# ezeli/InSentiCap_model

Hardware: AMD Instinct MI355X
Metric: captions/sec (greedy, 36-region feats, len-20) (higher is better)
Workload: dtype f32

## Files before the change

include/insenticap_hip.h:

```cpp
#ifndef INSENTICAP_HIP_H
#define INSENTICAP_HIP_H

#include <stdint.h>

#ifdef __cplusplus
extern "C" {
#endif

#define ISC_OK 0
#define ISC_E_NULL (-1)
#define ISC_E_SHAPE (-2)
#define ISC_E_ALIGN (-3)
#define ISC_E_WORKSPACE (-4)
#define ISC_E_STATE (-5)

#define ISC_MAX_SEG 4

int isc_abi_version(void);
const char *isc_target_arch(void);
int isc_set_tile_override(int tile);
int isc_set_h3_mode(int mode);
long long isc_h3_launches(void);
int isc_set_gemv_rows(int rows);
long long isc_gemv_launches(void);
long long isc_h3x_launches(void);
long long isc_h3s_launches(void);
long long isc_f32_launches(int kind);
long long isc_h3_kernel_launches(int kind);
int isc_h3_weights_begin(void *buf, long long bytes, void *stream);
int isc_h3_weights_end(void *stream);
int isc_h3_weights_suspend(void *stream);
int isc_h3_weights_resume(void *buf, void *stream);
int isc_h3_weights_refresh(void *stream);

typedef struct {
    const float *A;
    const float *W;
    int32_t lda, ldw, K;
    int32_t a_f16;
    const void *A_hi, *A_lo;
} isc_seg;

typedef struct {
    isc_seg seg[ISC_MAX_SEG];
    int32_t nseg, M, N, relu;
    const float *bias0, *bias1, *bias2;
    const uint8_t *keep_mask;
    float mask_scale;
    int32_t ldc;
    float *C;
    float *C_pre;
    int32_t accumulate;
    int32_t _pad;
    float *splitk_ws;
    int64_t splitk_ws_floats;
} isc_linear_problem;

int isc_linear_fwd(const isc_linear_problem *probs_host, int n_prob, void *stream);
int isc_linear_f16_native(const isc_linear_problem *probs_host, int n_prob, void *stream);
long long isc_h3_f16a_launches(void);
int isc_f16_to_f32(const void *src, int64_t ld_src, float *dst, int64_t ld_dst, int64_t rows, int64_t cols,
                   void *stream);
long long isc_f16_convert_launches(void);

#define ISC_LAYOUT_NN 1
#define ISC_LAYOUT_TN 2
int isc_gemm_bwd(const isc_linear_problem *probs_host, int n_prob, int layout, void *stream);

typedef struct {
    isc_seg seg[ISC_MAX_SEG];
    int32_t nseg, M, H, _pad;
    const float *b_ih, *b_hh;
    const float *c_prev;
    float *h_out, *c_out;
    float *gates_out;
    const uint8_t *h_keep_mask;
    float mask_scale;
    float *hdrop_out;
    void *h_hi, *h_lo;
    const float *pre;
    const float *tab;
    const int64_t *tab_ids;
    int64_t tab_ids_stride;
    float *splitk_ws;
    int64_t splitk_ws_floats;
    int32_t pre_div, _pad2;
} isc_lstm_problem;

int isc_lstm_fwd(const isc_lstm_problem *prob_host, void *stream);

int isc_vocab_fwd(const float *h, int ldh, const float *W, int ldw, const float *bias,
                  int M, int V, int K, float *logits, int64_t ld_logits,
                  float *part_max, float *part_sum, int32_t *part_idx,
                  const void *h_hi, const void *h_lo,
                  float *splitk_ws, int64_t splitk_ws_floats, void *stream);

int isc_logsoftmax_apply(float *logits, int64_t ld_logits, int M, int V,
                         const float *part_max, const float *part_sum, float *lse_out,
                         void *stream);
int isc_logsoftmax_apply_steps(float *logits, int64_t ld_b, int64_t ld_t, int B, int T, int V,
                               const float *part_max, const float *part_sum, const float *src, int step_rows,
                               void *stream);

typedef struct {
    const float *P, *V, *q, *q2, *w;
    const float *w_bias;
    int32_t R, A, D;
    int32_t rows;
    float *out;
    float *alpha_out;
    int64_t alpha_ld;
    void *out_hi, *out_lo;
    const int64_t *row_ids;
    int64_t row_ids_ld;
    int32_t row_div, _pad;
} isc_scan_problem;

int isc_attn_scan_fwd(const isc_scan_problem *probs_host, int n_prob, int B, void *stream);

typedef struct {
    isc_scan_problem scan[2];
    const float *G[2];
    const float *zh;
    const float *b_gc, *b_gs;
    const float *w_gate;
    const float *b_gate;
    float *f;
    void *f_hi, *f_lo;
    float *beta;
    int64_t beta_ld;
} isc_scan_gate_args;
int isc_attn_scan_gate_fwd(const isc_scan_gate_args *args_host, int B, void *stream);

int isc_gate_mix_fwd(const float *z, const float *w, const float *w_bias, const float *v,
                     const float *s, int B, int A, int D, float *out, float *beta_out,
                     int64_t beta_ld, void *out_hi, void *out_lo, void *stream);

int isc_embed_relu_fwd(const float *emb, int V, int W, const int64_t *ids, int64_t ids_stride,
                       const float *add, int B, float *out, void *stream);

int isc_embed_relu_mean_fwd(const float *emb, int V, int W, const int64_t *ids, int C, int B,
                            float *out, void *stream);

int isc_embed_senti_words_fwd(const float *emb, int V, int W, const int64_t *ids, int n_words,
                              int64_t pad_id, int B, const uint8_t *keep_mask, float mask_scale,
                              float *out, void *stream);

typedef struct {
    int32_t B, V, T, t;
    int32_t n_tile, W;
    const float *part_max, *part_sum;
    const int32_t *part_idx;
    const float *logits;
    int64_t ld_logits;
    const int64_t *forced;
    const float *sample_u;
    int64_t eos_id;
    int64_t *seq;
    float *seq_logprobs;
    float *seq_masks;
    int32_t *unfinished;
    int32_t *alive;
    int64_t *raw_tokens;
    const float *emb;
    const float *xt_add;
    float *xt_next;
} isc_rollout_step;

int isc_rollout_finalize(const isc_rollout_step *s_host, void *stream);
long long isc_rollout_finalize_launches(void);

typedef struct {
// ... 17 lines not shown
int isc_sched_sample(const float *logp, int64_t ld, int M, int V, const float *part_max,
                     const float *part_sum, const int32_t *part_idx, const float *u_select,
                     const float *u_draw, float ss_prob, const int64_t *base_ids, int64_t base_stride,
                     int64_t *out_ids, void *stream);
int isc_sched_sample_raw(const float *logits, int64_t ld, int M, int V, const float *part_max,
                     const float *part_sum, const int32_t *part_idx, const float *u_select,
                     const float *u_draw, float ss_prob, const int64_t *base_ids, int64_t base_stride,
                     int64_t *out_ids, void *stream);

int isc_beam_topk(const float *logits, int64_t ld_logits, const float *part_max,
                  const float *part_sum, int n_tile, int rows, int V, int beam,
                  const int64_t *last_word, int64_t pad_id, int64_t sos_id, int64_t unk_id,
                  int mask_special, int decoding_constraint, float *top_val, int64_t *top_idx,
                  void *stream);

typedef struct {
    int32_t n_img, beam, T, t;
    int64_t eos_id;
    const float *top_val;
    const int64_t *top_idx;
    const double *score_in;
    double *score_out;
    const int64_t *last_in;
    int64_t *last_out;
    const int64_t *words_in;
    int64_t *words_out;
    const int32_t *len_in;
    int32_t *len_out;
    int32_t *done;
    int64_t *gather;
    int32_t *live;
} isc_beam_merge_args;

int isc_beam_merge(const isc_beam_merge_args *args_host, void *stream);
int isc_beam_gather(const float *state_next, const float *state_cur, const int64_t *gather, float *out,
                    int planes, int rows, int H, void *stream);

#define ISC_COPY_MULTI_MAX 8
int isc_copy_multi(void *const *dst, const void *const *src, const int64_t *bytes, int n, void *stream);

int isc_xe_loss_fwd(const float *logp, const int64_t *target, const int32_t *lengths, int B,
                    int T, int V, float *out2, void *stream);


typedef struct {
    int32_t rows, H, E, A, W, V, R, Mw;
    const float *Wih1, *Whh1;
    const float *Wih2, *Whh2;
    const float *b_ih2, *b_hh2;
    const float *W_h2att, *b_h2att, *w_alpha_c, *b_alpha_c;
    const float *W_h2word, *b_h2word, *w_alpha_s, *b_alpha_s;
    const float *W_gh, *b_gh, *W_gc, *b_gc, *W_gs, *b_gs, *w_gate, *b_gate;
    const float *W_cls, *b_cls;
    const float *pre1;
    const float *tab;
    const float *att_p, *att_e;
    const float *words_p, *words_e;
    const float *label_w;
    const float *xt;
    const int64_t *tok;
    int64_t tok_stride;
    const float *h1_prev, *c1_prev, *h2_prev, *c2_prev;
    float *h1, *c1, *h2, *c2;
    float *g1, *g2;
    float *qa, *v, *qw, *s, *z, *f;
    float *alpha_c, *alpha_s, *beta;
    int64_t alpha_c_ld, alpha_s_ld, beta_ld;
    const uint8_t *out_mask;
    float out_scale;
    int32_t apply_logsoftmax;
    float *hdrop;
    float *logits;
    int64_t ld_logits;
    float *pmax, *psum;
    int32_t *pidx;
    float *splitk_ws;
    int64_t splitk_ws_floats;
    const void *h1_prev_hi, *h1_prev_lo, *h2_prev_hi, *h2_prev_lo;
    void *h1_hi, *h1_lo, *h2_hi, *h2_lo;
    void *v_hi, *v_lo, *s_hi, *s_lo, *f_hi, *f_lo;
    const int64_t *words_ids;
    int64_t words_ids_ld;
    const float *gate_Gc, *gate_Gs;
    int32_t pair_rows_c, _pad2;
    int32_t row_div, pre_rows;
} isc_step_plan;

int isc_step_fwd(const isc_step_plan *plan_host, void *stream);

int isc_set_stream_gate(const int32_t *flag, void *stream);

typedef struct {
    const int64_t *src_row;
    int32_t stats_tile, beam;
    float *cand_val;
    int32_t *cand_idx;
    const int64_t *last_word;
    int64_t pad_id, sos_id, unk_id;
    int32_t mask_special, decoding_constraint;
    int32_t row_div, _pad;
    const int32_t *live_in;
    const isc_rollout_step *fin_prev;
    int32_t *fin_unfinished_out;
} isc_rows_ext;
int isc_rows_stats_tile(int V);
int isc_rows_step_supported(const isc_step_plan *plan_host);
int isc_rows_step_fwd(const isc_step_plan *plan_host, const isc_rows_ext *ext_host, void *stream);
int isc_rows_vocab_fwd(const float *h, int ldh, const float *W, int ldw, const float *bias, int M, int V, int K,
                       float *part_max, float *part_sum, int32_t *part_idx, float *logits, int64_t ld_logits,
                       const isc_rows_ext *ext_host, void *stream);
int isc_set_rows_nt(int mode);
long long isc_rows_launches(void);
int isc_set_rows_scan_max(int rows);
int isc_set_rows_scan_regions(int regions);
int isc_set_h3v(int on);
int isc_set_h3_ksplit(int on);
int isc_set_h3_vocab_tile(int rows);

typedef struct {
    int32_t n_img, beam, T, t;
    int32_t n_tile, V;
    int64_t eos_id;
    const float *part_max, *part_sum;
    const float *cand_val;
    const int32_t *cand_idx;
    const double *score_in;
    double *score_out;
    const int64_t *last_in;
    int64_t *last_out;
    const int64_t *words_in;
    int64_t *words_out;
    const int32_t *len_in;
    int32_t *len_out;
    int32_t *done;
    int64_t *src_row;
    int32_t *live;
    float *top_val;
    int64_t *top_idx;
    const int32_t *live_in;
    const float *state_in;
    float *state_out;
    int32_t state_planes, H;
} isc_beam_select_args;
int isc_beam_select(const isc_beam_select_args *args_host, void *stream);

typedef struct {
    int32_t rows, H, E, A, W, R, Mw, first, last;
    int32_t pair_rows_c;
    const float *Wih1, *Whh1, *Wih2, *Whh2;
    const float *W_h2att, *w_alpha_c, *W_h2word, *w_alpha_s, *W_gh, *W_gc, *W_gs, *w_gate;
    const float *att_p, *att_e, *words_p, *words_e, *label_w;
    const float *g1, *c1_prev, *c1, *g2, *c2_prev, *c2;
    const float *qa, *qw, *v, *s, *z;
    const float *alpha_c, *alpha_s, *beta;
    int64_t alpha_c_ld, alpha_s_ld, beta_ld;
    const float *dhd;
    float *dG1, *dG2;
    float *dG1_sum;
    float *d_feat, *dh1, *dv, *ds;
    float *dh2_rec, *dh1_rec;
    const float *dc1_in, *dc2_in;
    float *dc1_out, *dc2_out;
    float *dqa, *dqw, *dz;
    float *dP_att, *dV_att, *dP_w, *dV_w;
    float *dwc_rows, *dws_rows, *dwg_rows, *dbg_rows;
    float *splitk_ws;
    int64_t splitk_ws_floats;
    float *de_c, *de_s;
    int32_t row_div, _pad;
} isc_step_bwd_plan;

// ... 172 lines not shown
```

insenticap_model_amd/_lib.py:

```python
import ctypes as C
import os

_HERE = os.path.dirname(os.path.abspath(__file__))
LIB_PATH = os.environ.get('ISC_HIP_LIB') or os.path.join(_HERE, 'lib', 'libinsenticap_hip.so')

ISC_MAX_SEG = 4

c_f32p = C.c_void_p


class Seg(C.Structure):
    _fields_ = [('A', C.c_void_p), ('W', C.c_void_p), ('lda', C.c_int32), ('ldw', C.c_int32),
                ('K', C.c_int32), ('a_f16', C.c_int32), ('A_hi', C.c_void_p), ('A_lo', C.c_void_p)]


class LinearProblem(C.Structure):
    _fields_ = [('seg', Seg * ISC_MAX_SEG), ('nseg', C.c_int32), ('M', C.c_int32), ('N', C.c_int32),
                ('relu', C.c_int32), ('bias0', C.c_void_p), ('bias1', C.c_void_p), ('bias2', C.c_void_p),
                ('keep_mask', C.c_void_p), ('mask_scale', C.c_float), ('ldc', C.c_int32),
                ('C', C.c_void_p), ('C_pre', C.c_void_p), ('accumulate', C.c_int32), ('_pad', C.c_int32),
                ('splitk_ws', C.c_void_p), ('splitk_ws_floats', C.c_int64)]


class LstmProblem(C.Structure):
    _fields_ = [('seg', Seg * ISC_MAX_SEG), ('nseg', C.c_int32), ('M', C.c_int32), ('H', C.c_int32),
                ('_pad', C.c_int32), ('b_ih', C.c_void_p), ('b_hh', C.c_void_p),
                ('c_prev', C.c_void_p), ('h_out', C.c_void_p), ('c_out', C.c_void_p),
                ('gates_out', C.c_void_p), ('h_keep_mask', C.c_void_p), ('mask_scale', C.c_float),
                ('hdrop_out', C.c_void_p), ('h_hi', C.c_void_p), ('h_lo', C.c_void_p),
                ('pre', C.c_void_p), ('tab', C.c_void_p),
                ('tab_ids', C.c_void_p), ('tab_ids_stride', C.c_int64),
                ('splitk_ws', C.c_void_p), ('splitk_ws_floats', C.c_int64),
                ('pre_div', C.c_int32), ('_pad2', C.c_int32)]


class ScanProblem(C.Structure):
    _fields_ = [('P', C.c_void_p), ('V', C.c_void_p), ('q', C.c_void_p), ('q2', C.c_void_p),
                ('w', C.c_void_p), ('w_bias', C.c_void_p), ('R', C.c_int32), ('A', C.c_int32),
                ('D', C.c_int32), ('rows', C.c_int32), ('out', C.c_void_p), ('alpha_out', C.c_void_p),
                ('alpha_ld', C.c_int64), ('out_hi', C.c_void_p), ('out_lo', C.c_void_p),
                ('row_ids', C.c_void_p), ('row_ids_ld', C.c_int64), ('row_div', C.c_int32), ('_pad', C.c_int32)]


class ScanBwdProblem(C.Structure):
    _fields_ = [('P', C.c_void_p), ('V', C.c_void_p), ('q', C.c_void_p), ('q2', C.c_void_p),
                ('w', C.c_void_p), ('alpha', C.c_void_p), ('dout', C.c_void_p), ('alpha_ld', C.c_int64),
                ('R', C.c_int32), ('A', C.c_int32), ('D', C.c_int32), ('accumulate', C.c_int32),
                ('dP', C.c_void_p), ('dV', C.c_void_p), ('dq', C.c_void_p), ('dw_rows', C.c_void_p),
                ('de_out', C.c_void_p), ('rows', C.c_int32), ('row_div', C.c_int32)]


class ScanGateArgs(C.Structure):
    _fields_ = [('scan', ScanProblem * 2), ('G', C.c_void_p * 2), ('zh', C.c_void_p), ('b_gc', C.c_void_p),
                ('b_gs', C.c_void_p), ('w_gate', C.c_void_p), ('b_gate', C.c_void_p), ('f', C.c_void_p),
                ('f_hi', C.c_void_p), ('f_lo', C.c_void_p), ('beta', C.c_void_p), ('beta_ld', C.c_int64)]


def _f(names, ctype):
    return [(n, ctype) for n in names.split()]


class StepPlan(C.Structure):
    _fields_ = (_f('rows H E A W V R Mw', C.c_int32) +
                _f('Wih1 Whh1 Wih2 Whh2 b_ih2 b_hh2 W_h2att b_h2att w_alpha_c b_alpha_c W_h2word b_h2word '
                   'w_alpha_s b_alpha_s W_gh b_gh W_gc b_gc W_gs b_gs w_gate b_gate W_cls b_cls '
                   'pre1 tab att_p att_e words_p words_e label_w xt tok', C.c_void_p) +
                [('tok_stride', C.c_int64)] +
                _f('h1_prev c1_prev h2_prev c2_prev h1 c1 h2 c2 g1 g2 qa v qw s z f alpha_c alpha_s beta',
                   C.c_void_p) +
                _f('alpha_c_ld alpha_s_ld beta_ld', C.c_int64) +
                [('out_mask', C.c_void_p), ('out_scale', C.c_float), ('apply_logsoftmax', C.c_int32),
                 ('hdrop', C.c_void_p), ('logits', C.c_void_p), ('ld_logits', C.c_int64),
                 ('pmax', C.c_void_p), ('psum', C.c_void_p), ('pidx', C.c_void_p),
                 ('splitk_ws', C.c_void_p), ('splitk_ws_floats', C.c_int64)] +
                _f('h1_prev_hi h1_prev_lo h2_prev_hi h2_prev_lo h1_hi h1_lo h2_hi h2_lo '
                   'v_hi v_lo s_hi s_lo f_hi f_lo words_ids', C.c_void_p) + [('words_ids_ld', C.c_int64)] +
                _f('gate_Gc gate_Gs', C.c_void_p) + _f('pair_rows_c _pad2 row_div pre_rows', C.c_int32))


class StepBwdPlan(C.Structure):
    _fields_ = (_f('rows H E A W R Mw first last pair_rows_c', C.c_int32) +
                _f('Wih1 Whh1 Wih2 Whh2 W_h2att w_alpha_c W_h2word w_alpha_s W_gh W_gc W_gs w_gate '
                   'att_p att_e words_p words_e label_w g1 c1_prev c1 g2 c2_prev c2 qa qw v s z '
                   'alpha_c alpha_s beta', C.c_void_p) +
                _f('alpha_c_ld alpha_s_ld beta_ld', C.c_int64) +
                _f('dhd dG1 dG2 dG1_sum d_feat dh1 dv ds dh2_rec dh1_rec dc1_in dc2_in dc1_out dc2_out '
                   'dqa dqw dz dP_att dV_att dP_w dV_w dwc_rows dws_rows dwg_rows dbg_rows splitk_ws',
                   C.c_void_p) + [('splitk_ws_floats', C.c_int64), ('de_c', C.c_void_p), ('de_s', C.c_void_p),
                              ('row_div', C.c_int32), ('_pad', C.c_int32)])


class BeamMergeArgs(C.Structure):
    _fields_ = ([('n_img', C.c_int32), ('beam', C.c_int32), ('T', C.c_int32), ('t', C.c_int32), ('eos_id', C.c_int64)] +
                _f('top_val top_idx score_in score_out last_in last_out words_in words_out len_in len_out done gather live',
                   C.c_void_p))


class RowsExt(C.Structure):
    _fields_ = [('src_row', C.c_void_p), ('stats_tile', C.c_int32), ('beam', C.c_int32), ('cand_val', C.c_void_p),
                ('cand_idx', C.c_void_p), ('last_word', C.c_void_p), ('pad_id', C.c_int64), ('sos_id', C.c_int64),
                ('unk_id', C.c_int64), ('mask_special', C.c_int32), ('decoding_constraint', C.c_int32),
                ('row_div', C.c_int32), ('_pad', C.c_int32), ('live_in', C.c_void_p), ('fin_prev', C.c_void_p),
                ('fin_unfinished_out', C.c_void_p)]


class BeamSelectArgs(C.Structure):
    _fields_ = ([('n_img', C.c_int32), ('beam', C.c_int32), ('T', C.c_int32), ('t', C.c_int32), ('n_tile', C.c_int32),
                 ('V', C.c_int32), ('eos_id', C.c_int64)] +
                _f('part_max part_sum cand_val cand_idx score_in score_out last_in last_out words_in words_out len_in '
                   'len_out done src_row live top_val top_idx live_in state_in state_out', C.c_void_p) +
                [('state_planes', C.c_int32), ('H', C.c_int32)])


ISC_COLSUM_MAX_JOBS, ISC_COLSUM_MAX_OUT = 24, 3
ISC_SCALE_SRC_MAX = 4


class ColsumJob(C.Structure):
    _fields_ = [('x', C.c_void_p), ('ld', C.c_int64), ('M', C.c_int32), ('N', C.c_int32),
                ('out', C.c_void_p * ISC_COLSUM_MAX_OUT), ('n_out', C.c_int32), ('accumulate', C.c_int32)]


class RolloutStep(C.Structure):
    _fields_ = [('B', C.c_int32), ('V', C.c_int32), ('T', C.c_int32), ('t', C.c_int32),
                ('n_tile', C.c_int32), ('W', C.c_int32),
                ('part_max', C.c_void_p), ('part_sum', C.c_void_p), ('part_idx', C.c_void_p),
                ('logits', C.c_void_p), ('ld_logits', C.c_int64),
                ('forced', C.c_void_p), ('sample_u', C.c_void_p), ('eos_id', C.c_int64),
                ('seq', C.c_void_p), ('seq_logprobs', C.c_void_p), ('seq_masks', C.c_void_p),
                ('unfinished', C.c_void_p), ('alive', C.c_void_p), ('raw_tokens', C.c_void_p),
                ('emb', C.c_void_p), ('xt_add', C.c_void_p), ('xt_next', C.c_void_p)]


class SampleFilter(C.Structure):
    _fields_ = [('temperature', C.c_float), ('top_k', C.c_int32), ('top_p', C.c_float),
                ('sampling_logprobs', C.c_void_p)]


class DecodeConstraints(C.Structure):
    _fields_ = [('ban_ids', C.c_int64 * 8), ('n_ban', C.c_int32), ('no_repeat', C.c_int32), ('first_id', C.c_int64),
                ('min_len', C.c_int32)]


class SentClsProblem(C.Structure):
    _fields_ = (_f('B L W H V k T_out _pad', C.c_int32) + [('tokens', C.c_void_p), ('tokens_ld', C.c_int64)] +
                _f('lens emb w_ih w_hh b_ih b_hh ex0_w ex0_b ex2_w ex2_b cls0_w cls0_b cls3_w cls3_b labels workspace',
                   C.c_void_p) + [('workspace_bytes', C.c_int64)] + _f('logits weights pred reward feats', C.c_void_p))


SENTI_DET_MAX_CONVS = SENTI_DET_MAX_FCS = 4
SENTI_DET_MAX_HW = 1024
SENTI_DET_KINDS = ('direct', 'split', 'reduce', 'tail', 'pack', 'f16')


class SentiDetProblem(C.Structure):
    _fields_ = ([('feats', C.c_void_p)] + _f('feats_f16 B h w C n_convs n_fcs k neu_idx ksplit', C.c_int32) +
                [('threshold', C.c_float), ('_pad', C.c_int32), ('packed', C.c_void_p),
                 ('conv_b', C.c_void_p * SENTI_DET_MAX_CONVS)] + _f('senti_w senti_b', C.c_void_p) +
                [('fc_w', C.c_void_p * SENTI_DET_MAX_FCS), ('fc_b', C.c_void_p * SENTI_DET_MAX_FCS),
                 ('workspace', C.c_void_p), ('workspace_bytes', C.c_int64)] +
                _f('logits maps labels scores conv_out', C.c_void_p))


SIGNATURES = {
    'isc_abi_version': (C.c_int, []),
    'isc_target_arch': (C.c_char_p, []),
    'isc_set_tile_override': (C.c_int, [C.c_int]),
    'isc_set_h3_mode': (C.c_int, [C.c_int]),
    'isc_h3_launches': (C.c_longlong, []),
    'isc_set_gemv_rows': (C.c_int, [C.c_int]),
    'isc_colsum_multi': (C.c_int, [C.POINTER(ColsumJob), C.c_int, C.c_void_p, C.c_int64, C.c_void_p]),
    'isc_gemv_launches': (C.c_longlong, []),
    'isc_h3x_launches': (C.c_longlong, []),
    'isc_h3s_launches': (C.c_longlong, []),
    'isc_f32_launches': (C.c_longlong, [C.c_int]),
    'isc_h3_kernel_launches': (C.c_longlong, [C.c_int]),
    'isc_h3_weights_begin': (C.c_int, [C.c_void_p, C.c_longlong, C.c_void_p]),
    'isc_h3_weights_end': (C.c_int, [C.c_void_p]),
    'isc_h3_weights_suspend': (C.c_int, [C.c_void_p]),
    'isc_h3_weights_resume': (C.c_int, [C.c_void_p, C.c_void_p]),
    'isc_h3_weights_refresh': (C.c_int, [C.c_void_p]),
    'isc_linear_fwd': (C.c_int, [C.POINTER(LinearProblem), C.c_int, C.c_void_p]),
    'isc_linear_f16_native': (C.c_int, [C.POINTER(LinearProblem), C.c_int, C.c_void_p]),
    'isc_h3_f16a_launches': (C.c_longlong, []),
    'isc_f16_to_f32': (C.c_int, [C.c_void_p, C.c_int64, C.c_void_p, C.c_int64, C.c_int64, C.c_int64, C.c_void_p]),
    'isc_f16_convert_launches': (C.c_longlong, []),
    'isc_gemm_bwd': (C.c_int, [C.POINTER(LinearProblem), C.c_int, C.c_int, C.c_void_p]),
    'isc_lstm_fwd': (C.c_int, [C.POINTER(LstmProblem), C.c_void_p]),
    'isc_step_fwd': (C.c_int, [C.POINTER(StepPlan), C.c_void_p]),
    'isc_set_stream_gate': (C.c_int, [C.c_void_p, C.c_void_p]),
    'isc_step_bwd': (C.c_int, [C.POINTER(StepBwdPlan), C.c_void_p]),
    'isc_rows_stats_tile': (C.c_int, [C.c_int]),
    'isc_rows_step_supported': (C.c_int, [C.POINTER(StepPlan)]),
    'isc_rows_step_fwd': (C.c_int, [C.POINTER(StepPlan), C.POINTER(RowsExt), C.c_void_p]),
    'isc_rows_vocab_fwd': (C.c_int, [C.c_void_p, C.c_int, C.c_void_p, C.c_int, C.c_void_p, C.c_int, C.c_int, C.c_int,
                                     C.c_void_p, C.c_void_p, C.c_void_p, C.c_void_p, C.c_int64, C.POINTER(RowsExt),
                                     C.c_void_p]),
    'isc_set_rows_nt': (C.c_int, [C.c_int]),
    'isc_set_rows_scan_max': (C.c_int, [C.c_int]),
    'isc_set_rows_scan_regions': (C.c_int, [C.c_int]),
    'isc_set_h3v': (C.c_int, [C.c_int]),
    'isc_set_h3_ksplit': (C.c_int, [C.c_int]),
    'isc_set_h3_vocab_tile': (C.c_int, [C.c_int]),
    'isc_copy_multi': (C.c_int, [C.POINTER(C.c_void_p), C.POINTER(C.c_void_p), C.POINTER(C.c_int64), C.c_int, C.c_void_p]),
    'isc_rows_launches': (C.c_longlong, []),
    'isc_beam_select': (C.c_int, [C.POINTER(BeamSelectArgs), C.c_void_p]),
    'isc_vocab_fwd': (C.c_int, [C.c_void_p, C.c_int, C.c_void_p, C.c_int, C.c_void_p, C.c_int, C.c_int,
                                C.c_int, C.c_void_p, C.c_int64, C.c_void_p, C.c_void_p, C.c_void_p,
                                C.c_void_p, C.c_void_p, C.c_void_p, C.c_int64, C.c_void_p]),
    'isc_sched_sample': (C.c_int, [C.c_void_p, C.c_int64, C.c_int, C.c_int, C.c_void_p, C.c_void_p, C.c_void_p,
                                   C.c_void_p, C.c_void_p, C.c_float, C.c_void_p, C.c_int64, C.c_void_p,
                                   C.c_void_p]),
    'isc_sched_sample_raw': (C.c_int, [C.c_void_p, C.c_int64, C.c_int, C.c_int, C.c_void_p, C.c_void_p, C.c_void_p,
                                   C.c_void_p, C.c_void_p, C.c_float, C.c_void_p, C.c_int64, C.c_void_p,
                                   C.c_void_p]),
    'isc_logsoftmax_apply': (C.c_int, [C.c_void_p, C.c_int64, C.c_int, C.c_int, C.c_void_p, C.c_void_p,
                                       C.c_void_p, C.c_void_p]),
    'isc_logsoftmax_apply_steps': (C.c_int, [C.c_void_p, C.c_int64, C.c_int64, C.c_int, C.c_int, C.c_int, C.c_void_p,
                                             C.c_void_p, C.c_void_p, C.c_int, C.c_void_p]),
    'isc_attn_scan_fwd': (C.c_int, [C.POINTER(ScanProblem), C.c_int, C.c_int, C.c_void_p]),
    'isc_attn_scan_gate_fwd': (C.c_int, [C.POINTER(ScanGateArgs), C.c_int, C.c_void_p]),
    'isc_gate_mix_fwd': (C.c_int, [C.c_void_p, C.c_void_p, C.c_void_p, C.c_void_p, C.c_void_p, C.c_int,
                                   C.c_int, C.c_int, C.c_void_p, C.c_void_p, C.c_int64, C.c_void_p, C.c_void_p,
                                   C.c_void_p]),
    'isc_embed_relu_fwd': (C.c_int, [C.c_void_p, C.c_int, C.c_int, C.c_void_p, C.c_int64, C.c_void_p,
                                     C.c_int, C.c_void_p, C.c_void_p]),
    'isc_embed_relu_mean_fwd': (C.c_int, [C.c_void_p, C.c_int, C.c_int, C.c_void_p, C.c_int, C.c_int,
                                          C.c_void_p, C.c_void_p]),
    'isc_embed_senti_words_fwd': (C.c_int, [C.c_void_p, C.c_int, C.c_int, C.c_void_p, C.c_int, C.c_int64,
                                            C.c_int, C.c_void_p, C.c_float, C.c_void_p, C.c_void_p]),
    'isc_rollout_finalize': (C.c_int, [C.POINTER(RolloutStep), C.c_void_p]),
    'isc_rollout_finalize_launches': (C.c_longlong, []),
    'isc_rollout_finalize_filtered': (C.c_int, [C.POINTER(RolloutStep), C.POINTER(SampleFilter), C.c_void_p]),
    'isc_rollout_finalize_constrained': (C.c_int, [C.POINTER(RolloutStep), C.POINTER(SampleFilter),
                                                   C.POINTER(DecodeConstraints), C.c_void_p]),
    'isc_beam_merge': (C.c_int, [C.POINTER(BeamMergeArgs), C.c_void_p]),
    'isc_beam_gather': (C.c_int, [C.c_void_p, C.c_void_p, C.c_void_p, C.c_void_p, C.c_int, C.c_int, C.c_int, C.c_void_p]),
    'isc_beam_topk': (C.c_int, [C.c_void_p, C.c_int64, C.c_void_p, C.c_void_p, C.c_int, C.c_int, C.c_int,
                                C.c_int, C.c_void_p, C.c_int64, C.c_int64, C.c_int64, C.c_int, C.c_int,
                                C.c_void_p, C.c_void_p, C.c_void_p]),
    'isc_xe_loss_fwd': (C.c_int, [C.c_void_p, C.c_void_p, C.c_void_p, C.c_int, C.c_int, C.c_int,
                                  C.c_void_p, C.c_void_p]),
    'isc_logsoftmax_bwd': (C.c_int, [C.c_void_p, C.c_void_p, C.c_int64, C.c_int, C.c_int, C.c_void_p,
                                     C.c_int64, C.c_int, C.c_void_p]),
    'isc_lstm_bwd': (C.c_int, [C.c_void_p, C.c_void_p, C.c_void_p, C.c_void_p, C.c_void_p, C.c_void_p,
                               C.c_int, C.c_int, C.c_void_p, C.c_void_p, C.c_void_p, C.c_void_p]),
    'isc_attn_scan_bwd': (C.c_int, [C.POINTER(ScanBwdProblem), C.c_int, C.c_int, C.c_void_p]),
    'isc_attn_dv_from_alpha': (C.c_int, [C.c_void_p, C.c_int64, C.c_int64, C.c_void_p, C.c_int, C.c_int, C.c_int,
                                         C.c_int, C.c_void_p, C.c_int, C.c_void_p]),
    'isc_attn_dp_from_de': (C.c_int, [C.c_void_p, C.c_void_p, C.c_void_p, C.c_void_p, C.c_void_p, C.c_int, C.c_int,
                                      C.c_int, C.c_int, C.c_void_p, C.c_void_p]),
    'isc_attn_dv_from_alpha_group': (C.c_int, [C.c_void_p, C.c_int64, C.c_int64, C.c_void_p, C.c_int, C.c_int, C.c_int,
                                               C.c_int, C.c_int, C.c_void_p, C.c_int, C.c_void_p]),
    'isc_attn_dp_from_de_group': (C.c_int, [C.c_void_p, C.c_void_p, C.c_void_p, C.c_void_p, C.c_void_p, C.c_int, C.c_int,
                                            C.c_int, C.c_int, C.c_int, C.c_void_p, C.c_void_p]),
    'isc_gate_mix_bwd': (C.c_int, [C.c_void_p, C.c_void_p, C.c_void_p, C.c_void_p, C.c_void_p, C.c_int64,
                                   C.c_void_p, C.c_int, C.c_int, C.c_int, C.c_void_p, C.c_void_p,
                                   C.c_void_p, C.c_void_p, C.c_void_p, C.c_int, C.c_void_p]),
    'isc_embed_relu_bwd': (C.c_int, [C.c_void_p, C.c_int, C.c_int, C.c_void_p, C.c_int64, C.c_int, C.c_int,
                                     C.c_int, C.c_int64, C.c_void_p, C.c_float, C.c_void_p, C.c_float,
                                     C.c_void_p, C.c_int64, C.c_void_p]),
    'isc_embed_relu_bwd_ws': (C.c_int, [C.c_void_p, C.c_int, C.c_int, C.c_void_p, C.c_int64, C.c_int, C.c_int,
                                        C.c_int, C.c_int64, C.c_void_p, C.c_float, C.c_void_p, C.c_float,
                                        C.c_void_p, C.c_int64, C.c_void_p, C.c_int64, C.c_void_p]),
    'isc_colsum': (C.c_int, [C.c_void_p, C.c_int64, C.c_int, C.c_int, C.c_void_p, C.c_int, C.c_void_p, C.c_int64,
                             C.c_void_p]),
    'isc_relu_mask_bwd': (C.c_int, [C.c_void_p, C.c_void_p, C.c_void_p, C.c_float, C.c_int64, C.c_void_p,
                                    C.c_void_p]),
    'isc_xe_loss_bwd': (C.c_int, [C.c_void_p, C.c_void_p, C.c_int, C.c_int, C.c_int, C.c_void_p,
                                  C.c_void_p, C.c_void_p, C.c_void_p]),
    'isc_xe_loss_bwd_sparse': (C.c_int, [C.c_void_p, C.c_int, C.c_int, C.c_void_p, C.c_void_p, C.c_void_p, C.c_void_p]),
    'isc_reward_loss_fwd': (C.c_int, [C.c_void_p, C.c_void_p, C.c_void_p, C.c_int, C.c_int, C.c_void_p, C.c_void_p]),
# ... 71 lines not shown
```

insenticap_model_amd/captioner.py:

```python
import ctypes as C
import itertools
import weakref

import torch
import torch.nn as nn

from . import _lib, ops
from ._lib import RolloutStep


class ContentAttention(nn.Module):
    def __init__(self, settings):
        super().__init__()
        self.h2att = nn.Linear(settings['rnn_hid_dim'], settings['att_hid_dim'])
        self.att_alpha = nn.Linear(settings['att_hid_dim'], 1)


class SentiAttention(nn.Module):
    def __init__(self, settings):
        super().__init__()
        self.h2word = nn.Linear(settings['rnn_hid_dim'], settings['att_hid_dim'])
        self.label2word = nn.Linear(settings['word_emb_dim'], settings['att_hid_dim'])
        self.word_alpha = nn.Linear(settings['att_hid_dim'], 1)

# ... 315 lines not shown
        if cached is not None:
            return cached
        if not build:
            return None
        st = self.settings
        H, E, Wd, V = st['rnn_hid_dim'], st['feat_emb_dim'], st['word_emb_dim'], self.vocab_size
        act = self._new(V, Wd)
        ops.embed_relu_fwd(emb, torch.arange(V, dtype=torch.int64, device=self._dev), act)
        tab = self._new(V, 4 * H)
        ops.linear_fwd([ops.linear_problem([(act, Wih[:, H + E:])], tab)])
        return self._table_cache('_tab_cache', key, tab)

    ROWS_STEP_MAX = 8

    def _rows_step_ok(self, rows, P):
        st = self.settings
        E, A, Wd, H = st['feat_emb_dim'], st['att_hid_dim'], st['word_emb_dim'], st['rnn_hid_dim']
        return (getattr(self, 'rows_step', True) and 0 < rows <= self.ROWS_STEP_MAX and not ops.TIMER.armed
                and self._rows_vocab_ok()
                and ops.TIMER.arm_step is None and getattr(P, 'gate_Gc', None) is not None
                and getattr(P, 'gate_Gs', None) is not None and A == E == Wd and A <= 512 and A % 4 == 0 and H % 4 == 0
                and H <= 1024)

    def _rows_vocab_ok(self):
        V = self.vocab_size
        tw = ops.rows_stats_tile(V)
        return tw > 0 and (V + tw - 1) // tw <= 256

    def _alloc_step_ws(self, rows, P, stats_tile=128):
        st = self.settings
        E, A = st['feat_emb_dim'], st['att_hid_dim']
        has_cont, has_senti = P.att_e3 is not None, P.words_e3 is not None
        ws = {}
        if has_cont:
            ws['qa'], ws['v'] = self._new(rows, A), self._new(rows, E)
        if has_senti:
            ws['qw'], ws['s'] = self._new(rows, A), self._new(rows, E)
        if has_cont and has_senti:
            ws['z'], ws['f'] = self._new(rows, A), self._new(rows, E)
        n_tile = (self.vocab_size + stats_tile - 1) // stats_tile
        ws['pmax'] = self._new(rows, n_tile)
        ws['psum'] = self._new(rows, n_tile)
        ws['pidx'] = self._new(rows, n_tile, dtype=torch.int32)
        return ws

    def _make_plan(self, p, P, rows):
        st = self.settings
        pl = _lib.StepPlan()
        pl.rows, pl.H, pl.E, pl.A = rows, st['rnn_hid_dim'], st['feat_emb_dim'], st['att_hid_dim']
        pl.W, pl.V, pl.R, pl.Mw = st['word_emb_dim'], self.vocab_size, P.R, P.Mw
        for field, key in (('Wih1', 'att_lstm.weight_ih'), ('Whh1', 'att_lstm.weight_hh'),
                           ('Wih2', 'lang_lstm.weight_ih'), ('Whh2', 'lang_lstm.weight_hh'),
                           ('b_ih2', 'lang_lstm.bias_ih'), ('b_hh2', 'lang_lstm.bias_hh'),
                           ('W_h2att', 'attention.cont_att.h2att.weight'), ('b_h2att', 'attention.cont_att.h2att.bias'),
                           ('w_alpha_c', 'attention.cont_att.att_alpha.weight'),
                           ('b_alpha_c', 'attention.cont_att.att_alpha.bias'),
                           ('W_h2word', 'attention.senti_att.h2word.weight'),
                           ('b_h2word', 'attention.senti_att.h2word.bias'),
                           ('w_alpha_s', 'attention.senti_att.word_alpha.weight'),
                           ('b_alpha_s', 'attention.senti_att.word_alpha.bias'),
                           ('W_gh', 'attention.h2att.weight'), ('b_gh', 'attention.h2att.bias'),
                           ('W_gc', 'attention.cont2att.weight'), ('b_gc', 'attention.cont2att.bias'),
                           ('W_gs', 'attention.senti2att.weight'), ('b_gs', 'attention.senti2att.bias'),
                           ('w_gate', 'attention.att_alpha.weight'), ('b_gate', 'attention.att_alpha.bias'),
                           ('W_cls', 'classifier.weight'), ('b_cls', 'classifier.bias')):
            t = p[key]
            assert t.is_contiguous()
            setattr(pl, field, t.data_ptr())
        for field, t in (('pre1', P.pre1), ('tab', P.tab), ('att_p', P.att_p3), ('att_e', P.att_e3),
                         ('words_p', P.words_p3), ('words_e', P.words_e3), ('label_w', P.label_w)):
            if t is not None:
                assert t.is_contiguous()
                setattr(pl, field, t.data_ptr())
        if P.words_ids is not None:
            pl.words_ids, pl.words_ids_ld = P.words_ids.data_ptr(), P.words_ids.stride(0)
        ws = ops.splitk_ws(self._dev)
        pl.splitk_ws, pl.splitk_ws_floats = ws.data_ptr(), ws.numel()
        pl.row_div = P.row_div if P.row_div > 1 else 0
        pl.pre_rows = int(P.pre_rows)
        return pl

    def _step(self, p, P, ws, xt, h_cur, c_cur, h_nxt, c_nxt, alpha_c=None, alpha_s=None, beta=None,
              logits=None, out_mask=None, out_scale=1.0, save=None, tok=None, normalize=False,
              hp_cur=None, hp_nxt=None, rows_ext=None):
        if ops.TIMER.armed:
            return self._step_py(p, P, ws, xt, h_cur, c_cur, h_nxt, c_nxt, alpha_c, alpha_s, beta, logits,
                                 out_mask, out_scale, save, tok, normalize, hp_cur, hp_nxt)
        save = save or {}
        pl = ws.get('_plan')
        if pl is None:
            pl = ws['_plan'] = self._make_plan(p, P, h_cur[0].shape[0])
        ptr = ops.ptr
        pl.xt = ptr(xt)
        if tok is not None and P.tab is not None:
            pl.tok, pl.tok_stride = tok.data_ptr(), tok.stride(0)
        pl.h1_prev, pl.h2_prev, pl.c1_prev, pl.c2_prev = (h_cur[0].data_ptr(), h_cur[1].data_ptr(),
                                                          c_cur[0].data_ptr(), c_cur[1].data_ptr())
        pl.h1, pl.h2, pl.c1, pl.c2 = (h_nxt[0].data_ptr(), h_nxt[1].data_ptr(), c_nxt[0].data_ptr(),
                                      c_nxt[1].data_ptr())
        if hp_cur is not None:
            pl.h1_prev_hi, pl.h1_prev_lo = ops.planes_ptrs(hp_cur[0])
            pl.h2_prev_hi, pl.h2_prev_lo = ops.planes_ptrs(hp_cur[1])
            pl.h1_hi, pl.h1_lo = ops.planes_ptrs(hp_nxt[0])
            pl.h2_hi, pl.h2_lo = ops.planes_ptrs(hp_nxt[1])
            for k in ('v', 's', 'f'):
                pp = ws.get(k + 'p')
                hi, lo = (None, None) if pp is None else ops.planes_ptrs(pp)
                setattr(pl, k + '_hi', hi)
                setattr(pl, k + '_lo', lo)
        else:
            for k in ('h1_prev_hi', 'h1_prev_lo', 'h2_prev_hi', 'h2_prev_lo', 'h1_hi', 'h1_lo', 'h2_hi', 'h2_lo',
                      'v_hi', 'v_lo', 's_hi', 's_lo', 'f_hi', 'f_lo'):
                setattr(pl, k, None)
        pl.g1, pl.g2 = ptr(save.get('g1')), ptr(save.get('g2'))
        for k in ('qa', 'v', 'qw', 's', 'z', 'f'):
            setattr(pl, k, ptr(ws.get(k)))
        pl.alpha_c, pl.alpha_c_ld = (alpha_c.data_ptr(), alpha_c.stride(0)) if alpha_c is not None else (None, 0)
        pl.alpha_s, pl.alpha_s_ld = (alpha_s.data_ptr(), alpha_s.stride(0)) if alpha_s is not None else (None, 0)
        pl.beta, pl.beta_ld = (beta.data_ptr(), beta.stride(0)) if beta is not None else (None, 0)
        hdrop = None
        if out_mask is not None:
            hdrop = save['hdrop'] if 'hdrop' in save else self._new(h_cur[0].shape[0], pl.H)
        pl.out_mask, pl.out_scale, pl.hdrop = ptr(out_mask), out_scale, ptr(hdrop)
        pl.logits, pl.ld_logits = (logits.data_ptr(), logits.stride(0)) if logits is not None else (None, 0)
        pl.apply_logsoftmax = int(normalize)
        pl.pmax, pl.psum, pl.pidx = ptr(ws.get('pmax')), ptr(ws.get('psum')), ptr(ws.get('pidx'))
        pl.gate_Gc, pl.gate_Gs = ptr(getattr(P, 'gate_Gc', None)), ptr(getattr(P, 'gate_Gs', None))
        if rows_ext is not None:
            ops.rows_step_fwd(pl, rows_ext)
        else:
            ops.step_fwd(pl)

    def _step_py(self, p, P, ws, xt, h_cur, c_cur, h_nxt, c_nxt, alpha_c=None, alpha_s=None, beta=None,
                 logits=None, out_mask=None, out_scale=1.0, save=None, tok=None, normalize=False,
                 hp_cur=None, hp_nxt=None):
        save = save or {}
        st = self.settings
        E, H = st['feat_emb_dim'], st['rnn_hid_dim']
        Wih, Whh = p['att_lstm.weight_ih'], p['att_lstm.weight_hh']
        rows = h_cur[0].shape[0]
        pc = (lambda l: None) if hp_cur is None else (lambda l: hp_cur[l])
        pn = (lambda l: None) if hp_nxt is None else (lambda l: hp_nxt[l])
        wp = (lambda k: None) if hp_cur is None else (lambda k: ws.get(k + 'p'))
        segs = [(h_cur[1], Wih[:, 0:H], pc(1)), (h_cur[0], Whh, pc(0))]
        if P.tab is None:
            segs.insert(1, (xt, Wih[:, H + E:]))
        ops.lstm_fwd(segs, None, None, c_cur[0], h_nxt[0], c_nxt[0], gates_out=save.get('g1'),
                     pre=P.pre1, tab=P.tab, tab_ids=tok if P.tab is not None else None, h_planes=pn(0),
                     pre_div=1 if P.pre_rows else P.row_div)
        h1 = h_nxt[0]
        has_cont, has_senti = P.att_e3 is not None, P.words_e3 is not None
        probs, scans = [], []
        if has_cont:
            probs.append(ops.linear_problem([(h1, p['attention.cont_att.h2att.weight'], pn(0))], ws['qa'],
                                            p['attention.cont_att.h2att.bias']))
            scans.append(ops.scan_problem(P.att_p3, P.att_e3, ws['qa'],
                                          p['attention.cont_att.att_alpha.weight'],
                                          p['attention.cont_att.att_alpha.bias'], ws['v'], alpha_c,
                                          out_planes=wp('v'), row_div=P.row_div))
        if has_senti:
            probs.append(ops.linear_problem([(h1, p['attention.senti_att.h2word.weight'], pn(0))], ws['qw'],
                                            p['attention.senti_att.h2word.bias']))
            scans.append(ops.scan_problem(P.words_p3, P.words_e3, ws['qw'],
                                          p['attention.senti_att.word_alpha.weight'],
                                          p['attention.senti_att.word_alpha.bias'], ws['s'], alpha_s,
                                          q2=P.label_w, out_planes=wp('s'), row_ids=P.words_ids,
                                          row_div=P.row_div))
        gate = has_cont and has_senti
        if gate:
            probs.append(ops.linear_problem([(h1, p['attention.h2att.weight'], pn(0))], ws['z'],
                                            p['attention.h2att.bias']))
        ops.linear_fwd(probs)
        fused_gate = gate and getattr(P, 'gate_Gc', None) is not None and getattr(P, 'gate_Gs', None) is not None
        if fused_gate:
            ops.attn_scan_gate_fwd(scans, (P.gate_Gc, P.gate_Gs), ws['z'], p['attention.cont2att.bias'],
                                   p['attention.senti2att.bias'], p['attention.att_alpha.weight'],
                                   p['attention.att_alpha.bias'], ws['f'], beta, f_planes=wp('f'))
            feat, featp = ws['f'], wp('f')
        else:
            ops.attn_scan_fwd(scans, rows)
        if fused_gate:
            pass
        elif gate:
            ops.linear_fwd([ops.linear_problem(
                [(ws['v'], p['attention.cont2att.weight'], wp('v')),
                 (ws['s'], p['attention.senti2att.weight'], wp('s'))],
                ws['z'], p['attention.cont2att.bias'], p['attention.senti2att.bias'], accumulate=True)])
            ops.gate_mix_fwd(ws['z'], p['attention.att_alpha.weight'], p['attention.att_alpha.bias'],
                             ws['v'], ws['s'], ws['f'], beta, out_planes=wp('f'))
            feat, featp = ws['f'], wp('f')
        else:
            feat, featp = (ws['v'], wp('v')) if has_cont else (ws['s'], wp('s'))
        Wih2, Whh2 = p['lang_lstm.weight_ih'], p['lang_lstm.weight_hh']
        hdrop = None
        if out_mask is not None:
            hdrop = save['hdrop'] if 'hdrop' in save else self._new(rows, H)
        ops.lstm_fwd([(feat, Wih2[:, 0:E], featp), (h1, Wih2[:, E:E + H], pn(0)), (h_cur[1], Whh2, pc(1))],
                     p['lang_lstm.bias_ih'], p['lang_lstm.bias_hh'], c_cur[1], h_nxt[1], c_nxt[1],
                     gates_out=save.get('g2'), h_keep_mask=out_mask, mask_scale=out_scale, hdrop_out=hdrop,
                     h_planes=pn(1))
        if ws.get('pmax') is None:
            return
        ops.vocab_fwd(hdrop if hdrop is not None else h_nxt[1], p['classifier.weight'],
                      p['classifier.bias'], ws['pmax'], ws['psum'], ws['pidx'], logits,
                      h_planes=None if hdrop is not None else pn(1))
        if normalize:
            ops.logsoftmax_apply(logits, ws['pmax'], ws['psum'])

    def _set_weights(self, aC, aS, bG, steps):
        self._weights_pending = (aC, aS, bG, steps)
# ... 190 lines not shown
                             'torch.no_grad() (the backward through 1 / temperature is not built)')
        if not sample_max and not self._needs_grad() and _replay is None and (
                filtered or return_sampling_logprobs or _uniforms is not None or generator is not None):
            filt = self._sample_filter(temperature, top_k, top_p, generator, _uniforms, return_sampling_logprobs)
            out = self._rollout(fc_feats, att_feats, cpt_words, senti_words, senti_labels, max_seq_len, 0, None,
                                _masks, filt, group=n_cap, cons=cons)
            return out[:3] + ((filt['slp'],) if return_sampling_logprobs else ())
        if return_sampling_logprobs or _uniforms is not None or generator is not None:
            raise ValueError('generator / return_sampling_logprobs / _uniforms are not available with gradients enabled')
        if not sample_max and self._needs_grad():
            from .autograd import rollout_with_grad
            return rollout_with_grad(self, fc_feats, att_feats, cpt_words, senti_words, senti_labels,
                                     max_seq_len, _replay, _masks, cons, group=n_cap)
        if (sample_max and cons is None and self.__dict__.get('_rollout_graphs') is not None and not self._needs_grad()
                and not self.training and _replay is None and _masks is None and ops.TIMER.arm_step is None
                and fc_feats.shape[0] <= self.ROLLOUT_GRAPH_MAX_ROWS and ops.graphs_allowed_here()
                and fc_feats.is_cuda and not torch.cuda.is_current_stream_capturing()
                and self._features_in_domain(fc_feats, att_feats)):
            return self._graphed_rollout(fc_feats, att_feats, cpt_words, senti_words, senti_labels, max_seq_len)
        return self._rollout(fc_feats, att_feats, cpt_words, senti_words, senti_labels, max_seq_len,
                             sample_max, _replay, _masks, group=n_cap, cons=cons)[:3]

    def _decode_constraints(self, suppress_special, decoding_constraint, min_len, max_seq_len):
        special, no_repeat, min_len = ops.check_decode_constraints(suppress_special, decoding_constraint, min_len,
                                                                   max_seq_len)
        ban = []
        if special and self.pad_id != self.eos_id:
            for i in (self.pad_id, self.sos_id, self.unk_id):
                if i not in ban:
                    ban.append(i)
        if not ban and not no_repeat and not min_len:
            return None
        if self.vocab_size <= len(ban) + 2:
            raise ValueError('a vocabulary of %d words leaves nothing to choose under the constraints' % self.vocab_size)
        return ops.decode_constraints(ban, no_repeat, self.sos_id, min_len)

    def _check_captions_per_image(self, n, sample_max, masks, fc_feats=None, senti_labels=None):
        if isinstance(n, bool) or not hasattr(n, '__index__'):
            raise ValueError('captions_per_image must be an integer >= 1, got %r' % (n,))
        n = int(n)
        if n < 1:
            raise ValueError('captions_per_image must be an integer >= 1, got %r' % (n,))
        if n == 1:
            return 1
        if sample_max:
            raise ValueError('captions_per_image > 1 applies to sampled roll-outs (sample_max=0): %d greedy captions of '
                             'one image would be identical' % n)
        grad = self._needs_grad()
        if bool(self.training) != grad:
            raise ValueError('captions_per_image > 1 runs in two forms: inference-only (eval mode under torch.no_grad()) '
                             'or the differentiable training roll-out (training mode with gradients enabled); got '
                             'training=%s with gradients %s' % (bool(self.training), 'enabled' if grad else 'disabled'))
        if masks is not None and not grad:
            raise ValueError('captions_per_image > 1 without gradients does not take _masks (dropout masks belong to '
                             'training)')
        if grad and fc_feats is not None and senti_labels is not None:
            images, labels = int(fc_feats.shape[0]), int(senti_labels.numel())
            if labels != images:
                raise ValueError('captions_per_image=%d with gradients: senti_labels must hold one label per image (%d) - '
                                 'the roll-out takes its labels from the image - got %d' % (n, images, labels))
        return n

    def _sample_filter(self, temperature=1.0, top_k=0, top_p=1.0, generator=None, uniforms=None, want_slp=False):
        temperature, top_k, top_p = ops.check_sample_filter(temperature, top_k, top_p)
        return dict(temperature=temperature, top_k=top_k, top_p=top_p, generator=generator, uniforms=uniforms,
                    want_slp=bool(want_slp),
                    filtered=temperature != 1.0 or 0 < top_k < self.vocab_size or top_p < 1.0)

    def enable_rollout_graphs(self, on=True, max_graphs=4):
        self._rollout_graphs = {} if on else None
        self._rollout_graphs_max = max_graphs
        self._graphs_explicit = bool(on)

    def _rollout_stream(self):
        st = self.__dict__.get('_ro_stream')
        if st is None or st.device != self._dev:
            st = self.__dict__['_ro_stream'] = ops.private_stream(self._dev)
            idx = self._dev.index if self._dev.index is not None else torch.cuda.current_device()
            weakref.finalize(self, ops.release_stream_state, idx, st.cuda_stream)
        return st

    def _graphed_rollout(self, fc_feats, att_feats, cpt_words, senti_words, senti_labels, T):
        ins = [self._feat(fc_feats), self._feat(att_feats), cpt_words, senti_words, senti_labels]
        key = (tuple((tuple(x.shape), x.dtype) for x in ins), T, self._weights_key(), torch.cuda.current_device())
        cache = self._rollout_graphs
        st = self._rollout_stream()
        idx = self._dev.index if self._dev.index is not None else torch.cuda.current_device()
        skey = ((idx, st.cuda_stream),)
        cur = torch.cuda.current_stream(self._dev)

        def on_stream(fn):
            st.wait_stream(cur)
            with torch.cuda.stream(st):
                out = fn()
            cur.wait_stream(st)
            return out
        entry = cache.get(key)
        if isinstance(entry, tuple) and entry[4] != ops.h3_weights_scope.cold_begins(skey):
            entry = cache[key] = 'seen'
        if entry is None:
            while len(cache) >= self._rollout_graphs_max:
                self._graph_evicted(cache.pop(next(iter(cache))), 'roll-out')
                if self._rollout_graphs is None:
                    return self._rollout(*ins, T, 1, None, None)[:3]
            cache[key] = 'seen'
            outs = on_stream(lambda: self._rollout(*ins, T, 1, None, None)[:3])
            for o in outs:
                o.record_stream(cur)
            return outs
        cache[key] = cache.pop(key)
        if entry == 'seen':
            static = [x.clone() for x in ins]
            graph = torch.cuda.CUDAGraph()

            def capture():
                with ops.graph_capture(graph, stream=st):
                    o = self._rollout(*static, T, 1, None, None)[:3]
                    return o, self.__dict__.get('_weights_pending')
            outs, pending = on_stream(capture)
            entry = cache[key] = (graph, static, outs, pending, ops.h3_weights_scope.cold_begins(skey))
        graph, static, outs, pending = entry[:4]
        ops.stage_inputs(static, ins)
        graph.replay()
        self._weights_pending = pending
        fresh = [torch.empty_like(o) for o in outs]
        ops.copy_multi(fresh, outs)
        return tuple(fresh)

    GRAPH_THRASH_LIMIT = 8

    def _graph_evicted(self, entry, what):
        if isinstance(entry, str):
            return
        n = self.__dict__['_graph_evictions'] = self.__dict__.get('_graph_evictions', 0) + 1
        if n == self.GRAPH_THRASH_LIMIT and not self.__dict__.get('_graphs_explicit', False):
            import warnings
            warnings.warn('insenticap_model_amd: %d captured %s / beam graphs evicted - input geometries keep changing; '
                          'default graph serving is off for this captioner (enable_rollout_graphs / enable_beam_graphs '
                          'with a larger max_graphs to keep it)' % (n, what))
            self._rollout_graphs = None
            self._beam_graphs = None

    def enable_beam_graphs(self, on=True, max_graphs=4):
        self._beam_graphs = {} if on else None
        self._beam_graphs_max = max_graphs
        self._graphs_explicit = bool(on)

    def _weights_key(self):
        return (('captioner', self._wnonce[0]),) + tuple((q.data_ptr(), q._version) for q in self.parameters()) + \
            (ops.WEIGHT_EPOCH,)

    def _renew_weights_nonce(self):
        self._wnonce[0] = next(_INSTANCE_NONCE)

    def _apply(self, fn, *args, **kwargs):
        out = super()._apply(fn, *args, **kwargs)
        self._renew_weights_nonce()
        return out

    def load_state_dict(self, *args, **kwargs):
        out = super().load_state_dict(*args, **kwargs)
        self._renew_weights_nonce()
        return out

    def _graph_buffers(self):
        gb = self.__dict__.get('_graph_bufs')
        if gb is None or gb[0].device != self._dev:
# ... 8 lines not shown
        if not self._features_in_domain(fc_feats, att_feats):
            with ops.exact_fp32_engine(), ops.h3_weights_scope(self._dev, key=self._weights_key()):
                return self._rollout_impl(fc_feats, att_feats, cpt_words, senti_words, senti_labels, T, sample_max,
                                          replay, masks, filt, group, cons)
        with ops.h3_weights_scope(self._dev, key=self._weights_key()):
            return self._rollout_impl(fc_feats, att_feats, cpt_words, senti_words, senti_labels, T, sample_max,
                                      replay, masks, filt, group, cons)

    SPLIT_F16_MAX = 65504.0

    def _features_in_domain(self, *feats):
        feats = [x for x in feats if x is not None and torch.is_tensor(x) and x.is_floating_point()]
        if (not getattr(self, 'numerics_checks', True) or self.__dict__.get('_domain_check_off') or not feats
                or not all(x.is_cuda for x in feats)
                or ops.h3_mode() == 0 or torch.cuda.is_current_stream_capturing()):
            return True
        memo = self.__dict__.setdefault('_domain_memo', {})
        verdict, fresh = True, []
        for x in feats:
            e = memo.get(id(x))
            if e is not None and e[0]() is x and e[1] == x._version:
                verdict = verdict and e[2]
            else:
                fresh.append(x)
        if fresh:
            worst = torch.stack([torch.linalg.vector_norm(x.detach().reshape(-1), float('inf')).float()
                                 for x in fresh]).amax()
            v = float(worst)
            ok = bool(v < self.SPLIT_F16_MAX)
            for k in [k for k, e in memo.items() if e[0]() is None]:
                del memo[k]
            while len(memo) >= 16:
                memo.pop(next(iter(memo)))
            for x in fresh:
                memo[id(x)] = (weakref.ref(x), x._version, ok)
            verdict = verdict and ok
            if not ok:
                self._warn_out_of_domain('max |x| = %g' % v)
        return verdict

    def _known_out_of_domain(self, *feats, remember=False):
        bad = self.__dict__.setdefault('_domain_bad', {})
        keys = [(x.data_ptr(), x.numel(), x._version) for x in feats
                if x is not None and torch.is_tensor(x) and x.is_floating_point()]
        if remember:
            while len(bad) >= 16:
                bad.pop(next(iter(bad)))
            for k in keys:
                bad[k] = True
            return True
        return any(k in bad for k in keys)

    def _warn_out_of_domain(self, what):
        if not self.__dict__.get('_domain_warned'):
            import warnings
            self.__dict__['_domain_warned'] = True
            warnings.warn('insenticap_model_amd: features beyond the split-f16 operand domain |x| < 65504 (%s): the call '
                          'runs on the exact-fp32 GEMM engine (~2x slower; results as the reference\'s). Scale the '
                          'features to keep the fast engine.' % what)

    def _rollout_impl(self, fc_feats, att_feats, cpt_words, senti_words, senti_labels, T, sample_max, replay,
                      masks, filt=None, group=1, cons=None):
        p = self._p()
        arm = ops.TIMER.arm_step
        ops.TIMER.armed, ops.TIMER.phase = (arm == -1), 'prologue'
        n_rows = fc_feats.shape[0] * group
        want = False
        if not torch.is_grad_enabled() or not any(q.requires_grad for q in self.parameters()):
            want = 'build' if n_rows * T >= self.vocab_size // 4 else 'cached'
        P = self._prologue(p, 'rl', fc_feats, att_feats, cpt_words, senti_words, senti_labels, masks,
                           want_table=want, words_table=bool(want) and getattr(self, 'words_table', True),
                           gate_rows=n_rows if want and group == 1 else 0)
        ops.TIMER.armed, ops.TIMER.phase = False, 'step'
        P.row_div = group
        B, V = P.B * group, self.vocab_size
        H, Wd = self.att_lstm.hidden_size, self.settings['word_emb_dim']
        rows_ext = None
        if ((sample_max or replay is not None) and masks is None and not self.training and group == 1
                and cons is None and self._rows_step_ok(B, P)):
            rows_ext = _lib.RowsExt()
            rows_ext.stats_tile = ops.rows_stats_tile(V)
        planes = rows_ext is None and getattr(self, 'state_planes', True)
        f32, i64 = torch.float32, torch.int64
        h0, c0, hp0 = self._zeros_many(((2, B, H), f32), ((2, B, H), f32),
                                       ((2, 2, B, H) if planes else (0,), torch.float16))
        seq, raw, seq_logprobs, seq_masks, alive, aC, aS, bG, unf = self._zeros_many(
            ((B, T), i64), ((B, T), i64), ((B, T), f32), ((B, T), f32), ((T + 1,), torch.int32), ((B, T, P.R), f32),
            ((B, T, P.Mw), f32), ((B, T), f32), ((T + 1, B), torch.int32))
        h, c = [h0, self._new(2, B, H)], [c0, self._new(2, B, H)]
        hp = [hp0, torch.empty(2, 2, B, H, dtype=torch.float16, device=self._dev)] if planes else [None, None]
        ws = self._alloc_step_ws(B, P, rows_ext.stats_tile if rows_ext is not None else 128)
        if hp[0] is not None:
            for k in ('v', 's', 'f'):
                if k in ws:
                    ws[k + 'p'] = torch.empty((2,) + tuple(ws[k].shape), dtype=torch.float16, device=self._dev)
        unf[0:1].fill_(1)
        unfinished = unf[0]
        alive[0:1].fill_(B)
        use_tab = P.tab is not None
        xt = [None, None] if use_tab else [self._new(B, Wd) for _ in range(2)]
        emb = p['word_embed.0.weight']
        sos = torch.full((B,), self.sos_id, dtype=torch.int64, device=self._dev)
        if not use_tab:
            ops.embed_relu_fwd(emb, sos, xt[0])
        need_logits = (not sample_max) or cons is not None
        logits = self._new(B, V) if need_logits else None
        forced = sample_u = None
        if not sample_max:
            if replay is not None:
                forced = self._ids(replay)
            elif filt is not None and filt['uniforms'] is not None:
                sample_u = filt['uniforms']
                if (not torch.is_tensor(sample_u) or sample_u.dtype != torch.float32 or tuple(sample_u.shape) != (B, T)):
                    raise ValueError('_uniforms must be a float32 tensor of shape [B, T] = [%d, %d]' % (B, T))
                sample_u = sample_u.to(self._dev).contiguous()
            elif filt is not None and filt['generator'] is not None:
                sample_u = torch.rand(B, T, device=self._dev, generator=filt['generator'])
            else:
                sample_u = torch.rand(B, T, device=self._dev)
        filtered = filt is not None and filt['filtered']
        slp = None
        if filt is not None and filt['want_slp'] and (filtered or cons is not None):
            slp = self._zeros(B, T)
        mask_for = self._mask_source(masks)
        rs = RolloutStep()
        rs.B, rs.V, rs.T, rs.n_tile, rs.W = B, V, T, ws['pmax'].shape[1], Wd
        rs.part_max, rs.part_sum, rs.part_idx = ws['pmax'].data_ptr(), ws['psum'].data_ptr(), ws['pidx'].data_ptr()
        rs.logits, rs.ld_logits = ops.ptr(logits), V
        rs.forced, rs.sample_u = ops.ptr(forced), ops.ptr(sample_u)
        rs.eos_id = self.eos_id
        rs.seq, rs.seq_logprobs, rs.seq_masks = seq.data_ptr(), seq_logprobs.data_ptr(), seq_masks.data_ptr()
        rs.unfinished, rs.alive, rs.raw_tokens = unfinished.data_ptr(), alive.data_ptr(), raw.data_ptr()
        rs.emb, rs.xt_add = emb.data_ptr(), None
        fuse = (rows_ext is not None and sample_max and replay is None and use_tab and arm is None and B <= 4
                and getattr(self, 'rows_fused_finalize', True))
        rs_prev = RolloutStep.from_buffer_copy(rs) if fuse else None
        with ops.h3_weights_scope(self._dev):
            for t in range(T):
                cur, nxt = t & 1, (t + 1) & 1
                om, osc = mask_for('out%d' % t, B, H)
                ops.TIMER.armed = (arm == t)
                if fuse:
                    if t > 0:
                        rs_prev.t, rs_prev.unfinished = t - 1, unf[t - 1].data_ptr()
                        rows_ext.fin_prev, rows_ext.fin_unfinished_out = C.addressof(rs_prev), unf[t].data_ptr()
                    else:
                        rows_ext.fin_prev = rows_ext.fin_unfinished_out = None
                self._step(p, P, ws, xt[cur], h[cur], c[cur], h[nxt], c[nxt], aC[:, t], aS[:, t], bG[:, t:t + 1],
                           logits, om, osc, tok=(sos if t == 0 else seq[:, t - 1]) if use_tab else None,
                           hp_cur=hp[cur], hp_nxt=hp[nxt], rows_ext=rows_ext)
                if fuse and t + 1 < T:
                    continue
                rs.t = t
                rs.unfinished = unf[t].data_ptr() if fuse else unfinished.data_ptr()
                rs.xt_next = None if use_tab else xt[nxt].data_ptr()
                ops.rollout_finalize_step(rs, cons, filt, slp)
        ops.TIMER.armed = False
        if filt is not None and filt['want_slp']:
            filt['slp'] = slp if slp is not None else seq_logprobs.clone()
        self._set_weights(aC, aS, bG, alive)
        return seq, seq_logprobs, seq_masks, raw, alive

    def sample(self, fc_feat, att_feat, senti_words=None, senti_label=None,
               beam_size=3, decoding_constraint=1, max_seq_len=16):
        caps, scores, _ = self.sample_batch(
            fc_feat.reshape(1, -1), att_feat.reshape(1, -1, att_feat.shape[-1]),
            None if senti_words is None else senti_words.reshape(1, -1),
            None if senti_label is None else senti_label.reshape(1),
            beam_size, decoding_constraint, max_seq_len)
        return caps[0], scores[0]

    @torch.no_grad()
    def sample_batch(self, fc_feats, att_feats, senti_words=None, senti_labels=None,
                     beam_size=3, decoding_constraint=1, max_seq_len=16):
        from .beam import beam_search_batch, replay_if_captured
        if self.training:
            self.eval()
        checks = getattr(self, 'numerics_checks', True)

        def on_exact_engine():
            self._p()
            with ops.exact_fp32_engine(), ops.h3_weights_scope(self._dev, key=self._weights_key()):
                res = beam_search_batch(self, fc_feats, att_feats, senti_words, senti_labels, beam_size,
                                        decoding_constraint, max_seq_len, graphs=False)
            ops.device_status(reset=True)
            return res
        if checks and ops.h3_mode() != 0 and self._known_out_of_domain(fc_feats, att_feats):
            return on_exact_engine()
        out = replay_if_captured(self, fc_feats, att_feats, senti_words, senti_labels, beam_size, decoding_constraint,
                                 max_seq_len)
        if out is None:
            self._p()
            with ops.h3_weights_scope(self._dev, key=self._weights_key()):
                out = beam_search_batch(self, fc_feats, att_feats, senti_words, senti_labels, beam_size,
                                        decoding_constraint, max_seq_len)
        if checks:
            if ops.h3_mode() != 0 and ops.device_status(reset=True):
                self._known_out_of_domain(fc_feats, att_feats, remember=True)
                self._warn_out_of_domain('non-finite values in a beam search')
                return on_exact_engine()
            ops.check_numerics('Captioner.sample')
        return out

    @torch.no_grad()
    def sample_captions(self, fc_feats, att_feats, cpt_words, senti_words, senti_labels, n=1, max_seq_len=16,
                        temperature=1.0, top_k=0, top_p=1.0, generator=None, _uniforms=None, share_image=False,
                        suppress_special=False, decoding_constraint=0, min_len=0):
        n = int(n)
        if n < 1:
            raise ValueError('n must be >= 1, got %r' % (n,))
        ops.check_sample_filter(temperature, top_k, top_p)
        cons = dict(zip(('suppress_special', 'decoding_constraint', 'min_len'),
                        ops.check_decode_constraints(suppress_special, decoding_constraint, min_len, max_seq_len)))
        if self.training:
            self.eval()

        def rep(x):
            return None if x is None else x.repeat_interleave(n, dim=0)
        if share_image and n > 1:
            seq, _, masks = self.forward_rl(fc_feats, att_feats, cpt_words, senti_words, senti_labels, max_seq_len, 0,
                                            temperature=temperature, top_k=top_k, top_p=top_p, generator=generator,
                                            _uniforms=_uniforms, captions_per_image=n, **cons)
        else:
            seq, _, masks = self.forward_rl(rep(fc_feats), rep(att_feats), rep(cpt_words), rep(senti_words),
                                            rep(senti_labels), max_seq_len, 0, temperature=temperature, top_k=top_k,
                                            top_p=top_p, generator=generator, _uniforms=_uniforms, **cons)
        seq_h, len_h = seq.cpu().tolist(), masks.sum(1).long().cpu().tolist()
        i2w, eos = self.idx2word, self.eos_id
        captions, ids = [], []
        for i in range(len(seq_h) // n):
            rows = [seq_h[i * n + j][:len_h[i * n + j]] for j in range(n)]
            captions.append([' '.join(i2w[w] for w in words if w != eos) for words in rows])
            ids.append(rows)
# ... 23 lines not shown
```

insenticap_model_amd/csrc/attention.hip:

```cpp
#include "common.h"

struct DevScan {
    const float *P, *V, *q, *q2, *w, *w_bias;
    int R, A, D;
    float *out, *alpha_out;
    long long alpha_ld;
    _Float16 *out_hi, *out_lo;
    const int64_t *ids;
    long long ids_ld;
    int rid_off;
    int rows;
};
struct DevScanLaunch {
    DevScan p[2];
    int nt;
    const int *gate;
};
#define ISC_SCAN_NT_BYTES (128LL << 20)
typedef float f4v __attribute__((ext_vector_type(4)));
__device__ __forceinline__ float4 ld4(const float4 *p, bool nt) {
    if (nt) {
        const f4v v = __builtin_nontemporal_load(reinterpret_cast<const f4v *>(p));
        return make_float4(v.x, v.y, v.z, v.w);
    }
// ... 593 lines not shown
    {
        int rc = ISC_OK;
        if (rows_scan_gate_try(a, B, (hipStream_t)stream, &rc)) return rc;
    }
    DevScanGate L = {};
    L.gate = isc_stream_gate_(stream);
    size_t lds = 0;
    const int A = a->scan[0].A, D = a->scan[0].D;
    if (A <= 0 || A != D || (A & 3) || A > 1024) return ISC_E_SHAPE;
    for (int i = 0; i < 2; ++i) {
        const isc_scan_problem &q = a->scan[i];
        if (!q.P || !q.V || !q.q || !q.w) return ISC_E_NULL;
        if (q.R <= 0 || q.A != A || q.D != D) return ISC_E_SHAPE;
        if (!isc_aligned16(q.P) || !isc_aligned16(q.V) || !isc_aligned16(q.q) || !isc_aligned16(q.w) ||
            !isc_aligned16(a->G[i]) || (q.q2 && !isc_aligned16(q.q2)) || (q.out && !isc_aligned16(q.out)))
            return ISC_E_ALIGN;
        if ((q.out_hi == nullptr) != (q.out_lo == nullptr)) return ISC_E_NULL;
        DevScan &d = L.p[i];
        d.P = q.P; d.V = q.V; d.q = q.q; d.q2 = q.q2; d.w = q.w; d.w_bias = q.w_bias;
        d.R = q.R; d.A = q.A; d.D = q.D; d.out = q.out; d.alpha_out = q.alpha_out; d.alpha_ld = q.alpha_ld;
        d.out_hi = static_cast<_Float16 *>(q.out_hi); d.out_lo = static_cast<_Float16 *>(q.out_lo);
        const int nd4 = q.D / 4;
        size_t need = (((size_t)q.R + 3) & ~(size_t)3) + 2 * (size_t)(256 / nd4) * q.D;
        d.ids = q.row_ids; d.ids_ld = q.row_ids_ld; d.rid_off = (int)need;
        if (q.row_ids) need += ((size_t)q.R + 3) & ~(size_t)3;
        if (need > lds) lds = need;
        L.G[i] = a->G[i];
    }
    if (!isc_aligned16(a->zh) || !isc_aligned16(a->b_gc) || !isc_aligned16(a->b_gs) || !isc_aligned16(a->w_gate) ||
        !isc_aligned16(a->f))
        return ISC_E_ALIGN;
    if (lds < (size_t)(2 * A + 16)) lds = 2 * A + 16;
    lds = (lds + 3) & ~(size_t)3;
    L.lds_half = (int)lds;
    lds *= 2 * sizeof(float);
    if (lds > 60000) return ISC_E_SHAPE;
    L.zh = a->zh; L.b_c = a->b_gc; L.b_s = a->b_gs; L.w_g = a->w_gate; L.b_g = a->b_gate;
    L.f = a->f; L.beta = a->beta; L.beta_ld = a->beta_ld;
    L.f_hi = static_cast<_Float16 *>(a->f_hi); L.f_lo = static_cast<_Float16 *>(a->f_lo);
    dim3 grid(B), block(512);
    hipStream_t st = (hipStream_t)stream;
    if (A <= 256) hipLaunchKernelGGL((attn_scan_gate_kernel<1>), grid, block, lds, st, L);
    else if (A <= 512) hipLaunchKernelGGL((attn_scan_gate_kernel<2>), grid, block, lds, st, L);
    else hipLaunchKernelGGL((attn_scan_gate_kernel<4>), grid, block, lds, st, L);
    ISC_LAUNCH_CHECK();
    return ISC_OK;
}

__device__ __forceinline__ bool isc_aligned16_dev(const void *p) { return (reinterpret_cast<uintptr_t>(p) & 15u) == 0; }

__global__ __launch_bounds__(256) void gate_mix_kernel(const float *z, const float *w, const float *w_bias,
                                                       const float *v, const float *s, int B, int A,
                                                       int D, float *out, float *beta_out,
                                                       long long beta_ld, _Float16 *out_hi, _Float16 *out_lo) {
    const int lane = threadIdx.x & 63;
    const int b = blockIdx.x * 4 + (threadIdx.x >> 6);
    if (b >= B) return;
    float acc = 0.f;
    if ((A & 3) == 0 && isc_aligned16_dev(z) && isc_aligned16_dev(w)) {
        const float4 *z4 = reinterpret_cast<const float4 *>(z + (long long)b * A);
        const float4 *w4 = reinterpret_cast<const float4 *>(w);
        for (int a = lane; a < (A >> 2); a += 64) {
            const float4 zz = z4[a], ww = w4[a];
            acc += ww.x * isc_tanh(zz.x);
            acc += ww.y * isc_tanh(zz.y);
            acc += ww.z * isc_tanh(zz.z);
            acc += ww.w * isc_tanh(zz.w);
        }
    } else {
        for (int a = lane; a < A; a += 64) acc += w[a] * isc_tanh(z[(long long)b * A + a]);
    }
    acc = wave_sum(acc);
    const float beta = isc_sigmoid(acc + (w_bias ? w_bias[0] : 0.f));
    if (lane == 0 && beta_out) beta_out[(long long)b * beta_ld] = beta;
    if ((D & 3) == 0) {
        const float4 *v4 = reinterpret_cast<const float4 *>(v + (long long)b * D);
        const float4 *s4 = reinterpret_cast<const float4 *>(s + (long long)b * D);
        float4 *o4 = reinterpret_cast<float4 *>(out + (long long)b * D);
        for (int d = lane; d < (D >> 2); d += 64) {
            const float4 a = v4[d], c = s4[d];
            float4 f;
            f.x = beta * a.x + (1.0f - beta) * c.x; f.y = beta * a.y + (1.0f - beta) * c.y;
            f.z = beta * a.z + (1.0f - beta) * c.z; f.w = beta * a.w + (1.0f - beta) * c.w;
            o4[d] = f;
            if (out_hi) store_planes4(out_hi, out_lo, b, 4 * d, D, f);
        }
        return;
    }
    for (int d = lane; d < D; d += 64) {
        const long long o = (long long)b * D + d;
        const float f = beta * v[o] + (1.0f - beta) * s[o];
        out[o] = f;
        if (out_hi) {
            const long long po = plane_index(b, d, D);
            isc_split_f16(f, out_hi[po], out_lo[po]);
        }
    }
}

extern "C" int isc_gate_mix_fwd(const float *z, const float *w, const float *w_bias, const float *v,
                                const float *s, int B, int A, int D, float *out, float *beta_out,
                                int64_t beta_ld, void *out_hi, void *out_lo, void *stream) {
    if (!z || !w || !v || !s || !out) return ISC_E_NULL;
    if ((out_hi == nullptr) != (out_lo == nullptr)) return ISC_E_NULL;
    if ((D & 3) == 0 && (!isc_aligned16(v) || !isc_aligned16(s) || !isc_aligned16(out))) return ISC_E_ALIGN;
    if (B <= 0 || A <= 0 || D <= 0) return ISC_E_SHAPE;
    hipLaunchKernelGGL(gate_mix_kernel, dim3((B + 3) / 4), dim3(256), 0, (hipStream_t)stream, z, w,
                       w_bias, v, s, B, A, D, out, beta_out, (long long)beta_ld, static_cast<_Float16 *>(out_hi),
                       static_cast<_Float16 *>(out_lo));
    ISC_LAUNCH_CHECK();
    return ISC_OK;
}
```

insenticap_model_amd/csrc/gemm_f32.hip:

```cpp
#include <atomic>
#include <mutex>
#include <type_traits>
#include <utility>

#include "common.h"

typedef float f32x16 __attribute__((ext_vector_type(16)));

using I0 = std::integral_constant<int, 0>;
using I1 = std::integral_constant<int, 1>;
using I2 = std::integral_constant<int, 2>;
using I3 = std::integral_constant<int, 3>;
template <class F, int... Is>
__device__ __forceinline__ void static_for_seq(F &&f, std::integer_sequence<int, Is...>) {
    (f(std::integral_constant<int, Is>{}), ...);
}
template <int N, class F>
__device__ __forceinline__ void static_for(F &&f) {
    static_for_seq(f, std::make_integer_sequence<int, N>{});
}

#define BK 32
#define LDT 36

// ... 239 lines not shown
            if (P.C_pre)
                *reinterpret_cast<float4 *>(P.C_pre + (long long)gm * P.ldc + gn) =
                    make_float4(pre[0], pre[1], pre[2], pre[3]);
            return;
        }
    }
    for (int e = 0; e < NE && gn + e < N; ++e) {
        dst[e] = o[e];
        if (P.C_pre) P.C_pre[(long long)gm * P.ldc + gn + e] = pre[e];
    }
}

template <int BM, int BN>
__device__ __forceinline__ void epi_linear_tile(const DevProb &P, const float *Cs, int row0, int col0, int tid,
                                                int ks, int ksplit) {
    constexpr int LDC = BN + 4;
    const int M = P.M, N = P.N;
    if (ksplit > 1) {
        float *slab = P.slab + (long long)ks * P.slab_stride;
        for (int idx = tid; idx < BM * (BN / 4); idx += 256) {
            const int row = idx / (BN / 4), c4 = (idx % (BN / 4)) * 4;
            const int gm = row0 + row, gn = col0 + c4;
            if (gm < M && gn < N)
                *reinterpret_cast<float4 *>(slab + (long long)gm * N + gn) =
                    *reinterpret_cast<const float4 *>(Cs + row * LDC + c4);
        }
        return;
    }
    for (int idx = tid; idx < BM * (BN / 4); idx += 256) {
        const int row = idx / (BN / 4), c4 = (idx % (BN / 4)) * 4;
        const int gm = row0 + row, gn = col0 + c4;
        if (gm >= M || gn >= N) continue;
        const float4 v = *reinterpret_cast<const float4 *>(Cs + row * LDC + c4);
        float o[4] = {v.x, v.y, v.z, v.w};
        epi_linear_finish<4>(P, gm, gn, o);
    }
}

template <int NE>
__device__ __forceinline__ void lstm_cells(const DevProb &P, const int (&gm)[NE], int unit, const bool (&ok)[NE],
                                           float (&g)[NE][4]) {
    const int H = P.H;
    const bool has_b = P.bias0 != nullptr, has_pre = P.pre != nullptr, has_tab = P.tab != nullptr;
    float q[NE][4], t[NE][4], b[4], cp[NE];
    long long tok[NE];
    if (has_tab) {
#pragma unroll
        for (int e = 0; e < NE; ++e) tok[e] = ok[e] ? P.tab_ids[(long long)gm[e] * P.tab_ids_stride] : 0;
    }
#pragma unroll
    for (int e = 0; e < NE; ++e) cp[e] = ok[e] ? P.c_prev[(long long)gm[e] * H + unit] : 0.f;
    if (has_pre && P.pre_div > 1) {
#pragma unroll
        for (int e = 0; e < NE; ++e) {
            const long long pm = ok[e] ? (unsigned)gm[e] / (unsigned)P.pre_div : 0;
#pragma unroll
            for (int k = 0; k < 4; ++k) q[e][k] = ok[e] ? P.pre[pm * 4 * H + k * H + unit] : 0.f;
        }
    } else if (has_pre) {
#pragma unroll
        for (int e = 0; e < NE; ++e)
#pragma unroll
            for (int k = 0; k < 4; ++k) q[e][k] = ok[e] ? P.pre[(long long)gm[e] * 4 * H + k * H + unit] : 0.f;
    }
    if (has_tab) {
#pragma unroll
        for (int e = 0; e < NE; ++e)
#pragma unroll
            for (int k = 0; k < 4; ++k) t[e][k] = ok[e] ? P.tab[tok[e] * 4 * H + k * H + unit] : 0.f;
    }
    if (has_b) {
#pragma unroll
        for (int k = 0; k < 4; ++k) b[k] = P.bias0[k * H + unit] + P.bias1[k * H + unit];
    }
#pragma unroll
    for (int e = 0; e < NE; ++e) {
#pragma unroll
        for (int k = 0; k < 4; ++k) g[e][k] = isc_lstm_gate_sum(g[e][k], has_b, b[k], has_pre, q[e][k], has_tab, t[e][k]);
        float c2, h2;
        isc_lstm_cell(g[e], cp[e], c2, h2);
        if (ok[e]) {
            const long long o = (long long)gm[e] * H + unit;
            P.c_out[o] = c2;
            P.h_out[o] = h2;
            if (P.h_hi) {
                const long long po = plane_index(gm[e], unit, H);
                isc_split_f16(h2, P.h_hi[po], P.h_lo[po]);
            }
            if (P.hmask) P.hdrop[o] = h2 * (float)P.hmask[o] * P.mask_scale;
            if (P.gates_out) {
                float *go_ = P.gates_out + (long long)gm[e] * 4 * H + unit;
#pragma unroll
                for (int k = 0; k < 4; ++k) go_[k * H] = g[e][k];
            }
        }
    }
}

template <int BM, int BN>
__device__ __forceinline__ void epi_lstm_tile(const DevProb &P, const float *Cs, int row0, int tn, int tid) {
    constexpr int LDC = BN + 4, NE = 4;
    static_assert(BM * 32 % (256 * NE) == 0, "tile rows per thread must be a multiple of the batch");
    const int u = tid & 31;
    for (int base = tid; base < BM * 32; base += 256 * NE) {
        int gm[NE];
        bool ok[NE];
        float g[NE][4];
#pragma unroll
        for (int e = 0; e < NE; ++e) {
            const int row = (base + 256 * e) >> 5;
            gm[e] = row0 + row;
            ok[e] = gm[e] < P.M;
            const float *cr = Cs + row * LDC + u;
            g[e][0] = cr[0]; g[e][1] = cr[32]; g[e][2] = cr[64]; g[e][3] = cr[96];
        }
        lstm_cells<NE>(P, gm, tn * 32 + u, ok, g);
    }
}

__device__ __forceinline__ void epi_lstm_frag(const DevProb &P, f32x16 (&acc)[4], int frow0, int lane, int row0, int tn) {
#pragma unroll
    for (int half = 0; half < 2; ++half) {
        int gm[8];
        bool ok[8];
        float g[8][4];
#pragma unroll
        for (int e = 0; e < 8; ++e) {
            const int r = half * 8 + e;
            gm[e] = row0 + frow0 + Frag32::row(r, lane);
            ok[e] = gm[e] < P.M;
#pragma unroll
            for (int k = 0; k < 4; ++k) g[e][k] = acc[k][r];
        }
        lstm_cells<8>(P, gm, tn * 32 + (lane & 31), ok, g);
    }
}

ISC_STATUS_DECL(gemm)

template <class F, int NC, bool EDGE, bool FEAT, bool RELU, bool CHECK, class Acc>
__device__ __forceinline__ void epi_linear_frag_impl(const DevProb &P, const Acc &acc, int frow0, int fcol0, int lane,
                                                     int row0, int col0) {
    const int M = P.M, N = P.N, gn0 = col0 + fcol0 + F::col(lane);
    float b0[NC], b1[NC], b2[NC];
    bool cok[NC];
    const bool h0 = P.bias0 != nullptr, h1 = P.bias1 != nullptr, h2 = P.bias2 != nullptr;
    const bool f_acc = FEAT && P.accumulate, f_pre = FEAT && P.C_pre != nullptr, f_mask = FEAT && P.mask != nullptr;
    [[maybe_unused]] bool bad = false;
#pragma unroll
    for (int j = 0; j < NC; ++j) {
        const int gn = gn0 + j * F::CW;
        cok[j] = !EDGE || gn < N;
        b0[j] = (h0 && cok[j]) ? P.bias0[gn] : 0.f;
        b1[j] = (h1 && cok[j]) ? P.bias1[gn] : 0.f;
        b2[j] = (h2 && cok[j]) ? P.bias2[gn] : 0.f;
    }
#pragma unroll
    for (int e = 0; e < F::NR; ++e) {
        const int gm = row0 + frow0 + F::row(e, lane);
        if (EDGE && gm >= M) continue;
        float *crow = P.C + (long long)gm * P.ldc + gn0;
        float prev[NC];
        if (f_acc) {
#pragma unroll
            for (int j = 0; j < NC; ++j) prev[j] = (!EDGE || cok[j]) ? crow[j * F::CW] : 0.f;
        }
#pragma unroll
// ... 503 lines not shown
    ISC_GATE_RETURN(L);
    f32_dma_tile_body<F32TileMD, EPI_LINEAR>(L);
}

__device__ __forceinline__ int h3_lstm_wrow_in_gate(int t) { return 2 * (t & 15) + ((t >> 4) & 1); }

__device__ __forceinline__ void epi_lstm_frag16(const DevProb &P, f32x4 (&acc)[2][8], int frow0, int lane, int row0,
                                                int tn) {
    const int H = P.H, u0 = tn * 32 + 2 * (lane & 15);
    const bool has_b = P.bias0 != nullptr, has_pre = P.pre != nullptr, has_tab = P.tab != nullptr;
    float2 b[4];
    if (has_b) {
#pragma unroll
        for (int k = 0; k < 4; ++k) {
            const float2 x = *reinterpret_cast<const float2 *>(P.bias0 + k * H + u0);
            const float2 y = *reinterpret_cast<const float2 *>(P.bias1 + k * H + u0);
            b[k] = make_float2(x.x + y.x, x.y + y.y);
        }
    }
#pragma unroll
    for (int i = 0; i < 2; ++i) {
        int gm[4];
        bool ok[4];
        long long tok[4];
        float2 cp[4], q[4][4], t[4][4];
#pragma unroll
        for (int r = 0; r < 4; ++r) {
            gm[r] = row0 + frow0 + i * 16 + 4 * (lane >> 4) + r;
            ok[r] = gm[r] < P.M;
        }
        if (has_tab) {
#pragma unroll
            for (int r = 0; r < 4; ++r) tok[r] = ok[r] ? P.tab_ids[(long long)gm[r] * P.tab_ids_stride] : 0;
        }
#pragma unroll
        for (int r = 0; r < 4; ++r)
            cp[r] = ok[r] ? *reinterpret_cast<const float2 *>(P.c_prev + (long long)gm[r] * H + u0) : make_float2(0.f, 0.f);
        if (has_pre && P.pre_div > 1) {
#pragma unroll
            for (int r = 0; r < 4; ++r) {
                const long long pm = ok[r] ? (unsigned)gm[r] / (unsigned)P.pre_div : 0;
#pragma unroll
                for (int k = 0; k < 4; ++k)
                    q[r][k] = ok[r] ? *reinterpret_cast<const float2 *>(P.pre + pm * 4 * H + k * H + u0)
                                    : make_float2(0.f, 0.f);
            }
        } else if (has_pre) {
#pragma unroll
            for (int r = 0; r < 4; ++r)
#pragma unroll
                for (int k = 0; k < 4; ++k)
                    q[r][k] = ok[r] ? *reinterpret_cast<const float2 *>(P.pre + (long long)gm[r] * 4 * H + k * H + u0)
                                    : make_float2(0.f, 0.f);
        }
        if (has_tab) {
#pragma unroll
            for (int r = 0; r < 4; ++r)
#pragma unroll
                for (int k = 0; k < 4; ++k)
                    t[r][k] = ok[r] ? *reinterpret_cast<const float2 *>(P.tab + tok[r] * 4 * H + k * H + u0)
                                    : make_float2(0.f, 0.f);
        }
#pragma unroll
        for (int r = 0; r < 4; ++r) {
            float h2[2], c2[2], ga[2][4];
#pragma unroll
            for (int hf = 0; hf < 2; ++hf) {
                float g[4];
#pragma unroll
                for (int k = 0; k < 4; ++k) {
                    g[k] = acc[i][2 * k + hf][r];
                    if (has_b) g[k] += hf ? b[k].y : b[k].x;
                    if (has_pre) g[k] += hf ? q[r][k].y : q[r][k].x;
                    if (has_tab) g[k] += hf ? t[r][k].y : t[r][k].x;
                }
                const float gi = isc_sigmoid(g[0]), gf = isc_sigmoid(g[1]), gg = isc_tanh(g[2]), go = isc_sigmoid(g[3]);
                c2[hf] = gf * (hf ? cp[r].y : cp[r].x) + gi * gg;
                h2[hf] = go * isc_tanh(c2[hf]);
                ga[hf][0] = gi; ga[hf][1] = gf; ga[hf][2] = gg; ga[hf][3] = go;
            }
            if (ok[r]) {
                const long long o = (long long)gm[r] * H + u0;
                *reinterpret_cast<float2 *>(P.c_out + o) = make_float2(c2[0], c2[1]);
                *reinterpret_cast<float2 *>(P.h_out + o) = make_float2(h2[0], h2[1]);
                if (P.h_hi) {
                    typedef _Float16 h2v __attribute__((ext_vector_type(2)));
                    _Float16 a0, a1, l0, l1;
                    isc_split_f16(h2[0], a0, l0);
                    isc_split_f16(h2[1], a1, l1);
                    const long long po = plane_index(gm[r], u0, H);
                    h2v hi = {a0, a1};
                    h2v lo = {l0, l1};
                    *reinterpret_cast<h2v *>(P.h_hi + po) = hi;
                    *reinterpret_cast<h2v *>(P.h_lo + po) = lo;
                }
                if (P.hmask) {
                    const uint8_t m0 = P.hmask[o], m1 = P.hmask[o + 1];
                    *reinterpret_cast<float2 *>(P.hdrop + o) =
                        make_float2(h2[0] * (float)m0 * P.mask_scale, h2[1] * (float)m1 * P.mask_scale);
                }
                if (P.gates_out) {
                    float *go_ = P.gates_out + (long long)gm[r] * 4 * H + u0;
#pragma unroll
                    for (int k = 0; k < 4; ++k)
                        *reinterpret_cast<float2 *>(go_ + k * H) = make_float2(ga[0][k], ga[1][k]);
                }
            }
        }
    }
}

template <int NB, bool CHECK>
__device__ __forceinline__ void epi_slab_frag16(const DevProb &P, f32x4 (&acc)[2][NB], int frow0, int lane, int row0, int col0,
                                                int ks) {
    float *base = P.slab + (long long)ks * P.slab_stride;
    bool bad = false;
#pragma unroll
    for (int e = 0; e < Frag16::NR; ++e) {
        const int gm = row0 + frow0 + Frag16::row(e, lane);
        if (gm >= P.M) continue;
#pragma unroll
        for (int j = 0; j < NB; ++j) {
            const int gn = col0 + j * Frag16::CW + Frag16::col(lane);
            if (gn >= P.N) continue;
            const float o = Frag16::get(acc, e, j);
            if constexpr (CHECK) bad |= !(fabsf(o) <= 3.0e38f);
            base[(long long)gm * P.N + gn] = o;
        }
    }
    if constexpr (CHECK) {
        if (__any(bad) && lane == 0) isc_flag_gemm(ISC_STATUS_WORD_LINEAR);
    }
}

typedef _Float16 h8 __attribute__((ext_vector_type(8)));

__device__ __forceinline__ void h3_frag_from_f32(const char *row, int oct, int sw, h8 &hi, h8 &lo) {
    const float4 v0 = *reinterpret_cast<const float4 *>(row + (((2 * oct) ^ sw) * 16));
    const float4 v1 = *reinterpret_cast<const float4 *>(row + (((2 * oct + 1) ^ sw) * 16));
    const float x[8] = {v0.x, v0.y, v0.z, v0.w, v1.x, v1.y, v1.z, v1.w};
#pragma unroll
    for (int e = 0; e < 8; ++e) {
        _Float16 h, l;
        isc_split_f16(x[e], h, l);
        hi[e] = h;
        lo[e] = l;
    }
}

#ifndef H3_STAMP
#define H3_STAMP 0
#endif
#if H3_STAMP
#define H3_STAMP_AT(v) const unsigned long long v = __builtin_amdgcn_s_memtime()
__device__ unsigned long long g_h3_stamp[16];
extern "C" int isc_debug_h3_stamps(unsigned long long *out16_host, int reset) {
    if (out16_host && hipMemcpyFromSymbol(out16_host, HIP_SYMBOL(g_h3_stamp), sizeof(g_h3_stamp)) != hipSuccess) return 1;
    if (reset) {
        const unsigned long long z[16] = {};
        if (hipMemcpyToSymbol(HIP_SYMBOL(g_h3_stamp), z, sizeof(z)) != hipSuccess) return 1;
    }
    return ISC_OK;
}
#else
#define H3_STAMP_AT(v)
#endif

// ... 684 lines not shown
    for (int i = 0; i < AHEAD; ++i)
        if (i < nblk) issue(i, i);
    int st = 0;
    for (int b = 0; b < nblk; ++b) {
        const int younger = nblk - 1 - b < AHEAD - 1 ? nblk - 1 - b : AHEAD - 1;
        if (younger >= 3) asm volatile("s_waitcnt vmcnt(15)" ::: "memory");
        else if (younger == 2) asm volatile("s_waitcnt vmcnt(10)" ::: "memory");
        else if (younger == 1) asm volatile("s_waitcnt vmcnt(5)" ::: "memory");
        else asm volatile("s_waitcnt vmcnt(0)" ::: "memory");
        __syncthreads();
        if (b + AHEAD < nblk) issue(b + AHEAD, st == 0 ? H3V_STAGES - 1 : st - 1);
        const char *ia = lds + st * H3V_STAGE_BYTES + fr * 128;
        const char *iw = ia + 4096 + wave * 4096;
        h8 a1[2], a2[2], b1[2], b2[2];
        h3s_read_frags(ia, iw, af32, fh, fsw, a1, a2, b1, b2);
#pragma unroll
        for (int kk = 0; kk < 2; ++kk) {
            acc0 = __builtin_amdgcn_mfma_f32_32x32x16_f16(a1[kk], b1[kk], acc0, 0, 0, 0);
            acc1 = __builtin_amdgcn_mfma_f32_32x32x16_f16(a1[kk], b2[kk], acc1, 0, 0, 0);
            acc1 = __builtin_amdgcn_mfma_f32_32x32x16_f16(a2[kk], b1[kk], acc1, 0, 0, 0);
        }
        st = st == H3V_STAGES - 1 ? 0 : st + 1;
    }
#pragma unroll
    for (int r = 0; r < 16; ++r) acc0[r] = fmaf(acc1[r], ISC_SPLIT_LO_WEIGHT, acc0[r]);
    __syncthreads();
    f32x16 accv[1] = {acc0};
    epi_vocab_frag<Frag32, 1, 4, BM>(P, accv, 0, wave * 32, wave, lane, row0, col0, tn, smem);
    __syncthreads();
    h3s_vocab_combine<BM>(P, smem, tid, row0, tn);
}

__global__ __launch_bounds__(256) void splitk_linear_kernel(const DevLaunch L) {
    ISC_GATE_RETURN(L);
    rows_kernarg_warm<ROWS_KERNARG_LINES(DevLaunch)>();
    const DevProb &P = L.p[blockIdx.y];
    const long long n4 = (long long)P.M * (P.N >> 2);
    const long long i = (long long)blockIdx.x * 256 + threadIdx.x;
    if (i >= n4) return;
    const int N = P.N, gm = (int)(i / (N >> 2)), gn = (int)(i % (N >> 2)) * 4;
    const float *sl = P.slab + (long long)gm * N + gn;
    float4 part[16];
    const int S = P.ksplit;
#pragma unroll
    for (int s = 0; s < 16; ++s)
        part[s] = s < S ? *reinterpret_cast<const float4 *>(sl + (long long)s * P.slab_stride)
                        : make_float4(0.f, 0.f, 0.f, 0.f);
    float4 v = part[0];
#pragma unroll
    for (int s = 1; s < 16; ++s) { v.x += part[s].x; v.y += part[s].y; v.z += part[s].z; v.w += part[s].w; }
    float o[4] = {v.x, v.y, v.z, v.w};
    epi_linear_finish<4>(P, gm, gn, o);
}

__global__ __launch_bounds__(256) __attribute__((amdgpu_waves_per_eu(6))) void splitk_lstm_kernel(const DevLaunch L) {
    ISC_GATE_RETURN(L);
    const DevProb &P = L.p[0];
    const int H = P.H;
    const long long i = (long long)blockIdx.x * 256 + threadIdx.x;
    if (i >= (long long)P.M * H) return;
    const int gm = (int)(i / H), unit = (int)(i % H);
    float part[4][16];
    const int S = P.ksplit;
#pragma unroll
    for (int k = 0; k < 4; ++k) {
        const float *sl = P.slab + (long long)gm * 4 * H + k * H + unit;
#pragma unroll
        for (int s = 0; s < 16; ++s) part[k][s] = s < S ? sl[(long long)s * P.slab_stride] : 0.f;
    }
    const int gma[1] = {gm};
    const bool ok[1] = {true};
    float g[1][4];
#pragma unroll
    for (int k = 0; k < 4; ++k) {
        float a = part[k][0];
#pragma unroll
        for (int s = 1; s < 16; ++s) a += part[k][s];
        g[0][k] = a;
    }
    asm volatile("" : "+v"(g[0][0]), "+v"(g[0][1]), "+v"(g[0][2]), "+v"(g[0][3]));
    lstm_cells<1>(P, gma, unit, ok, g);
}

__device__ __forceinline__ void wave_vocab_tile128(const DevProb &P, int gm, int tn, const float (&v)[2], int lane) {
    float x[2];
    int col[2];
#pragma unroll
    for (int h = 0; h < 2; ++h) {
        col[h] = tn * 128 + lane + 64 * h;
        const bool ok = col[h] < P.N;
        x[h] = ok ? v[h] + P.bias0[col[h]] : -INFINITY;
        if (ok && P.C) P.C[(long long)gm * P.ld_logits + col[h]] = x[h];
    }
    float mx = x[0];
    int ix = col[0];
    if (x[1] > mx) { mx = x[1]; ix = col[1]; }
    wave_argmax(mx, ix);
    float sm = (x[0] > -INFINITY ? __expf(x[0] - mx) : 0.f) + (x[1] > -INFINITY ? __expf(x[1] - mx) : 0.f);
    sm = wave_sum(sm);
    if (lane == 0) {
        const long long o = (long long)gm * P.ntile_total + tn;
        P.pmax[o] = mx;
        P.psum[o] = sm;
        P.pidx[o] = ix;
    }
}

__global__ __launch_bounds__(256) void splitk_vocab_kernel(const DevLaunch L) {
    ISC_GATE_RETURN(L);
    const DevProb &P = L.p[0];
    const int lane = threadIdx.x & 63;
    const long long w = (long long)blockIdx.x * 4 + (threadIdx.x >> 6);
    const int n_tile = P.ntile_total;
    if (w >= (long long)P.M * n_tile) return;
    const int gm = (int)(w / n_tile), tn = (int)(w % n_tile);
    const int N = P.N, S = P.ksplit;
    float v[2];
#pragma unroll
    for (int h = 0; h < 2; ++h) {
        const int col = tn * 128 + lane + 64 * h;
        const bool ok = col < N;
        const float *sl = P.slab + (long long)gm * N + (ok ? col : 0);
        float part[16];
#pragma unroll
        for (int s = 0; s < 16; ++s) part[s] = (ok && s < S) ? sl[(long long)s * P.slab_stride] : 0.f;
        float a = part[0];
#pragma unroll
        for (int s = 1; s < 16; ++s) a += part[s];
        v[h] = a;
    }
    wave_vocab_tile128(P, gm, tn, v, lane);
}

#define GEMV_MAX_ROWS 8
#define GEMV_MAX_K 4096
template <int HALF, int MASK, int NV>
__device__ __forceinline__ void wave_reduce_scatter_step(float (&v)[NV], int lane) {
    const bool up = (lane & MASK) != 0;
#pragma unroll
    for (int i = 0; i < HALF; ++i) {
        const float send = up ? v[i] : v[i + HALF];
        const float keep = up ? v[i + HALF] : v[i];
        v[i] = keep + __shfl_xor(send, MASK, 64);
    }
    if constexpr (HALF > 1) wave_reduce_scatter_step<HALF / 2, MASK / 2, NV>(v, lane);
}
template <int NV>
__device__ __forceinline__ void wave_reduce_scatter(float (&v)[NV], int lane) {
    static_assert(NV == 32 || NV == 64, "4 or 8 weight rows x 8 activation rows");
    wave_reduce_scatter_step<NV / 2, 32, NV>(v, lane);
    if (NV == 32) v[0] += __shfl_xor(v[0], 1, 64);
}

template <int NR, int CB>
__device__ __forceinline__ void gemv_batch(const float *Wb, const long long (&wrow)[NR], long long ldw, int Ks, int c0,
                                           const float *Ak, int Ktot, int lane, float (&acc)[NR * GEMV_MAX_ROWS]) {
    constexpr int MR = GEMV_MAX_ROWS;
    float4 w[NR][CB];
    int kc[CB];
    bool in[CB];
#pragma unroll
    for (int c = 0; c < CB; ++c) {
        const int kk = c0 + c * 256 + lane * 4;
        in[c] = kk < Ks;
        kc[c] = in[c] ? kk : Ks - 4;
    }
// ... 77 lines not shown
                for (int m = 0; m < MR; ++m)
                    v[m] = *reinterpret_cast<const float4 *>(Ab + (long long)(m < M ? m : M - 1) * lda + k4 * 4);
#pragma unroll
                for (int m = 0; m < MR; ++m) {
                    if (m >= M) v[m] = make_float4(0.f, 0.f, 0.f, 0.f);
                    *reinterpret_cast<float4 *>(As + (long long)m * Ktot + koff + k4 * 4) = v[m];
                }
            }
            koff += Ks;
        }
    }
    __syncthreads();

    if constexpr (EPI == EPI_VOCAB) {
        const int col0 = tile * 128;
        for (int rnd = 0; rnd < 2; ++rnd) {
            long long wrow[8];
#pragma unroll
            for (int r = 0; r < 8; ++r) {
                const int c = col0 + wave * 16 + rnd * 8 + r;
                wrow[r] = c < N ? c : N - 1;
            }
            float acc[8 * MR];
            gemv_accumulate<2, 2>(P, wrow, As, Ktot, lane, 0, nchunk, acc);
            wave_reduce_scatter<64>(acc, lane);
            red[(lane & 7) * 128 + wave * 16 + rnd * 8 + (lane >> 3)] = acc[0];
        }
        __syncthreads();
        for (int m = wave; m < M; m += NW) {
            const float v[2] = {red[m * 128 + lane], red[m * 128 + lane + 64]};
            wave_vocab_tile128(P, m, tile, v, lane);
        }
    } else {
        const int KS = P.ksplit;
        const int qpw = NW / KS;
        const int qw = wave / KS, ks = wave - qw * KS;
        const int quad = tile * qpw + qw;
        long long wrow[4];
        bool live;
        if constexpr (EPI == EPI_LSTM) {
            live = quad < P.H;
#pragma unroll
            for (int r = 0; r < 4; ++r) wrow[r] = (long long)r * P.H + (live ? quad : 0);
        } else {
            live = quad * 4 < N;
#pragma unroll
            for (int r = 0; r < 4; ++r) { const int c = quad * 4 + r; wrow[r] = c < N ? c : N - 1; }
        }
        float acc[4 * MR];
        gemv_accumulate<1, 8>(P, wrow, As, Ktot, lane, nchunk * ks / KS, nchunk * (ks + 1) / KS, acc);
        wave_reduce_scatter<32>(acc, lane);
        if ((lane & 1) == 0) red[wave * 32 + (lane >> 1)] = acc[0];
        __syncthreads();
        if (ks == 0 && live) {
            const float *rq = red + wave * 32;
            if constexpr (EPI == EPI_LSTM) {
                if (lane < M) {
                    const int gm[1] = {lane};
                    const bool ok[1] = {true};
                    float g[1][4];
#pragma unroll
                    for (int k = 0; k < 4; ++k) {
                        float v = rq[k * MR + lane];
                        for (int j = 1; j < KS; ++j) v += rq[j * 32 + k * MR + lane];
                        g[0][k] = v;
                    }
                    lstm_cells<1>(P, gm, quad, ok, g);
                }
            } else {
                const int m = lane >> 2, e = lane & 3, n = quad * 4 + e;
                if (lane < 4 * MR && m < M && n < N) {
                    float o[1] = {rq[e * MR + m]};
                    for (int j = 1; j < KS; ++j) o[0] += rq[j * 32 + e * MR + m];
                    epi_linear_finish<1>(P, m, n, o);
                }
            }
        }
    }
}

static int check_segs(const isc_seg *seg, int nseg) {
    if (nseg < 1 || nseg > ISC_MAX_SEG) return ISC_E_SHAPE;
    for (int s = 0; s < nseg; ++s) {
        if (!seg[s].A || !seg[s].W) return ISC_E_NULL;
        if (seg[s].K <= 0 || (seg[s].K % BK) != 0) return ISC_E_SHAPE;
        if ((seg[s].lda & 3) || (seg[s].ldw & 3)) return ISC_E_ALIGN;
        if (!isc_aligned16(seg[s].A) || !isc_aligned16(seg[s].W)) return ISC_E_ALIGN;
    }
    return ISC_OK;
}

static void copy_segs(DevProb &d, const isc_seg *seg, int nseg) {
    d.nseg = nseg;
    for (int s = 0; s < nseg; ++s) {
        d.seg[s].A = seg[s].A; d.seg[s].W = seg[s].W;
        d.seg[s].lda = seg[s].lda; d.seg[s].ldw = seg[s].ldw; d.seg[s].K = seg[s].K; d.seg[s].a_f16 = seg[s].a_f16;
        d.seg[s].A_hi = static_cast<const _Float16 *>(seg[s].A_hi);
        d.seg[s].A_lo = static_cast<const _Float16 *>(seg[s].A_lo);
    }
}

static bool segs_any_f16(const isc_seg *seg, int nseg) {
    for (int s = 0; s < nseg && s < ISC_MAX_SEG; ++s)
        if (seg[s].a_f16) return true;
    return false;
}

template <class K>
static int lds_attr_once(std::atomic<bool> &done, size_t bytes, K k0, K k1 = nullptr) {
    if (bytes <= 65536 || done.load()) return ISC_OK;
    for (K k : {k0, k1}) {
        if (!k) continue;
        hipError_t e = hipFuncSetAttribute(reinterpret_cast<const void *>(k), hipFuncAttributeMaxDynamicSharedMemorySize,
                                           (int)bytes);
        if (e != hipSuccess) return (int)e;
    }
    done.store(true);
    return ISC_OK;
}

enum { F32_KIND_XL = 3, F32_KIND_LD = 4, F32_KIND_MD = 5, F32_KIND_REDUCE = 6, F32_KINDS = 7 };
static std::atomic<long long> g_f32_launches[F32_KINDS];
extern "C" long long isc_f32_launches(int kind) {
    return kind >= 0 && kind < F32_KINDS ? g_f32_launches[kind].load() : -1;
}

template <int WM, int WN, int TN, int EPI, bool AKM, bool BKM>
static int launch_cfg(const DevLaunch &L, hipStream_t st) {
    constexpr int BM = 32 * WM, BN = 32 * TN * WN;
    constexpr size_t k_bytes = (size_t)2 * (Tile<BM, AKM>::SIZE + Tile<BN, BKM>::SIZE) * sizeof(float);
    constexpr size_t c_bytes = (size_t)BM * (BN + 4) * sizeof(float);
    constexpr size_t lds = k_bytes > c_bytes ? k_bytes : c_bytes;
    static std::atomic<bool> attr_set{false};
    if (int rc = lds_attr_once(attr_set, lds, &gemm_kernel<WM, WN, TN, EPI, AKM, BKM>)) return rc;
    hipLaunchKernelGGL((gemm_kernel<WM, WN, TN, EPI, AKM, BKM>), dim3(L.total_tiles), dim3(256), lds, st, L);
    ++g_f32_launches[WM == 4 ? 0 : (WM == 2 ? 1 : 2)];
    ISC_LAUNCH_CHECK();
    return ISC_OK;
}

template <class G, int EPI>
static constexpr auto f32_dma_kernel() {
    if constexpr (std::is_same_v<G, F32TileXL>) return &gemm_xl_kernel<EPI>;
    else if constexpr (std::is_same_v<G, F32TileLD>) return &gemm_ld_kernel<EPI>;
    else return &gemm_md_kernel;
}

template <class G, int EPI>
static int launch_f32_dma(const DevLaunch &L, hipStream_t st) {
    static_assert(EPI == EPI_LINEAR || !std::is_same_v<G, F32TileMD>, "the 64-row kernel has the linear epilogue only");
    constexpr size_t lds = G::LDS_BYTES;
    constexpr auto kernel = f32_dma_kernel<G, EPI>();
    static std::atomic<bool> attr_set{false};
    if (int rc = lds_attr_once(attr_set, lds, kernel)) return rc;
    hipLaunchKernelGGL(kernel, dim3(L.total_tiles), dim3(G::THREADS), lds, st, L);
    ++g_f32_launches[std::is_same_v<G, F32TileXL> ? F32_KIND_XL : (std::is_same_v<G, F32TileLD> ? F32_KIND_LD : F32_KIND_MD)];
    ISC_LAUNCH_CHECK();
    return ISC_OK;
}

static const int kTileBM[5] = {128, F32TileMD::BM, 32, F32TileXL::BM, F32TileLD::BM};

static std::atomic<int> g_md_enabled{1};

template <int EPI, bool AKM, bool BKM>
static int launch_any(const DevLaunch &L, int tile, hipStream_t st) {
    if constexpr (EPI == EPI_LINEAR && !AKM && !BKM) {
// ... 762 lines not shown
        const long long Kp = h3_kp(p);
        bool ok = true;
        for (int s = 0; s < p.nseg; ++s) ok = ok && (p.seg[s].K & 31) == 0;
        if (contraction_flops(p) < H3_TN_MIN_FLOPS && mode != 2) ok = false;
        const long long per_k = (long long)p.M + p.N;
        chunk[i] = Kp;
        if (ok && per_k * Kp + 1024 > ws_floats) {
            chunk[i] = ((ws_floats - 1024) / per_k) & ~31LL;
            if (chunk[i] < 512) ok = false;
        }
        if (ok) take |= 1u << i;
    }
    if (L.nprob >= 2 && take == (1u << L.nprob) - 1u) {
        bool same = true;
        long long n_sum = 0;
        const DevProb &p0 = L.p[0];
        for (int i = 0; i < L.nprob; ++i) {
            const DevProb &p = L.p[i];
            same = same && p.nseg == 1 && p.seg[0].A == p0.seg[0].A && p.seg[0].lda == p0.seg[0].lda &&
                   p.seg[0].K == p0.seg[0].K && p.M == p0.M &&
                   (long long)((p.M + 127) / 128) * ((p.N + 127) / 128) < H3_MIN_TILES / 2;
            n_sum += p.N;
        }
        const long long K = p0.nseg == 1 ? p0.seg[0].K : 0;
        const long long per_k = (long long)p0.M + n_sum;
        const long long kc_max = ((ws_floats - 1024LL * (L.nprob + 1)) / (per_k > 0 ? per_k : 1)) & ~31LL;
        if (same && K > 0 && kc_max >= 2048) {
            const long long nchunk = (K + kc_max - 1) / kc_max;
            const long long kc0 = ((K + nchunk - 1) / nchunk + 31) & ~31LL;
            rc = tn_run_chunks(L, K, kc0, false, ws, mode, true, st);
            return take;
        }
    }
    for (int i = 0; i < L.nprob; ++i) {
        if (!(take & (1u << i))) continue;
        const DevProb &pfull = L.p[i];
        const bool by_seg = pfull.nseg > 1 && chunk[i] < h3_kp(pfull);
        const int npass = by_seg ? pfull.nseg : 1;
        for (int pass = 0; pass < npass; ++pass) {
            DevLaunch L1 = {};
            L1.nprob = 1;
            L1.p[0] = pfull;
            if (by_seg) {
                L1.p[0].nseg = 1;
                L1.p[0].seg[0] = pfull.seg[pass];
            }
            rc = tn_run_chunks(L1, h3_kp(L1.p[0]), chunk[i], pass > 0, ws, mode, false, st);
            if (rc) return take;
        }
    }
    return take;
}

static int plan_splitk(DevLaunch &L, float *ws, long long ws_floats) {
    if (!ws || ws_floats <= 0) return 1;
    const long long blocks = count_tiles(L, 32, 128);
    long long need1 = 0;
    int min_chunks = 1 << 30;
    for (int i = 0; i < L.nprob; ++i) {
        const DevProb &p = L.p[i];
        if (p.N & 3) return 1;
        need1 += (long long)p.M * p.N;
        int ch = 0;
        for (int s = 0; s < p.nseg; ++s) ch += (p.seg[s].K + BK - 1) / BK;
        if (ch < min_chunks) min_chunks = ch;
    }
    if (blocks >= 384) return 1;
    long long S = 768 / blocks;
    if (S > 16) S = 16;
    if (S > min_chunks / 4) S = min_chunks / 4;
    if (S > ws_floats / need1) S = ws_floats / need1;
    if (S < 2) return 1;
    float *at = ws;
    for (int i = 0; i < L.nprob; ++i) {
        DevProb &p = L.p[i];
        p.ksplit = (int)S;
        p.slab = at;
        p.slab_stride = (long long)p.M * p.N;
        at += S * p.slab_stride;
    }
    return (int)S;
}

template <int EPI>
static int route_nt(DevLaunch &L, float *ws, long long ws_floats, hipStream_t st, bool allow_xl, bool decide_only) {
    if (const int kmax = gemv_plan<EPI>(L)) return decide_only ? 0 : gemv_run<EPI>(L, kmax, st);
    const H3sPlan hs = h3s_plan<EPI>(L, ws, ws_floats, st, 0);
    if (hs.T) return decide_only ? 0 : h3s_run<EPI>(L, hs, ws, ws_floats, st, 0);
    if (plan_splitk(L, ws, ws_floats) > 1) {
        if (decide_only) return 0;
        finish_tiling(L, 2);
        const int rc = launch_any<EPI_LINEAR, false, false>(L, 2, st);
        return rc ? rc : launch_splitk_reduce<EPI>(L, st);
    }
    const H3Plan h = h3_plan<EPI>(L, ws, ws_floats, st, 0);
    if (h.take) return decide_only ? 1 : h3_run<EPI>(L, h, ws, st, 0);
    if (decide_only) return 0;
    const int tile = pick_tile(L, allow_xl, true, true);
    finish_tiling(L, tile);
    return launch_any<EPI, false, false>(L, tile, st);
}

static int linear_fwd_run(const isc_linear_problem *pr, int n_prob, void *stream, bool decide_only) {
    if (!pr) return ISC_E_NULL;
    if (n_prob < 1 || n_prob > 3) return ISC_E_SHAPE;
    DevLaunch L = {};
    L.nprob = n_prob;
    L.gate = isc_stream_gate_(stream);
    for (int i = 0; i < n_prob; ++i) {
        const isc_linear_problem &q = pr[i];
        int rc = check_segs(q.seg, q.nseg);
        if (rc) return rc;
        if (!q.C) return ISC_E_NULL;
        if (q.M <= 0 || q.N <= 0) return ISC_E_SHAPE;
        if (q.keep_mask && q.ldc != q.N) return ISC_E_SHAPE;
        DevProb &d = L.p[i];
        copy_segs(d, q.seg, q.nseg);
        d.M = q.M; d.N = q.N; d.relu = q.relu;
        d.bias0 = q.bias0; d.bias1 = q.bias1; d.bias2 = q.bias2;
        d.mask = q.keep_mask; d.mask_scale = q.mask_scale;
        d.ldc = q.ldc; d.C = q.C; d.C_pre = q.C_pre; d.accumulate = q.accumulate;
    }
    return route_nt<EPI_LINEAR>(L, pr[0].splitk_ws, pr[0].splitk_ws_floats, (hipStream_t)stream, true, decide_only);
}

static bool f16_segs_aligned(const isc_linear_problem *pr, int n_prob) {
    for (int i = 0; i < n_prob; ++i)
        for (int s = 0; s < pr[i].nseg && s < ISC_MAX_SEG; ++s)
            if (pr[i].seg[s].a_f16 && ((pr[i].seg[s].lda & 7) || !isc_aligned16(pr[i].seg[s].A))) return false;
    return true;
}

extern "C" int isc_linear_f16_native(const isc_linear_problem *pr, int n_prob, void *stream) {
    if (!pr || n_prob < 1 || n_prob > 3 || !f16_segs_aligned(pr, n_prob)) return 0;
    return linear_fwd_run(pr, n_prob, stream, true) == 1 ? 1 : 0;
}

extern "C" int isc_linear_fwd(const isc_linear_problem *pr, int n_prob, void *stream) {
    bool any16 = false;
    for (int i = 0; pr && i < n_prob && i < 3; ++i) any16 = any16 || segs_any_f16(pr[i].seg, pr[i].nseg);
    if (any16) {
        if (!f16_segs_aligned(pr, n_prob)) return ISC_E_ALIGN;
        const int native = linear_fwd_run(pr, n_prob, stream, true);
        if (native != 1) return native < 0 ? native : ISC_E_SHAPE;
    }
    return linear_fwd_run(pr, n_prob, stream, false);
}

#define H3_NN_MIN_FLOPS 5.0e9

static int gemm_bwd_run(const isc_linear_problem *pr, int n_prob, int layout, hipStream_t st) {
    DevLaunch L = {};
    L.nprob = n_prob;
    bool k32 = true;
    for (int i = 0; i < n_prob; ++i) {
        const isc_linear_problem &q = pr[i];
        if (q.nseg < 1 || q.nseg > ISC_MAX_SEG || !q.C) return q.C ? ISC_E_SHAPE : ISC_E_NULL;
        if (q.M <= 0 || q.N <= 0 || (q.N & 3) || (q.ldc & 3)) return ISC_E_SHAPE;
        if (layout == ISC_LAYOUT_TN && (q.M & 3)) return ISC_E_SHAPE;
        for (int s = 0; s < q.nseg; ++s) {
            const isc_seg &g = q.seg[s];
            if (!g.A || !g.W) return ISC_E_NULL;
            if (g.K <= 0) return ISC_E_SHAPE;
            if ((g.lda & 3) || (g.ldw & 3) || !isc_aligned16(g.A) || !isc_aligned16(g.W)) return ISC_E_ALIGN;
            k32 = k32 && (g.K & 31) == 0;
        }
        DevProb &d = L.p[i];
        copy_segs(d, q.seg, q.nseg);
        d.M = q.M; d.N = q.N; d.relu = 0;
        d.bias0 = q.bias0; d.bias1 = q.bias1; d.bias2 = q.bias2;
        d.ldc = q.ldc; d.C = q.C; d.accumulate = q.accumulate;
    }
    float *ws = pr[0].splitk_ws;
    const long long ws_floats = pr[0].splitk_ws_floats;
    const int mode = g_h3_mode.load();
    const bool nn_big = mode == 1 && n_prob == 1 && contraction_flops(pr[0]) >= H3_NN_MIN_FLOPS;
    if (layout == ISC_LAYOUT_NN && k32 && (h3w_scope_of(st) || mode >= 2 || nn_big)) {
        const H3sPlan hs = h3s_plan<EPI_LINEAR>(L, ws, ws_floats, st, 1);
        if (hs.T) return h3s_run<EPI_LINEAR>(L, hs, ws, ws_floats, st, 1);
        const H3Plan h = h3_plan<EPI_LINEAR>(L, ws, ws_floats, st, 1);
        if (h.take) return h3_run<EPI_LINEAR>(L, h, ws, st, 1);
    }
    if (layout == ISC_LAYOUT_TN) {
        int rc_h3 = ISC_OK;
        const unsigned took = try_h3_tn(L, ws, ws_floats, st, rc_h3);
        if (rc_h3) return rc_h3;
        if (took) {
            int n = 0;
            for (int i = 0; i < L.nprob; ++i)
                if (!(took & (1u << i))) { if (n != i) L.p[n] = L.p[i]; ++n; }
            if (n == 0) return ISC_OK;
            L.nprob = n;
        }
    }
    const int S = plan_splitk(L, ws, ws_floats);
    const int tile = S > 1 ? 2 : pick_tile(L, false, false);
    finish_tiling(L, tile);
    int rc = layout == ISC_LAYOUT_NN ? launch_any<EPI_LINEAR, false, true>(L, tile, st)
                                     : launch_any<EPI_LINEAR, true, true>(L, tile, st);
    if (rc || S == 1) return rc;
    return launch_splitk_linear_reduce(L, st);
}

extern "C" int isc_gemm_bwd(const isc_linear_problem *pr, int n_prob, int layout, void *stream) {
    if (!pr) return ISC_E_NULL;
    if (n_prob < 1 || n_prob > 3 || (layout != ISC_LAYOUT_NN && layout != ISC_LAYOUT_TN)) return ISC_E_SHAPE;
    for (int i = 0; i < n_prob; ++i)
        if (segs_any_f16(pr[i].seg, pr[i].nseg)) return ISC_E_SHAPE;
    if (layout == ISC_LAYOUT_TN && n_prob == 1 && pr[0].nseg > 1 && pr[0].nseg <= ISC_MAX_SEG && g_h3_mode.load() != 0) {
        isc_linear_problem a = pr[0], b = pr[0];
        a.nseg = b.nseg = 0;
        for (int s = 0; s < pr[0].nseg; ++s) {
            isc_linear_problem &to = pr[0].seg[s].K > 0 && (pr[0].seg[s].K & 31) == 0 ? a : b;
            to.seg[to.nseg++] = pr[0].seg[s];
        }
        if (a.nseg > 0 && b.nseg > 0 && contraction_flops(a) >= H3_TN_MIN_FLOPS) {
            const int rc = gemm_bwd_run(&a, 1, layout, (hipStream_t)stream);
            if (rc) return rc;
            b.accumulate = 1; b.bias0 = b.bias1 = b.bias2 = nullptr;
            return gemm_bwd_run(&b, 1, layout, (hipStream_t)stream);
        }
    }
    return gemm_bwd_run(pr, n_prob, layout, (hipStream_t)stream);
}

extern "C" int isc_lstm_fwd(const isc_lstm_problem *q, void *stream) {
    if (!q) return ISC_E_NULL;
    int rc = check_segs(q->seg, q->nseg);
    if (rc) return rc;
    if (segs_any_f16(q->seg, q->nseg)) return ISC_E_SHAPE;
    if (!q->c_prev || !q->h_out || !q->c_out) return ISC_E_NULL;
    if ((!q->b_ih || !q->b_hh) && !q->pre) return ISC_E_NULL;
    if ((q->b_ih == nullptr) != (q->b_hh == nullptr)) return ISC_E_NULL;
    if (q->tab && !q->tab_ids) return ISC_E_NULL;
    if (q->M <= 0 || q->H <= 0 || (q->H % 32) != 0) return ISC_E_SHAPE;
    if (q->h_keep_mask && !q->hdrop_out) return ISC_E_NULL;
    if (q->pre_div > 1 && (!q->pre || q->M % q->pre_div)) return ISC_E_SHAPE;
    DevLaunch L = {};
    L.nprob = 1;
    L.gate = isc_stream_gate_(stream);
    DevProb &d = L.p[0];
    copy_segs(d, q->seg, q->nseg);
    d.M = q->M; d.N = 4 * q->H; d.H = q->H;
    d.bias0 = q->b_ih; d.bias1 = q->b_hh;
    d.c_prev = q->c_prev; d.h_out = q->h_out; d.c_out = q->c_out; d.gates_out = q->gates_out;
    d.hmask = q->h_keep_mask; d.mask_scale = q->mask_scale; d.hdrop = q->hdrop_out;
    if ((q->h_hi == nullptr) != (q->h_lo == nullptr)) return ISC_E_NULL;
    d.h_hi = static_cast<_Float16 *>(q->h_hi); d.h_lo = static_cast<_Float16 *>(q->h_lo);
    d.pre = q->pre; d.tab = q->tab; d.tab_ids = q->tab_ids; d.tab_ids_stride = q->tab_ids_stride;
    d.pre_div = q->pre_div > 1 ? q->pre_div : 1;
    return route_nt<EPI_LSTM>(L, q->splitk_ws, q->splitk_ws_floats, (hipStream_t)stream, !q->pre && !q->tab, false);
}

extern "C" int isc_vocab_fwd(const float *h, int ldh, const float *W, int ldw, const float *bias,
                             int M, int V, int K, float *logits, int64_t ld_logits,
                             float *part_max, float *part_sum, int32_t *part_idx,
                             const void *h_hi, const void *h_lo,
                             float *splitk_ws, int64_t splitk_ws_floats, void *stream) {
    if (!h || !W || !bias || !part_max || !part_sum || !part_idx) return ISC_E_NULL;
    isc_seg sg = {h, W, ldh, ldw, K, 0, h_hi, h_lo};
    int rc = check_segs(&sg, 1);
    if (rc) return rc;
    if (M <= 0 || V <= 0) return ISC_E_SHAPE;
    DevLaunch L = {};
    L.nprob = 1;
    L.gate = isc_stream_gate_(stream);
    DevProb &d = L.p[0];
    copy_segs(d, &sg, 1);
    d.M = M; d.N = V; d.bias0 = bias;
    d.C = logits; d.ld_logits = ld_logits;
    d.pmax = part_max; d.psum = part_sum; d.pidx = part_idx;
    d.ntile_total = (V + 127) / 128;
    return route_nt<EPI_VOCAB>(L, splitk_ws, splitk_ws_floats, (hipStream_t)stream, false, false);
}
```

insenticap_model_amd/csrc/rows.hip:

```cpp
#include <atomic>

#include "common.h"

#define ROWS_MAX 8
#define ROWS_FIN_MAX 4
#define ROWS_MAX_SLICE 12
#define ROWS_KC 8
#if ROWS_STAMP
RSTAMP_SETTER(isc_rows_set_stamp)
#endif

struct RSlice {
    const float *A;
    const float *W;
    int lda, ldw, klen, indirect;
};
struct RSeg {
    const float *A, *W;
    int lda, ldw, K, indirect;
};
struct RSegs {
    RSeg s[3];
    int nseg, nslice, cut_shift, pad;
};
// ... 993 lines not shown
    }
    hipLaunchKernelGGL(rows_scan_gate_kernel, dim3(rows), dim3(1024), lds, st, a);
    ISC_LAUNCH_CHECK();
    ++g_rows_launches;
    return ISC_OK;
}

static int rows_scan_gate(const isc_step_plan *p, int row_div, const int *skip, hipStream_t st) {
    RScanArgs a = {};
    a.row_div = row_div > 1 ? row_div : 1; a.skip = skip;
    a.P[0] = p->att_p; a.V[0] = p->att_e; a.G[0] = p->gate_Gc; a.q[0] = p->qa; a.w[0] = p->w_alpha_c; a.wb[0] = p->b_alpha_c;
    a.P[1] = p->words_p; a.V[1] = p->words_e; a.G[1] = p->gate_Gs; a.q[1] = p->qw; a.w[1] = p->w_alpha_s; a.wb[1] = p->b_alpha_s;
    a.q2 = p->label_w;
    a.ids = reinterpret_cast<const long long *>(p->words_ids); a.ids_ld = p->words_ids_ld;
    a.R[0] = p->R; a.R[1] = p->Mw; a.A = p->A;
    a.zh = p->z; a.b_c = p->b_gc; a.b_s = p->b_gs; a.w_g = p->w_gate; a.b_g = p->b_gate;
    a.f = p->f; a.alpha[0] = p->alpha_c; a.alpha[1] = p->alpha_s; a.beta = p->beta;
    a.alpha_ld[0] = p->alpha_c_ld; a.alpha_ld[1] = p->alpha_s_ld; a.beta_ld = p->beta_ld;
    return rows_scan_gate_launch(a, p->rows, st);
}

#define ROWS_SCAN_MAX_ROWS 256
static std::atomic<int> g_rows_scan_max{ROWS_SCAN_MAX_ROWS};
extern "C" int isc_set_rows_scan_max(int rows) {
    if (rows < 0) return g_rows_scan_max.load();
    return g_rows_scan_max.exchange(rows);
}

static std::atomic<int> g_rows_scan_regions{256};
extern "C" int isc_set_rows_scan_regions(int regions) {
    if (regions < 0) return g_rows_scan_regions.load();
    return g_rows_scan_regions.exchange(regions);
}

int rows_scan_gate_try(const isc_scan_gate_args *g, int rows, hipStream_t st, int *rc) {
    const isc_scan_problem &c = g->scan[0], &s = g->scan[1];
    if (rows > g_rows_scan_max.load()) return 0;
    if (c.out || s.out || c.out_hi || s.out_hi || c.q2 || c.row_ids) return 0;
    if (c.A != c.D || s.A != c.A || s.D != c.A || c.A > 512 || (c.A & 3) || c.R < 1 || s.R < 1) return 0;
    if (c.R > g_rows_scan_regions.load() || s.R > RS_NWS * RS_RPW) return 0;
    if (!c.P || !c.V || !c.q || !c.w || !s.P || !s.V || !s.q || !s.w || !g->G[0] || !g->G[1]) return 0;
    RScanArgs a = {};
    a.row_div = 1;
    a.skip = isc_stream_gate_(st);
    a.P[0] = c.P; a.V[0] = c.V; a.G[0] = g->G[0]; a.q[0] = c.q; a.w[0] = c.w; a.wb[0] = c.w_bias;
    a.P[1] = s.P; a.V[1] = s.V; a.G[1] = g->G[1]; a.q[1] = s.q; a.w[1] = s.w; a.wb[1] = s.w_bias;
    a.q2 = s.q2;
    a.ids = reinterpret_cast<const long long *>(s.row_ids); a.ids_ld = s.row_ids_ld;
    a.R[0] = c.R; a.R[1] = s.R; a.A = c.A;
    a.zh = g->zh; a.b_c = g->b_gc; a.b_s = g->b_gs; a.w_g = g->w_gate; a.b_g = g->b_gate;
    a.f = g->f; a.alpha[0] = c.alpha_out; a.alpha[1] = s.alpha_out; a.beta = g->beta;
    a.alpha_ld[0] = c.alpha_ld; a.alpha_ld[1] = s.alpha_ld; a.beta_ld = g->beta_ld;
    a.f_hi = static_cast<_Float16 *>(g->f_hi); a.f_lo = static_cast<_Float16 *>(g->f_lo);
    *rc = rows_scan_gate_launch(a, rows, st);
    return 1;
}

extern "C" int isc_rows_step_supported(const isc_step_plan *p) {
    if (!p) return 0;
    if (p->rows < 1 || p->rows > ROWS_MAX) return 0;
    if (!rows_scan_ok(p)) return 0;
    if (p->g1 || p->g2 || p->out_mask || p->apply_logsoftmax || p->pair_rows_c) return 0;
    {
        const int tw = isc_rows_stats_tile(p->V);
        if (tw <= 0 || (p->V + tw - 1) / tw > 256) return 0;
    }
    if ((p->H & 3) || (p->E & 3) || (p->W & 3) || (p->A & 3)) return 0;
    const int s1 = (p->H + 255) / 256 * 2 + (p->tab ? 0 : (p->W + 255) / 256);
    const int s2 = (p->E + 255) / 256 + (p->H + 255) / 256 * 2;
    if (s1 > ROWS_MAX_SLICE || s2 > ROWS_MAX_SLICE || (p->H + 255) / 256 > ROWS_MAX_SLICE) return 0;
    return 1;
}

#define RET(x)                 \
    do {                       \
        int rc__ = (x);        \
        if (rc__) return rc__; \
    } while (0)

extern "C" int isc_rows_step_fwd(const isc_step_plan *p, const isc_rows_ext *x, void *stream) {
    if (!p || !x) return ISC_E_NULL;
    if (!isc_rows_step_supported(p)) return ISC_E_SHAPE;
    if (!p->pmax || !p->psum || !p->pidx) return ISC_E_NULL;
    hipStream_t st = (hipStream_t)stream;
    const int rows = p->rows, H = p->H, E = p->E, A = p->A, W = p->W, V = p->V;
    const int ld1 = H + E + W, ld2 = E + H;
    const int64_t *src = x->src_row;
    const int row_div = x->row_div > 1 ? x->row_div : 1;
    const int *skip = x->live_in;
    if (rows % row_div) return ISC_E_SHAPE;
    {
        const float *As[3], *Ws[3];
        int lda[3], ldw[3], K[3], ind[3], n = 0;
        As[n] = p->h2_prev; lda[n] = H; Ws[n] = p->Wih1; ldw[n] = ld1; K[n] = H; ind[n] = 1; ++n;
        if (!p->tab) { As[n] = p->xt; lda[n] = W; Ws[n] = p->Wih1 + H + E; ldw[n] = ld1; K[n] = W; ind[n] = 0; ++n; }
        As[n] = p->h1_prev; lda[n] = H; Ws[n] = p->Whh1; ldw[n] = H; K[n] = H; ind[n] = 1; ++n;
        RLstmArgs::Fin fin = {};
        const isc_rollout_step *f = x->fin_prev;
        if (f) {
            if (!p->tab || row_div != 1 || src || skip || rows > ROWS_FIN_MAX) return ISC_E_SHAPE;
            if (f->forced || f->sample_u || f->xt_next) return ISC_E_SHAPE;
            if (!f->part_max || !f->part_sum || !f->part_idx || !f->seq || !f->seq_logprobs || !f->seq_masks ||
                !f->unfinished || !f->alive || !x->fin_unfinished_out)
                return ISC_E_NULL;
            if (f->B != rows || f->T <= 0 || f->t < 0 || f->t + 1 >= f->T || f->n_tile <= 0) return ISC_E_SHAPE;
            fin.pmax = f->part_max; fin.psum = f->part_sum; fin.pidx = f->part_idx;
            fin.n_tile = f->n_tile; fin.T = f->T; fin.t = f->t; fin.eos = f->eos_id;
            fin.seq = reinterpret_cast<long long *>(f->seq); fin.raw = reinterpret_cast<long long *>(f->raw_tokens);
            fin.lp = f->seq_logprobs; fin.masks = f->seq_masks;
            fin.unf_in = f->unfinished; fin.unf_out = x->fin_unfinished_out; fin.alive = f->alive;
        }
        RET(rows_lstm(As, lda, Ws, ldw, K, ind, n, rows, H, src, p->c1_prev, p->h1, p->c1, nullptr, nullptr, p->pre1,
                      p->tab, p->tok, p->tok_stride, row_div, skip, st, f ? &fin : nullptr));
    }
    {
        const float *Ws[3] = {p->W_h2att, p->W_h2word, p->W_gh}, *bs[3] = {p->b_h2att, p->b_h2word, p->b_gh};
        float *Cs[3] = {p->qa, p->qw, p->z};
        const int N[3] = {A, A, A}, ldc[3] = {A, A, A};
        RET(rows_linear3(p->h1, H, H, rows, Ws, bs, Cs, N, ldc, 3, skip, st));
    }
    RET(rows_scan_gate(p, row_div, skip, st));
    {
        const float *As[3] = {p->f, p->h1, p->h2_prev}, *Ws[3] = {p->Wih2, p->Wih2 + E, p->Whh2};
        const int lda[3] = {E, H, H}, ldw[3] = {ld2, ld2, H}, K[3] = {E, H, H}, ind[3] = {0, 0, 1};
        RET(rows_lstm(As, lda, Ws, ldw, K, ind, 3, rows, H, src, p->c2_prev, p->h2, p->c2, p->b_ih2, p->b_hh2, nullptr,
                      nullptr, nullptr, 0, 1, skip, st));
    }
    RET(rows_vocab(p->h2, H, p->W_cls, H, p->b_cls, rows, V, H, x->stats_tile, p->pmax, p->psum, p->pidx, p->logits,
                   p->ld_logits, x, st));
    return ISC_OK;
}

extern "C" int isc_rows_vocab_fwd(const float *h, int ldh, const float *W, int ldw, const float *bias, int M, int V,
                                  int K, float *part_max, float *part_sum, int32_t *part_idx, float *logits,
                                  int64_t ld_logits, const isc_rows_ext *ext, void *stream) {
    if (!ext) return ISC_E_NULL;
    return rows_vocab(h, ldh, W, ldw, bias, M, V, K, ext->stats_tile, part_max, part_sum, part_idx, logits, ld_logits,
                      ext, (hipStream_t)stream);
}
```

insenticap_model_amd/csrc/step.hip:

```cpp
#include "common.h"
#include <atomic>

static inline isc_seg seg(const float *A, int lda, const float *W, int ldw, int K, const void *hi = nullptr,
                          const void *lo = nullptr) {
    isc_seg s = {A, W, lda, ldw, K, 0, hi, lo};
    return s;
}

#define RET(x)            \
    do {                  \
        int rc__ = (x);   \
        if (rc__) return rc__; \
    } while (0)

extern "C" int isc_step_fwd(const isc_step_plan *p, void *stream) {
    if (!p) return ISC_E_NULL;
    const int rows = p->rows, H = p->H, E = p->E, A = p->A, W = p->W, V = p->V;
    if (rows <= 0 || H <= 0) return ISC_E_SHAPE;
    const bool has_c = p->att_e != nullptr, has_s = p->words_e != nullptr;
    if (!has_c && !has_s) return ISC_E_NULL;
    const bool pair = p->pair_rows_c > 0;
    if (p->pair_rows_c < 0 || (pair && (!has_c || !has_s || p->pair_rows_c >= rows))) return ISC_E_SHAPE;
    const bool gate = has_c && has_s && !pair;
    const int rows_c = pair ? p->pair_rows_c : rows, rows_s = pair ? rows - p->pair_rows_c : rows;
    const long long off_s = pair ? p->pair_rows_c : 0;
    if (pair && (p->s != p->v + off_s * E || p->gate_Gc || p->gate_Gs)) return ISC_E_SHAPE;
    const int row_div = p->row_div > 1 ? p->row_div : 1;
    if (row_div > 1 && (rows % row_div || pair || p->gate_Gc || p->gate_Gs)) return ISC_E_SHAPE;
    const int ld1 = H + E + W, ld2 = E + H;
    const bool planes = p->h1_prev_hi && p->h1_prev_lo && p->h2_prev_hi && p->h2_prev_lo && p->h1_hi && p->h1_lo &&
                        p->h2_hi && p->h2_lo;
    if (!planes && (p->h1_prev_hi || p->h1_prev_lo || p->h2_prev_hi || p->h2_prev_lo || p->h1_hi || p->h1_lo ||
                    p->h2_hi || p->h2_lo))
        return ISC_E_NULL;
    if (pair && planes) return ISC_E_SHAPE;
#define PL(x) (planes ? (x) : nullptr)
    const bool wplanes = planes && (!has_c || (p->v_hi && p->v_lo)) && (!has_s || (p->s_hi && p->s_lo)) &&
                         (!gate || (p->f_hi && p->f_lo));
#define PW(x) (wplanes ? (x) : nullptr)

    {
        isc_lstm_problem l = {};
        int n = 0;
        l.seg[n++] = seg(p->h2_prev, H, p->Wih1, ld1, H, PL(p->h2_prev_hi), PL(p->h2_prev_lo));
        if (!p->tab) l.seg[n++] = seg(p->xt, W, p->Wih1 + H + E, ld1, W);
        l.seg[n++] = seg(p->h1_prev, H, p->Whh1, H, H, PL(p->h1_prev_hi), PL(p->h1_prev_lo));
        l.nseg = n; l.M = rows; l.H = H;
        l.h_hi = PL(p->h1_hi); l.h_lo = PL(p->h1_lo);
        l.c_prev = p->c1_prev; l.h_out = p->h1; l.c_out = p->c1; l.gates_out = p->g1;
        l.pre = p->pre1; l.tab = p->tab; l.tab_ids = p->tok; l.tab_ids_stride = p->tok_stride;
        l.pre_div = p->pre_rows ? 1 : row_div;
        l.splitk_ws = p->splitk_ws; l.splitk_ws_floats = p->splitk_ws_floats;
        RET(isc_lstm_fwd(&l, stream));
    }
    {
        isc_linear_problem q[3] = {};
        int n = 0;
        auto lin = [&](const float *Wm, const float *b, float *out, long long row0, int M) {
            isc_linear_problem &x = q[n++];
            x.seg[0] = seg(p->h1 + row0 * H, H, Wm, H, H, row0 ? nullptr : PL(p->h1_hi), row0 ? nullptr : PL(p->h1_lo));
            x.nseg = 1; x.M = M; x.N = A; x.bias0 = b; x.ldc = A; x.C = out;
        };
        if (has_c) lin(p->W_h2att, p->b_h2att, p->qa, 0, rows_c);
        if (has_s) lin(p->W_h2word, p->b_h2word, p->qw, off_s, rows_s);
        if (gate) lin(p->W_gh, p->b_gh, p->z, 0, rows);
        q[0].splitk_ws = p->splitk_ws; q[0].splitk_ws_floats = p->splitk_ws_floats;
        RET(isc_linear_fwd(q, n, stream));
    }
    const bool fused_gate = gate && p->gate_Gc && p->gate_Gs;
    {
        isc_scan_problem sc[2] = {};
        int n = 0;
        if (has_c) {
            isc_scan_problem &x = sc[n++];
            x.P = p->att_p; x.V = p->att_e; x.q = p->qa; x.w = p->w_alpha_c; x.w_bias = p->b_alpha_c;
            x.R = p->R; x.A = A; x.D = E; x.out = p->v; x.alpha_out = p->alpha_c; x.alpha_ld = p->alpha_c_ld;
            x.out_hi = PW(p->v_hi); x.out_lo = PW(p->v_lo);
            x.rows = rows_c; x.row_div = row_div;
        }
        if (has_s) {
            isc_scan_problem &x = sc[n++];
            x.P = p->words_p; x.V = p->words_e; x.q = p->qw; x.q2 = p->label_w; x.w = p->w_alpha_s;
            x.w_bias = p->b_alpha_s; x.R = p->Mw; x.A = A; x.D = W; x.out = p->s; x.alpha_out = p->alpha_s;
            x.alpha_ld = p->alpha_s_ld;
            x.out_hi = PW(p->s_hi); x.out_lo = PW(p->s_lo);
            x.row_ids = p->words_ids; x.row_ids_ld = p->words_ids_ld;
            x.rows = rows_s; x.row_div = row_div;
        }
        if (fused_gate) {
            isc_scan_gate_args g = {};
            g.scan[0] = sc[0]; g.scan[1] = sc[1];
            g.scan[0].out = nullptr; g.scan[0].out_hi = g.scan[0].out_lo = nullptr;
            g.scan[1].out = nullptr; g.scan[1].out_hi = g.scan[1].out_lo = nullptr;
            g.G[0] = p->gate_Gc; g.G[1] = p->gate_Gs;
            g.zh = p->z; g.b_gc = p->b_gc; g.b_gs = p->b_gs; g.w_gate = p->w_gate; g.b_gate = p->b_gate;
            g.f = p->f; g.f_hi = PW(p->f_hi); g.f_lo = PW(p->f_lo); g.beta = p->beta; g.beta_ld = p->beta_ld;
            RET(isc_attn_scan_gate_fwd(&g, rows, stream));
        } else {
            RET(isc_attn_scan_fwd(sc, n, rows, stream));
        }
    }
    const float *feat = has_c ? p->v : p->s;
    const void *feat_hi = has_c ? PW(p->v_hi) : PW(p->s_hi), *feat_lo = has_c ? PW(p->v_lo) : PW(p->s_lo);
    if (fused_gate) {
        feat = p->f; feat_hi = PW(p->f_hi); feat_lo = PW(p->f_lo);
    } else if (gate) {
        isc_linear_problem x = {};
        x.seg[0] = seg(p->v, E, p->W_gc, E, E, PW(p->v_hi), PW(p->v_lo));
        x.seg[1] = seg(p->s, W, p->W_gs, W, W, PW(p->s_hi), PW(p->s_lo));
        x.nseg = 2; x.M = rows; x.N = A; x.bias0 = p->b_gc; x.bias1 = p->b_gs; x.ldc = A; x.C = p->z;
        x.accumulate = 1;
        x.splitk_ws = p->splitk_ws; x.splitk_ws_floats = p->splitk_ws_floats;
        RET(isc_linear_fwd(&x, 1, stream));
        RET(isc_gate_mix_fwd(p->z, p->w_gate, p->b_gate, p->v, p->s, rows, A, E, p->f, p->beta, p->beta_ld,
                             PW(p->f_hi), PW(p->f_lo), stream));
        feat = p->f; feat_hi = PW(p->f_hi); feat_lo = PW(p->f_lo);
    }
    {
        isc_lstm_problem l = {};
        l.seg[0] = seg(feat, E, p->Wih2, ld2, E, feat_hi, feat_lo);
        l.seg[1] = seg(p->h1, H, p->Wih2 + E, ld2, H, PL(p->h1_hi), PL(p->h1_lo));
        l.seg[2] = seg(p->h2_prev, H, p->Whh2, H, H, PL(p->h2_prev_hi), PL(p->h2_prev_lo));
        l.nseg = 3; l.M = rows; l.H = H; l.b_ih = p->b_ih2; l.b_hh = p->b_hh2;
        l.h_hi = PL(p->h2_hi); l.h_lo = PL(p->h2_lo);
        l.c_prev = p->c2_prev; l.h_out = p->h2; l.c_out = p->c2; l.gates_out = p->g2;
        l.h_keep_mask = p->out_mask; l.mask_scale = p->out_scale; l.hdrop_out = p->hdrop;
        l.splitk_ws = p->splitk_ws; l.splitk_ws_floats = p->splitk_ws_floats;
        RET(isc_lstm_fwd(&l, stream));
    }
    if (p->pmax)
    RET(isc_vocab_fwd(p->out_mask ? p->hdrop : p->h2, H, p->W_cls, H, p->b_cls, rows, V, H, p->logits,
                      p->ld_logits, p->pmax, p->psum, p->pidx, p->out_mask ? nullptr : PL(p->h2_hi),
                      p->out_mask ? nullptr : PL(p->h2_lo), p->splitk_ws, p->splitk_ws_floats, stream));
#undef PL
#undef PW
    if (p->apply_logsoftmax) {
        if (!p->logits || !p->pmax) return ISC_E_NULL;
        RET(isc_logsoftmax_apply(p->logits, p->ld_logits, rows, V, p->pmax, p->psum, nullptr, stream));
    }
    return ISC_OK;
}

static inline isc_linear_problem nn_problem(const float *A, int lda, const float *Wm, int ldw, int K, int M,
                                            int N, float *C, int accumulate) {
    isc_linear_problem x = {};
    x.seg[0] = seg(A, lda, Wm, ldw, K);
    x.nseg = 1; x.M = M; x.N = N; x.ldc = N; x.C = C; x.accumulate = accumulate;
    return x;
}

extern "C" int isc_step_bwd(const isc_step_bwd_plan *p, void *stream) {
    if (!p) return ISC_E_NULL;
    const int rows = p->rows, H = p->H, E = p->E, A = p->A, W = p->W;
    const bool has_c = p->att_e != nullptr, has_s = p->words_e != nullptr;
    const bool pair = p->pair_rows_c > 0;
    if (p->pair_rows_c < 0 || (pair && (!has_c || !has_s || p->pair_rows_c >= rows))) return ISC_E_SHAPE;
    const bool gate = has_c && has_s && !pair;
    const int rows_c = pair ? p->pair_rows_c : rows, rows_s = pair ? rows - p->pair_rows_c : rows;
    const long long off_s = pair ? p->pair_rows_c : 0;
    const int ld1 = H + E + W, ld2 = E + H, G = 4 * H;
    const int acc = p->first ? 0 : 1;
    const int row_div = p->row_div > 1 ? p->row_div : 1;
    if (row_div > 1 && (rows % row_div || pair)) return ISC_E_SHAPE;

    RET(isc_lstm_bwd(p->dhd, p->first ? nullptr : p->dh2_rec, p->first ? nullptr : p->dc2_in, p->g2,
                     p->c2_prev, p->c2, rows, H, p->dG2, p->dc2_out, nullptr, stream));
    {
        isc_linear_problem q[3] = {nn_problem(p->dG2, G, p->Wih2, ld2, G, rows, E, p->d_feat, 0),
                                   nn_problem(p->dG2, G, p->Wih2 + E, ld2, G, rows, H, p->dh1, 0),
                                   nn_problem(p->dG2, G, p->Whh2, H, G, rows, H, p->dh2_rec, 0)};
        q[0].splitk_ws = p->splitk_ws; q[0].splitk_ws_floats = p->splitk_ws_floats;
        RET(isc_gemm_bwd(q, 3, ISC_LAYOUT_NN, stream));
    }
    const float *dv = p->d_feat, *dsw = p->d_feat + off_s * E;
    if (gate) {
        RET(isc_gate_mix_bwd(p->z, p->w_gate, p->v, p->s, p->beta, p->beta_ld, p->d_feat, rows, A, E, p->dv,
                             p->ds, p->dz, p->dwg_rows, p->dbg_rows, acc, stream));
        isc_linear_problem q[3] = {nn_problem(p->dz, A, p->W_gc, E, A, rows, E, p->dv, 1),
                                   nn_problem(p->dz, A, p->W_gs, W, A, rows, W, p->ds, 1),
                                   nn_problem(p->dz, A, p->W_gh, H, A, rows, H, p->dh1, 1)};
        q[0].splitk_ws = p->splitk_ws; q[0].splitk_ws_floats = p->splitk_ws_floats;
        RET(isc_gemm_bwd(q, 3, ISC_LAYOUT_NN, stream));
        dv = p->dv;
        dsw = p->ds;
    }
    {
        isc_scan_bwd_problem sc[2] = {};
        int n = 0;
        if (has_c) {
            isc_scan_bwd_problem &x = sc[n++];
            x.P = p->att_p; x.V = p->att_e; x.q = p->qa; x.w = p->w_alpha_c; x.alpha = p->alpha_c;
            x.alpha_ld = p->alpha_c_ld; x.dout = dv; x.R = p->R; x.A = A; x.D = E; x.accumulate = acc;
            x.dP = p->dP_att; x.dV = p->dV_att; x.dq = p->dqa; x.dw_rows = p->dwc_rows; x.de_out = p->de_c;
            x.rows = rows_c; x.row_div = row_div;
        }
        if (has_s) {
            isc_scan_bwd_problem &x = sc[n++];
            x.P = p->words_p; x.V = p->words_e; x.q = p->qw; x.q2 = p->label_w; x.w = p->w_alpha_s;
            x.alpha = p->alpha_s; x.alpha_ld = p->alpha_s_ld; x.dout = dsw; x.R = p->Mw; x.A = A; x.D = W;
            x.accumulate = acc; x.dP = p->dP_w; x.dV = p->dV_w; x.dq = p->dqw; x.dw_rows = p->dws_rows; x.de_out = p->de_s;
            x.rows = rows_s; x.row_div = row_div;
        }
        RET(isc_attn_scan_bwd(sc, n, rows, stream));
    }
    if (pair) {
        isc_linear_problem q[2] = {nn_problem(p->dqa, A, p->W_h2att, H, A, rows_c, H, p->dh1, 1),
                                   nn_problem(p->dqw, A, p->W_h2word, H, A, rows_s, H, p->dh1 + off_s * H, 1)};
        q[0].splitk_ws = p->splitk_ws; q[0].splitk_ws_floats = p->splitk_ws_floats;
        RET(isc_gemm_bwd(q, 2, ISC_LAYOUT_NN, stream));
    } else {
        isc_linear_problem x = {};
        int n = 0;
        if (has_c) x.seg[n++] = seg(p->dqa, A, p->W_h2att, H, A);
        if (has_s) x.seg[n++] = seg(p->dqw, A, p->W_h2word, H, A);
        x.nseg = n; x.M = rows; x.N = H; x.ldc = H; x.C = p->dh1; x.accumulate = 1;
        x.splitk_ws = p->splitk_ws; x.splitk_ws_floats = p->splitk_ws_floats;
        RET(isc_gemm_bwd(&x, 1, ISC_LAYOUT_NN, stream));
    }
    RET(isc_lstm_bwd(p->dh1, p->first ? nullptr : p->dh1_rec, p->first ? nullptr : p->dc1_in, p->g1,
                     p->c1_prev, p->c1, rows, H, p->dG1, p->dc1_out, p->dG1_sum, stream));
    if (!p->last) {
        isc_linear_problem q[2] = {nn_problem(p->dG1, G, p->Wih1, ld1, G, rows, H, p->dh2_rec, 1),
                                   nn_problem(p->dG1, G, p->Whh1, H, G, rows, H, p->dh1_rec, 0)};
        q[0].splitk_ws = p->splitk_ws; q[0].splitk_ws_floats = p->splitk_ws_floats;
// ... 66 lines not shown
```

insenticap_model_amd/ops.py:

```python
import ctypes as C
import gc
import threading
import time

import torch

from . import _lib
from ._lib import LinearProblem, LstmProblem, RolloutStep, ScanProblem, check


def stream():
    return C.c_void_p(torch.cuda.current_stream().cuda_stream)


class KernelTimer:

    def __init__(self):
        self.armed = False
        self.arm_step = None
        self.phase = 'step'
        self.records = []

    def begin(self):
        if not self.armed:
# ... 324 lines not shown
            if self.wkey is not None and exc[0] is None:
                _lib.load().isc_h3_weights_suspend(C.c_void_p(self.key[1]))
            else:
                _lib.load().isc_h3_weights_end(C.c_void_p(self.key[1]))
        return False


def linear_problem(segs, out, bias0=None, bias1=None, bias2=None, relu=False, keep_mask=None, mask_scale=1.0,
                   out_pre=None, accumulate=False):
    p = LinearProblem()
    _fill_segs(p.seg, segs)
    p.f16_segs = [(i, sg[0]) for i, sg in enumerate(segs) if sg[0].dtype == torch.float16]
    p.nseg = len(segs)
    p.M, p.N = out.shape
    assert segs[0][0].shape[0] == p.M and segs[0][1].shape[0] == p.N
    assert out.stride(1) == 1
    p.relu = int(relu)
    p.bias0, p.bias1, p.bias2 = ptr(bias0), ptr(bias1), ptr(bias2)
    p.keep_mask = ptr(keep_mask)
    p.mask_scale = mask_scale
    p.ldc = out.stride(0)
    p.C = out.data_ptr()
    p.C_pre = ptr(out_pre)
    p.accumulate = int(accumulate)
    if out_pre is not None:
        assert out_pre.stride(0) == out.stride(0)
    return p


def f16_to_f32(x, out=None):
    assert x.dtype == torch.float16 and x.dim() == 2 and x.stride(1) == 1
    if out is None:
        out = torch.empty(x.shape, dtype=torch.float32, device=x.device)
    if x.numel():
        check(_lib.load().isc_f16_to_f32(x.data_ptr(), x.stride(0), out.data_ptr(), out.stride(0), x.shape[0],
                                         x.shape[1], stream()), 'isc_f16_to_f32')
    return out


def f16_convert_launches():
    return _lib.load().isc_f16_convert_launches()


def h3_f16a_launches():
    return _lib.load().isc_h3_f16a_launches()


def f32_launches(kind):
    return _lib.load().isc_f32_launches(int(kind))


H3_KINDS = 17


def h3_kernel_launches(kind):
    return _lib.load().isc_h3_kernel_launches(int(kind))


def linear_fwd(problems):
    lib = _lib.load()
    _attach_ws(problems[0], torch.cuda.current_device())
    arr = (LinearProblem * len(problems))(*problems)
    if any(getattr(q, 'f16_segs', None) for q in problems) and \
            not lib.isc_linear_f16_native(arr, len(problems), stream()):
        for q in problems:
            for i, A in getattr(q, 'f16_segs', None) or ():
                A32 = f16_to_f32(A)
                q.keep = getattr(q, 'keep', []) + [A32]
                q.seg[i].A, q.seg[i].lda, q.seg[i].a_f16 = A32.data_ptr(), A32.stride(0), 0
            q.f16_segs = []
        arr = (LinearProblem * len(problems))(*problems)
    e0 = TIMER.begin()
    check(lib.isc_linear_fwd(arr, len(problems), stream()), 'isc_linear_fwd')
    if e0 is not None:
        fl = sum(2.0 * q.M * q.N * sum(q.seg[i].K for i in range(q.nseg)) for q in problems)
        TIMER.end(e0, 'linear[' + '+'.join('%dx%dx%d' % (q.M, q.N, sum(q.seg[i].K for i in range(q.nseg)))
                                          for q in problems) + ']', fl)


def lstm_fwd(segs, b_ih, b_hh, c_prev, h_out, c_out, gates_out=None, h_keep_mask=None,
             mask_scale=1.0, hdrop_out=None, pre=None, tab=None, tab_ids=None, h_planes=None, pre_div=1, ws=None):
    lib = _lib.load()
    p = LstmProblem()
    _fill_segs(p.seg, segs)
    p.nseg = len(segs)
    p.M, p.H = c_prev.shape
    assert c_prev.is_contiguous() and h_out.is_contiguous() and c_out.is_contiguous()
    p.b_ih, p.b_hh = ptr(b_ih), ptr(b_hh)
    if pre is not None:
        pre_div = max(int(pre_div), 1)
        assert pre.is_contiguous() and p.M % pre_div == 0 and pre.shape == (p.M // pre_div, 4 * p.H)
        p.pre, p.pre_div = pre.data_ptr(), pre_div
    if tab is not None:
        assert tab.is_contiguous() and tab.shape[1] == 4 * p.H and tab_ids.dtype == torch.int64
        p.tab, p.tab_ids, p.tab_ids_stride = tab.data_ptr(), tab_ids.data_ptr(), tab_ids.stride(0)
    p.c_prev, p.h_out, p.c_out = c_prev.data_ptr(), h_out.data_ptr(), c_out.data_ptr()
    p.gates_out = ptr(gates_out)
    p.h_keep_mask = ptr(h_keep_mask)
    p.mask_scale = mask_scale
    p.hdrop_out = ptr(hdrop_out)
    if h_planes is not None:
        assert h_planes.dtype == torch.float16 and h_planes.is_contiguous() and h_planes.shape == (2, p.M, p.H)
        p.h_hi, p.h_lo = planes_ptrs(h_planes)
    if ws is not None:
        assert ws.dtype == torch.float32 and ws.is_contiguous()
        p.splitk_ws, p.splitk_ws_floats = ws.data_ptr(), ws.numel()
    _attach_ws(p, c_prev.device)
    e0 = TIMER.begin()
    check(lib.isc_lstm_fwd(C.byref(p), stream()), 'isc_lstm_fwd')
    if e0 is not None:
        k = _seg_k(segs)
        TIMER.end(e0, 'lstm[%dx%dx%d]' % (p.M, 4 * p.H, k), 2.0 * p.M * 4 * p.H * k)


def step_fwd(plan):
    check(_lib.load().isc_step_fwd(C.byref(plan), stream()), 'isc_step_fwd')


class stream_gate:

    def __init__(self, ptr):
        self.ptr = int(ptr) if ptr else 0
        self.st = None

    def __enter__(self):
        if self.ptr:
            self.st = stream()
            check(_lib.load().isc_set_stream_gate(C.c_void_p(self.ptr), self.st), 'isc_set_stream_gate')
        return self

    def __exit__(self, et, ev, tb):
        if self.st is not None:
            _lib.load().isc_set_stream_gate(None, self.st)
            self.st = None
        return False


def rows_stats_tile(V):
    return _lib.load().isc_rows_stats_tile(int(V))


def set_rows_scan_max(rows):
    return _lib.load().isc_set_rows_scan_max(int(rows))


def copy_multi(dsts, srcs):
    pairs = [(d, s) for d, s in zip(dsts, srcs) if d is not None and d.numel()]
    for d, s in pairs:
        if d.dtype != s.dtype or d.shape != s.shape or not (d.is_contiguous() and s.is_contiguous() and d.is_cuda and s.is_cuda):
            raise ValueError('copy_multi: contiguous device tensors of equal shape and dtype expected')
    lib = _lib.load()
    for i in range(0, len(pairs), 8):
        grp = pairs[i:i + 8]
        n = len(grp)
        D = (C.c_void_p * n)(*[d.data_ptr() for d, _ in grp])
        S = (C.c_void_p * n)(*[s.data_ptr() for _, s in grp])
        Bn = (C.c_int64 * n)(*[d.numel() * d.element_size() for d, _ in grp])
        check(lib.isc_copy_multi(D, S, Bn, n, stream()), 'isc_copy_multi')


def stage_inputs(dsts, srcs):
    pairs = [(d, s) for d, s in zip(dsts, srcs) if d is not None]
    if all(d.dtype == s.dtype and d.shape == s.shape and s.is_cuda and s.is_contiguous() and d.is_contiguous()
           for d, s in pairs):
        copy_multi([d for d, _ in pairs], [s for _, s in pairs])
        return
    by_dtype = {}
    for d, s in pairs:
        by_dtype.setdefault(d.dtype, ([], []))
        by_dtype[d.dtype][0].append(d)
        by_dtype[d.dtype][1].append(s)
    for ds, ss in by_dtype.values():
        torch._foreach_copy_(ds, ss, non_blocking=True)


def set_h3v(on):
    return _lib.load().isc_set_h3v(int(on))


def set_h3_vocab_tile(rows):
    rows = int(rows)
    if rows not in (0, 128, 256):
        raise ValueError('set_h3_vocab_tile: 0 (auto), 128 or 256, got %r' % rows)
    return _lib.load().isc_set_h3_vocab_tile(rows)


def rows_step_supported(plan):
    return bool(_lib.load().isc_rows_step_supported(C.byref(plan)))


def rows_step_fwd(plan, ext):
    check(_lib.load().isc_rows_step_fwd(C.byref(plan), C.byref(ext), stream()), 'isc_rows_step_fwd')


def rows_vocab_fwd(h, W, bias, part_max, part_sum, part_idx, ext, logits=None):
    lib = _lib.load()
    M, K = h.shape
    V = W.shape[0]
    assert h.stride(1) == 1 and W.stride(1) == 1
# ... 45 lines not shown
    assert logits_btv.stride(2) == 1
    if step_rows:
        n_tile = part_max_tbn.shape[2]
        assert step_rows >= B and part_max_tbn.shape[:2] == (T, B) and part_sum_tbn.shape == part_max_tbn.shape
        for x, w in ((part_max_tbn, n_tile), (part_sum_tbn, n_tile)) + (((src_tbv, V),) if src_tbv is not None else ()):
            assert x.stride(2) == 1 and x.stride(1) == w and x.stride(0) == step_rows * w, (x.shape, x.stride())
    else:
        assert part_max_tbn.is_contiguous() and part_sum_tbn.is_contiguous()
        assert part_max_tbn.shape[:2] == (T, B) and part_sum_tbn.shape == part_max_tbn.shape
        assert src_tbv is None or (src_tbv.is_contiguous() and src_tbv.shape == (T, B, V))
    check(_lib.load().isc_logsoftmax_apply_steps(logits_btv.data_ptr(), logits_btv.stride(0), logits_btv.stride(1), B, T,
                                                 V, part_max_tbn.data_ptr(), part_sum_tbn.data_ptr(), ptr(src_tbv),
                                                 int(step_rows), stream()),
          'isc_logsoftmax_apply_steps')


def _planes_ptrs(planes, like):
    if planes is None:
        return None, None
    assert planes.dtype == torch.float16 and planes.is_contiguous() and planes.shape == (2,) + tuple(like.shape)
    return planes_ptrs(planes)


def scan_problem(P, V, q, w, w_bias, out, alpha_out=None, q2=None, out_planes=None, row_ids=None, row_div=1):
    s = ScanProblem()
    assert P.is_contiguous() and V.is_contiguous() and q.is_contiguous() and out.is_contiguous()
    s.P, s.V, s.q, s.q2, s.w = P.data_ptr(), V.data_ptr(), q.data_ptr(), ptr(q2), w.data_ptr()
    s.w_bias = ptr(w_bias)
    if row_ids is not None:
        assert row_ids.dtype == torch.int64 and row_ids.dim() == 2 and row_ids.stride(1) == 1 and P.dim() == 2
        s.row_ids, s.row_ids_ld = row_ids.data_ptr(), row_ids.stride(0)
        s.R, s.A, s.D = row_ids.shape[1], P.shape[1], V.shape[1]
    else:
        s.R, s.A, s.D = P.shape[1], P.shape[2], V.shape[2]
    s.out = out.data_ptr()
    s.out_hi, s.out_lo = _planes_ptrs(out_planes, out)
    if alpha_out is not None:
        assert alpha_out.stride(1) == 1
        s.alpha_out, s.alpha_ld = alpha_out.data_ptr(), alpha_out.stride(0)
    row_div = max(int(row_div), 1)
    if row_div > 1:
        per_image = (row_ids if row_ids is not None else P).shape[0]
        assert q.shape[0] == per_image * row_div and (q2 is None or q2.shape[0] == per_image)
        s.row_div = row_div
    return s


def attn_scan_fwd(problems, B):
    lib = _lib.load()
    arr = (ScanProblem * len(problems))(*problems)
    e0 = TIMER.begin()
    check(lib.isc_attn_scan_fwd(arr, len(problems), B, stream()), 'isc_attn_scan_fwd')
    if e0 is not None:
        nb = sum(4.0 * B / max(q.row_div, 1) * q.R * (q.A + q.D) for q in problems)
        TIMER.end(e0, 'attn_scan[' + '+'.join('%dx%dx%d' % (B, q.R, q.A) for q in problems) + ']', 0.0, nb)


def attn_scan_gate_fwd(scans, G, zh, b_gc, b_gs, w_gate, b_gate, f, beta_out=None, f_planes=None):
    a = _lib.ScanGateArgs()
    for i in range(2):
        C.memmove(C.byref(a.scan[i]), C.byref(scans[i]), C.sizeof(ScanProblem))
        a.scan[i].out = None
        a.scan[i].out_hi = a.scan[i].out_lo = None
        assert G[i].is_contiguous() and G[i].dtype == torch.float32
        a.G[i] = G[i].data_ptr()
    B = zh.shape[0]
    assert zh.is_contiguous() and f.is_contiguous()
    a.zh, a.b_gc, a.b_gs, a.w_gate, a.b_gate = zh.data_ptr(), b_gc.data_ptr(), b_gs.data_ptr(), w_gate.data_ptr(), ptr(b_gate)
    a.f = f.data_ptr()
    a.f_hi, a.f_lo = _planes_ptrs(f_planes, f)
    if beta_out is not None:
        a.beta, a.beta_ld = beta_out.data_ptr(), beta_out.stride(0)
    e0 = TIMER.begin()
    check(_lib.load().isc_attn_scan_gate_fwd(C.byref(a), B, stream()), 'isc_attn_scan_gate_fwd')
    if e0 is not None:
        nb = sum(4.0 * B * q.R * (2 * q.A + q.D) for q in scans)
        TIMER.end(e0, 'attn_scan_gate[' + '+'.join('%dx%dx%d' % (B, q.R, q.A) for q in scans) + ']', 0.0, nb)


def gate_mix_fwd(z, w, w_bias, v, s, out, beta_out=None, out_planes=None):
    lib = _lib.load()
    B, A = z.shape
    D = v.shape[1]
    assert z.is_contiguous() and v.is_contiguous() and s.is_contiguous() and out.is_contiguous()
    bl = beta_out.stride(0) if beta_out is not None else 0
    e0 = TIMER.begin()
    check(lib.isc_gate_mix_fwd(z.data_ptr(), w.data_ptr(), ptr(w_bias), v.data_ptr(), s.data_ptr(), B, A, D,
                               out.data_ptr(), ptr(beta_out), bl, *_planes_ptrs(out_planes, out), stream()),
          'isc_gate_mix_fwd')
    TIMER.end(e0, 'gate_mix[%dx%d]' % (B, A), 0.0, 4.0 * B * (A + 3 * D))


def embed_relu_fwd(emb, ids, out, add=None):
    lib = _lib.load()
    V, W = emb.shape
    assert ids.dtype == torch.int64 and ids.dim() == 1 and out.is_contiguous()
    check(lib.isc_embed_relu_fwd(emb.data_ptr(), V, W, ids.data_ptr(), ids.stride(0), ptr(add),
                                 ids.shape[0], out.data_ptr(), stream()), 'isc_embed_relu_fwd')


def embed_relu_mean_fwd(emb, ids, out):
    lib = _lib.load()
    V, W = emb.shape
    assert ids.dtype == torch.int64 and ids.is_contiguous()
    B, Cn = ids.shape
    check(lib.isc_embed_relu_mean_fwd(emb.data_ptr(), V, W, ids.data_ptr(), Cn, B, out.data_ptr(),
                                      stream()), 'isc_embed_relu_mean_fwd')


def embed_senti_words_fwd(emb, ids, pad_id, out, keep_mask=None, mask_scale=1.0):
    lib = _lib.load()
    V, W = emb.shape
    assert ids.dtype == torch.int64 and ids.is_contiguous()
    B, n = ids.shape
    check(lib.isc_embed_senti_words_fwd(emb.data_ptr(), V, W, ids.data_ptr(), n, pad_id, B,
                                        ptr(keep_mask), mask_scale, out.data_ptr(), stream()),
          'isc_embed_senti_words_fwd')


def rollout_finalize(step):
    lib = _lib.load()
    e0 = TIMER.begin()
    check(lib.isc_rollout_finalize(C.byref(step), stream()), 'isc_rollout_finalize')
    TIMER.end(e0, 'rollout_finalize[%d]' % step.B, 0.0, 4.0 * step.B * (3 * step.n_tile + 2 * step.W))


def check_sample_filter(temperature, top_k, top_p):
    import math
    t, p = float(temperature), float(top_p)
    if not (math.isfinite(t) and t > 0.0):
        raise ValueError('temperature must be finite and > 0, got %r' % (temperature,))
    if int(top_k) != top_k or top_k < 0:
        raise ValueError('top_k must be an integer >= 0 (0: off), got %r' % (top_k,))
    if not p > 0.0:
        raise ValueError('top_p must be > 0 (>= 1: off), got %r' % (top_p,))
    return t, int(top_k), p


def rollout_finalize_filtered(step, temperature=1.0, top_k=0, top_p=1.0, sampling_logprobs=None):
    f = _lib.SampleFilter()
    f.temperature, f.top_k, f.top_p = check_sample_filter(temperature, top_k, top_p)
    f.sampling_logprobs = ptr(sampling_logprobs)
    lib = _lib.load()
    e0 = TIMER.begin()
    check(lib.isc_rollout_finalize_filtered(C.byref(step), C.byref(f), stream()), 'isc_rollout_finalize_filtered')
    TIMER.end(e0, 'rollout_finalize_filtered[%d]' % step.B, 0.0, 4.0 * step.B * (step.V + 2 * step.n_tile + 2 * step.W))


def check_decode_constraints(suppress_special, decoding_constraint, min_len, max_seq_len):
    if not isinstance(suppress_special, (bool, int)) or suppress_special not in (0, 1):
        raise ValueError('suppress_special must be a bool, got %r' % (suppress_special,))
    if not isinstance(decoding_constraint, (bool, int)) or decoding_constraint not in (0, 1):
        raise ValueError('decoding_constraint must be 0 or 1, got %r' % (decoding_constraint,))
    if isinstance(min_len, bool) or not hasattr(min_len, '__index__') or not 0 <= int(min_len) <= int(max_seq_len):
        raise ValueError('min_len must be an integer in [0, max_seq_len = %r], got %r' % (max_seq_len, min_len))
    return bool(suppress_special), bool(decoding_constraint), int(min_len)


def decode_constraints(ban_ids=(), no_repeat=False, first_id=0, min_len=0):
    ban_ids = [int(i) for i in ban_ids]
    if len(ban_ids) > 8:
        raise ValueError('at most 8 banned ids, got %d' % len(ban_ids))
    c = _lib.DecodeConstraints()
    for k, i in enumerate(ban_ids):
        c.ban_ids[k] = i
    c.n_ban, c.no_repeat, c.first_id, c.min_len = len(ban_ids), int(bool(no_repeat)), int(first_id), int(min_len)
    return c


def rollout_finalize_constrained(step, cons, filt=None, sampling_logprobs=None):
    f = None
# ... 667 lines not shown
```

Baseline: 438,800.

## Add lean rollout path skipping f32 hidden-state writes and zero-state GEMM segments

Adds a 'lean' greedy-rollout mode that drops the f32 h1/h2 (and gate feature) buffers when fp16 hi/lo planes carry the state, so LSTM, gate-mix and vocab kernels write and read only the planes. A probe entry point checks that every GEMM stage would route to a planes-capable kernel before the mode is enabled. At t=0 a state_zero flag removes the recurrent segments whose inputs are zero, or runs a cells-only LSTM kernel when a token table supplies the gates. This cuts memory traffic and GEMM work per step, at the cost of extra routing complexity and a separate cache key for the captured graph.

```diff
diff --git a/include/insenticap_hip.h b/include/insenticap_hip.h
--- a/include/insenticap_hip.h
+++ b/include/insenticap_hip.h
@@ -88,6 +88,7 @@
 } isc_lstm_problem;
 
 int isc_lstm_fwd(const isc_lstm_problem *prob_host, void *stream);
+long long isc_lstm_cells_launches(void);
 
 int isc_vocab_fwd(const float *h, int ldh, const float *W, int ldw, const float *bias,
                   int M, int V, int K, float *logits, int64_t ld_logits,
@@ -271,11 +272,13 @@
     const int64_t *words_ids;
     int64_t words_ids_ld;
     const float *gate_Gc, *gate_Gs;
-    int32_t pair_rows_c, _pad2;
+    int32_t pair_rows_c;
+    int32_t state_zero;
     int32_t row_div, pre_rows;
 } isc_step_plan;
 
 int isc_step_fwd(const isc_step_plan *plan_host, void *stream);
+int isc_step_fwd_check(const isc_step_plan *plan_host, void *stream);
 
 int isc_set_stream_gate(const int32_t *flag, void *stream);
 
diff --git a/insenticap_model_amd/_lib.py b/insenticap_model_amd/_lib.py
--- a/insenticap_model_amd/_lib.py
+++ b/insenticap_model_amd/_lib.py
@@ -75,7 +75,7 @@
                  ('splitk_ws', C.c_void_p), ('splitk_ws_floats', C.c_int64)] +
                 _f('h1_prev_hi h1_prev_lo h2_prev_hi h2_prev_lo h1_hi h1_lo h2_hi h2_lo '
                    'v_hi v_lo s_hi s_lo f_hi f_lo words_ids', C.c_void_p) + [('words_ids_ld', C.c_int64)] +
-                _f('gate_Gc gate_Gs', C.c_void_p) + _f('pair_rows_c _pad2 row_div pre_rows', C.c_int32))
+                _f('gate_Gc gate_Gs', C.c_void_p) + _f('pair_rows_c state_zero row_div pre_rows', C.c_int32))
 
 
 class StepBwdPlan(C.Structure):
@@ -188,6 +188,8 @@
     'isc_gemm_bwd': (C.c_int, [C.POINTER(LinearProblem), C.c_int, C.c_int, C.c_void_p]),
     'isc_lstm_fwd': (C.c_int, [C.POINTER(LstmProblem), C.c_void_p]),
     'isc_step_fwd': (C.c_int, [C.POINTER(StepPlan), C.c_void_p]),
+    'isc_step_fwd_check': (C.c_int, [C.POINTER(StepPlan), C.c_void_p]),
+    'isc_lstm_cells_launches': (C.c_longlong, []),
     'isc_set_stream_gate': (C.c_int, [C.c_void_p, C.c_void_p]),
     'isc_step_bwd': (C.c_int, [C.POINTER(StepBwdPlan), C.c_void_p]),
     'isc_rows_stats_tile': (C.c_int, [C.c_int]),
diff --git a/insenticap_model_amd/captioner.py b/insenticap_model_amd/captioner.py
--- a/insenticap_model_amd/captioner.py
+++ b/insenticap_model_amd/captioner.py
@@ -421,22 +421,22 @@
 
     def _step(self, p, P, ws, xt, h_cur, c_cur, h_nxt, c_nxt, alpha_c=None, alpha_s=None, beta=None,
               logits=None, out_mask=None, out_scale=1.0, save=None, tok=None, normalize=False,
-              hp_cur=None, hp_nxt=None, rows_ext=None):
-        if ops.TIMER.armed:
+              hp_cur=None, hp_nxt=None, rows_ext=None, state_zero=False, probe=False):
+        if ops.TIMER.armed and not probe:
             return self._step_py(p, P, ws, xt, h_cur, c_cur, h_nxt, c_nxt, alpha_c, alpha_s, beta, logits,
                                  out_mask, out_scale, save, tok, normalize, hp_cur, hp_nxt)
         save = save or {}
         pl = ws.get('_plan')
         if pl is None:
-            pl = ws['_plan'] = self._make_plan(p, P, h_cur[0].shape[0])
+            pl = ws['_plan'] = self._make_plan(p, P, c_cur[0].shape[0])
         ptr = ops.ptr
         pl.xt = ptr(xt)
         if tok is not None and P.tab is not None:
             pl.tok, pl.tok_stride = tok.data_ptr(), tok.stride(0)
-        pl.h1_prev, pl.h2_prev, pl.c1_prev, pl.c2_prev = (h_cur[0].data_ptr(), h_cur[1].data_ptr(),
+        pl.h1_prev, pl.h2_prev, pl.c1_prev, pl.c2_prev = (ptr(h_cur[0]), ptr(h_cur[1]),
                                                           c_cur[0].data_ptr(), c_cur[1].data_ptr())
-        pl.h1, pl.h2, pl.c1, pl.c2 = (h_nxt[0].data_ptr(), h_nxt[1].data_ptr(), c_nxt[0].data_ptr(),
-                                      c_nxt[1].data_ptr())
+        pl.h1, pl.h2, pl.c1, pl.c2 = ptr(h_nxt[0]), ptr(h_nxt[1]), c_nxt[0].data_ptr(), c_nxt[1].data_ptr()
+        pl.state_zero = int(bool(state_zero))
         if hp_cur is not None:
             pl.h1_prev_hi, pl.h1_prev_lo = ops.planes_ptrs(hp_cur[0])
             pl.h2_prev_hi, pl.h2_prev_lo = ops.planes_ptrs(hp_cur[1])
@@ -459,12 +459,14 @@
         pl.beta, pl.beta_ld = (beta.data_ptr(), beta.stride(0)) if beta is not None else (None, 0)
         hdrop = None
         if out_mask is not None:
-            hdrop = save['hdrop'] if 'hdrop' in save else self._new(h_cur[0].shape[0], pl.H)
+            hdrop = save['hdrop'] if 'hdrop' in save else self._new(c_cur[0].shape[0], pl.H)
         pl.out_mask, pl.out_scale, pl.hdrop = ptr(out_mask), out_scale, ptr(hdrop)
         pl.logits, pl.ld_logits = (logits.data_ptr(), logits.stride(0)) if logits is not None else (None, 0)
         pl.apply_logsoftmax = int(normalize)
         pl.pmax, pl.psum, pl.pidx = ptr(ws.get('pmax')), ptr(ws.get('psum')), ptr(ws.get('pidx'))
         pl.gate_Gc, pl.gate_Gs = ptr(getattr(P, 'gate_Gc', None)), ptr(getattr(P, 'gate_Gs', None))
+        if probe:
+            return ops.step_fwd_ok(pl)
         if rows_ext is not None:
             ops.rows_step_fwd(pl, rows_ext)
         else:
@@ -821,7 +823,8 @@
 
     def _graphed_rollout(self, fc_feats, att_feats, cpt_words, senti_words, senti_labels, T):
         ins = [self._feat(fc_feats), self._feat(att_feats), cpt_words, senti_words, senti_labels]
-        key = (tuple((tuple(x.shape), x.dtype) for x in ins), T, self._weights_key(), torch.cuda.current_device())
+        key = (tuple((tuple(x.shape), x.dtype) for x in ins), T, self._weights_key(), torch.cuda.current_device(),
+               bool(getattr(self, 'rollout_lean', True)))
         cache = self._rollout_graphs
         st = self._rollout_stream()
         idx = self._dev.index if self._dev.index is not None else torch.cuda.current_device()
@@ -996,25 +999,39 @@
             rows_ext.stats_tile = ops.rows_stats_tile(V)
         planes = rows_ext is None and getattr(self, 'state_planes', True)
         f32, i64 = torch.float32, torch.int64
-        h0, c0, hp0 = self._zeros_many(((2, B, H), f32), ((2, B, H), f32),
+        ws = self._alloc_step_ws(B, P, rows_ext.stats_tile if rows_ext is not None else 128)
+        use_tab = P.tab is not None
+        xt = [None, None] if use_tab else [self._new(B, Wd) for _ in range(2)]
+        c1 = self._new(2, B, H)
+        sos = torch.full((B,), self.sos_id, dtype=torch.int64, device=self._dev)
+        hp1 = torch.empty(2, 2, B, H, dtype=torch.float16, device=self._dev) if planes else None
+        if planes:
+            for k in ('v', 's', 'f'):
+                if k in ws:
+                    ws[k + 'p'] = torch.empty((2,) + tuple(ws[k].shape), dtype=torch.float16, device=self._dev)
+        lean_on = getattr(self, 'rollout_lean', True)
+        lean = False
+        if (lean_on and planes and arm is None and not torch.is_grad_enabled() and masks is None
+                and (not self.training or self.drop.p == 0.0) and ops.h3_mode() != 0):
+            fused_gate = getattr(P, 'gate_Gc', None) is not None and getattr(P, 'gate_Gs', None) is not None
+            f_rows = None if fused_gate else ws.pop('f', None)
+            with ops.h3_weights_scope(self._dev):
+                lean = self._step(p, P, ws, xt[0], (None, None), c1, (None, None), c1, hp_cur=hp1, hp_nxt=hp1,
+                                  tok=sos if use_tab else None, probe=True)
+            if not lean and f_rows is not None:
+                ws['f'] = f_rows
+        h0, c0, hp0 = self._zeros_many(((0,) if lean else (2, B, H), f32), ((2, B, H), f32),
                                        ((2, 2, B, H) if planes else (0,), torch.float16))
         seq, raw, seq_logprobs, seq_masks, alive, aC, aS, bG, unf = self._zeros_many(
             ((B, T), i64), ((B, T), i64), ((B, T), f32), ((B, T), f32), ((T + 1,), torch.int32), ((B, T, P.R), f32),
             ((B, T, P.Mw), f32), ((B, T), f32), ((T + 1, B), torch.int32))
-        h, c = [h0, self._new(2, B, H)], [c0, self._new(2, B, H)]
-        hp = [hp0, torch.empty(2, 2, B, H, dtype=torch.float16, device=self._dev)] if planes else [None, None]
-        ws = self._alloc_step_ws(B, P, rows_ext.stats_tile if rows_ext is not None else 128)
-        if hp[0] is not None:
-            for k in ('v', 's', 'f'):
-                if k in ws:
-                    ws[k + 'p'] = torch.empty((2,) + tuple(ws[k].shape), dtype=torch.float16, device=self._dev)
+        h = [(None, None), (None, None)] if lean else [h0, self._new(2, B, H)]
+        c = [c0, c1]
+        hp = [hp0, hp1] if planes else [None, None]
         unf[0:1].fill_(1)
         unfinished = unf[0]
         alive[0:1].fill_(B)
-        use_tab = P.tab is not None
-        xt = [None, None] if use_tab else [self._new(B, Wd) for _ in range(2)]
         emb = p['word_embed.0.weight']
-        sos = torch.full((B,), self.sos_id, dtype=torch.int64, device=self._dev)
         if not use_tab:
             ops.embed_relu_fwd(emb, sos, xt[0])
         need_logits = (not sample_max) or cons is not None
@@ -1062,7 +1079,8 @@
                         rows_ext.fin_prev = rows_ext.fin_unfinished_out = None
                 self._step(p, P, ws, xt[cur], h[cur], c[cur], h[nxt], c[nxt], aC[:, t], aS[:, t], bG[:, t:t + 1],
                            logits, om, osc, tok=(sos if t == 0 else seq[:, t - 1]) if use_tab else None,
-                           hp_cur=hp[cur], hp_nxt=hp[nxt], rows_ext=rows_ext)
+                           hp_cur=hp[cur], hp_nxt=hp[nxt], rows_ext=rows_ext,
+                           state_zero=(t == 0 and lean_on and rows_ext is None))
                 if fuse and t + 1 < T:
                     continue
                 rs.t = t
diff --git a/insenticap_model_amd/csrc/attention.hip b/insenticap_model_amd/csrc/attention.hip
--- a/insenticap_model_amd/csrc/attention.hip
+++ b/insenticap_model_amd/csrc/attention.hip
@@ -699,7 +699,7 @@
             float4 f;
             f.x = beta * a.x + (1.0f - beta) * c.x; f.y = beta * a.y + (1.0f - beta) * c.y;
             f.z = beta * a.z + (1.0f - beta) * c.z; f.w = beta * a.w + (1.0f - beta) * c.w;
-            o4[d] = f;
+            if (out) o4[d] = f;
             if (out_hi) store_planes4(out_hi, out_lo, b, 4 * d, D, f);
         }
         return;
@@ -707,7 +707,7 @@
     for (int d = lane; d < D; d += 64) {
         const long long o = (long long)b * D + d;
         const float f = beta * v[o] + (1.0f - beta) * s[o];
-        out[o] = f;
+        if (out) out[o] = f;
         if (out_hi) {
             const long long po = plane_index(b, d, D);
             isc_split_f16(f, out_hi[po], out_lo[po]);
@@ -718,8 +718,9 @@
 extern "C" int isc_gate_mix_fwd(const float *z, const float *w, const float *w_bias, const float *v,
                                 const float *s, int B, int A, int D, float *out, float *beta_out,
                                 int64_t beta_ld, void *out_hi, void *out_lo, void *stream) {
-    if (!z || !w || !v || !s || !out) return ISC_E_NULL;
+    if (!z || !w || !v || !s) return ISC_E_NULL;
     if ((out_hi == nullptr) != (out_lo == nullptr)) return ISC_E_NULL;
+    if (!out && !out_hi) return ISC_E_NULL;
     if ((D & 3) == 0 && (!isc_aligned16(v) || !isc_aligned16(s) || !isc_aligned16(out))) return ISC_E_ALIGN;
     if (B <= 0 || A <= 0 || D <= 0) return ISC_E_SHAPE;
     hipLaunchKernelGGL(gate_mix_kernel, dim3((B + 3) / 4), dim3(256), 0, (hipStream_t)stream, z, w,
diff --git a/insenticap_model_amd/csrc/gemm_f32.hip b/insenticap_model_amd/csrc/gemm_f32.hip
--- a/insenticap_model_amd/csrc/gemm_f32.hip
+++ b/insenticap_model_amd/csrc/gemm_f32.hip
@@ -345,7 +345,7 @@
         if (ok[e]) {
             const long long o = (long long)gm[e] * H + unit;
             P.c_out[o] = c2;
-            P.h_out[o] = h2;
+            if (P.h_out) P.h_out[o] = h2;
             if (P.h_hi) {
                 const long long po = plane_index(gm[e], unit, H);
                 isc_split_f16(h2, P.h_hi[po], P.h_lo[po]);
@@ -1015,7 +1015,7 @@
             if (ok[r]) {
                 const long long o = (long long)gm[r] * H + u0;
                 *reinterpret_cast<float2 *>(P.c_out + o) = make_float2(c2[0], c2[1]);
-                *reinterpret_cast<float2 *>(P.h_out + o) = make_float2(h2[0], h2[1]);
+                if (P.h_out) *reinterpret_cast<float2 *>(P.h_out + o) = make_float2(h2[0], h2[1]);
                 if (P.h_hi) {
                     typedef _Float16 h2v __attribute__((ext_vector_type(2)));
                     _Float16 a0, a1, l0, l1;
@@ -1866,6 +1866,26 @@
     lstm_cells<1>(P, gma, unit, ok, g);
 }
 
+__global__ __launch_bounds__(256) void lstm_cells_only_kernel(const DevLaunch L) {
+    ISC_GATE_RETURN(L);
+    const DevProb &P = L.p[0];
+    const int H = P.H;
+    const long long i = (long long)blockIdx.x * 256 + threadIdx.x;
+    if (i >= (long long)((P.M + 3) >> 2) * H) return;
+    const int m0 = (int)(i / H) * 4, unit = (int)(i % H);
+    int gm[4];
+    bool ok[4];
+    float g[4][4];
+#pragma unroll
+    for (int e = 0; e < 4; ++e) {
+        gm[e] = m0 + e;
+        ok[e] = gm[e] < P.M;
+#pragma unroll
+        for (int k = 0; k < 4; ++k) g[e][k] = 0.f;
+    }
+    lstm_cells<4>(P, gm, unit, ok, g);
+}
+
 __device__ __forceinline__ void wave_vocab_tile128(const DevProb &P, int gm, int tn, const float (&v)[2], int lane) {
     float x[2];
     int col[2];
@@ -2109,7 +2129,8 @@
 static int check_segs(const isc_seg *seg, int nseg) {
     if (nseg < 1 || nseg > ISC_MAX_SEG) return ISC_E_SHAPE;
     for (int s = 0; s < nseg; ++s) {
-        if (!seg[s].A || !seg[s].W) return ISC_E_NULL;
+        const bool planes = seg[s].A_hi && seg[s].A_lo && !seg[s].a_f16;
+        if ((!seg[s].A && !planes) || !seg[s].W) return ISC_E_NULL;
         if (seg[s].K <= 0 || (seg[s].K % BK) != 0) return ISC_E_SHAPE;
         if ((seg[s].lda & 3) || (seg[s].ldw & 3)) return ISC_E_ALIGN;
         if (!isc_aligned16(seg[s].A) || !isc_aligned16(seg[s].W)) return ISC_E_ALIGN;
@@ -3038,13 +3059,22 @@
     return (int)S;
 }
 
+static bool segs_planes_only(const DevLaunch &L) {
+    for (int i = 0; i < L.nprob; ++i)
+        for (int s = 0; s < L.p[i].nseg; ++s)
+            if (!L.p[i].seg[s].A) return true;
+    return false;
+}
+
 template <int EPI>
 static int route_nt(DevLaunch &L, float *ws, long long ws_floats, hipStream_t st, bool allow_xl, bool decide_only) {
-    if (const int kmax = gemv_plan<EPI>(L)) return decide_only ? 0 : gemv_run<EPI>(L, kmax, st);
+    const bool no_rows = !decide_only && segs_planes_only(L);
+    if (const int kmax = gemv_plan<EPI>(L)) return decide_only ? 0 : (no_rows ? ISC_E_NULL : gemv_run<EPI>(L, kmax, st));
     const H3sPlan hs = h3s_plan<EPI>(L, ws, ws_floats, st, 0);
-    if (hs.T) return decide_only ? 0 : h3s_run<EPI>(L, hs, ws, ws_floats, st, 0);
+    if (hs.T) return decide_only ? 2 : h3s_run<EPI>(L, hs, ws, ws_floats, st, 0);
     if (plan_splitk(L, ws, ws_floats) > 1) {
         if (decide_only) return 0;
+        if (no_rows) return ISC_E_NULL;
         finish_tiling(L, 2);
         const int rc = launch_any<EPI_LINEAR, false, false>(L, 2, st);
         return rc ? rc : launch_splitk_reduce<EPI>(L, st);
@@ -3052,6 +3082,7 @@
     const H3Plan h = h3_plan<EPI>(L, ws, ws_floats, st, 0);
     if (h.take) return decide_only ? 1 : h3_run<EPI>(L, h, ws, st, 0);
     if (decide_only) return 0;
+    if (no_rows) return ISC_E_NULL;
     const int tile = pick_tile(L, allow_xl, true, true);
     finish_tiling(L, tile);
     return launch_any<EPI, false, false>(L, tile, st);
@@ -3180,12 +3211,17 @@
     return gemm_bwd_run(pr, n_prob, layout, (hipStream_t)stream);
 }
 
-extern "C" int isc_lstm_fwd(const isc_lstm_problem *q, void *stream) {
+static std::atomic<long long> g_lstm_cells_launches{0};
+extern "C" long long isc_lstm_cells_launches(void) { return g_lstm_cells_launches.load(); }
+
+static int lstm_fwd_run(const isc_lstm_problem *q, void *stream, bool decide_only) {
     if (!q) return ISC_E_NULL;
-    int rc = check_segs(q->seg, q->nseg);
+    int rc = q->nseg == 0 ? ISC_OK : check_segs(q->seg, q->nseg);
     if (rc) return rc;
     if (segs_any_f16(q->seg, q->nseg)) return ISC_E_SHAPE;
-    if (!q->c_prev || !q->h_out || !q->c_out) return ISC_E_NULL;
+    if (!q->c_prev || !q->c_out) return ISC_E_NULL;
+    if ((q->h_hi == nullptr) != (q->h_lo == nullptr)) return ISC_E_NULL;
+    if (!q->h_out && (!q->h_hi || q->h_keep_mask)) return ISC_E_NULL;
     if ((!q->b_ih || !q->b_hh) && !q->pre) return ISC_E_NULL;
     if ((q->b_ih == nullptr) != (q->b_hh == nullptr)) return ISC_E_NULL;
     if (q->tab && !q->tab_ids) return ISC_E_NULL;
@@ -3201,19 +3237,33 @@
     d.bias0 = q->b_ih; d.bias1 = q->b_hh;
     d.c_prev = q->c_prev; d.h_out = q->h_out; d.c_out = q->c_out; d.gates_out = q->gates_out;
     d.hmask = q->h_keep_mask; d.mask_scale = q->mask_scale; d.hdrop = q->hdrop_out;
-    if ((q->h_hi == nullptr) != (q->h_lo == nullptr)) return ISC_E_NULL;
     d.h_hi = static_cast<_Float16 *>(q->h_hi); d.h_lo = static_cast<_Float16 *>(q->h_lo);
     d.pre = q->pre; d.tab = q->tab; d.tab_ids = q->tab_ids; d.tab_ids_stride = q->tab_ids_stride;
     d.pre_div = q->pre_div > 1 ? q->pre_div : 1;
-    return route_nt<EPI_LSTM>(L, q->splitk_ws, q->splitk_ws_floats, (hipStream_t)stream, !q->pre && !q->tab, false);
-}
-
-extern "C" int isc_vocab_fwd(const float *h, int ldh, const float *W, int ldw, const float *bias,
-                             int M, int V, int K, float *logits, int64_t ld_logits,
-                             float *part_max, float *part_sum, int32_t *part_idx,
-                             const void *h_hi, const void *h_lo,
-                             float *splitk_ws, int64_t splitk_ws_floats, void *stream) {
-    if (!h || !W || !bias || !part_max || !part_sum || !part_idx) return ISC_E_NULL;
+    if (q->nseg == 0) {
+        if (decide_only) return 0;
+        const long long n = (long long)((q->M + 3) >> 2) * q->H;
+        hipLaunchKernelGGL(lstm_cells_only_kernel, dim3((unsigned)((n + 255) / 256)), dim3(256), 0, (hipStream_t)stream, L);
+        ++g_lstm_cells_launches;
+        ISC_LAUNCH_CHECK();
+        return ISC_OK;
+    }
+    return route_nt<EPI_LSTM>(L, q->splitk_ws, q->splitk_ws_floats, (hipStream_t)stream, !q->pre && !q->tab, decide_only);
+}
+
+extern "C" int isc_lstm_fwd(const isc_lstm_problem *q, void *stream) { return lstm_fwd_run(q, stream, false); }
+
+int isc_lstm_route_(const isc_lstm_problem *q, void *stream) { return lstm_fwd_run(q, stream, true); }
+int isc_linear_route_(const isc_linear_problem *pr, int n_prob, void *stream) {
+    return linear_fwd_run(pr, n_prob, stream, true);
+}
+
+static int vocab_fwd_run(const float *h, int ldh, const float *W, int ldw, const float *bias,
+                         int M, int V, int K, float *logits, int64_t ld_logits,
+                         float *part_max, float *part_sum, int32_t *part_idx,
+                         const void *h_hi, const void *h_lo,
+                         float *splitk_ws, int64_t splitk_ws_floats, void *stream, bool decide_only) {
+    if (!W || !bias || !part_max || !part_sum || !part_idx) return ISC_E_NULL;
     isc_seg sg = {h, W, ldh, ldw, K, 0, h_hi, h_lo};
     int rc = check_segs(&sg, 1);
     if (rc) return rc;
@@ -3227,5 +3277,20 @@
     d.C = logits; d.ld_logits = ld_logits;
     d.pmax = part_max; d.psum = part_sum; d.pidx = part_idx;
     d.ntile_total = (V + 127) / 128;
-    return route_nt<EPI_VOCAB>(L, splitk_ws, splitk_ws_floats, (hipStream_t)stream, false, false);
-}
+    return route_nt<EPI_VOCAB>(L, splitk_ws, splitk_ws_floats, (hipStream_t)stream, false, decide_only);
+}
+
+extern "C" int isc_vocab_fwd(const float *h, int ldh, const float *W, int ldw, const float *bias,
+                             int M, int V, int K, float *logits, int64_t ld_logits,
+                             float *part_max, float *part_sum, int32_t *part_idx,
+                             const void *h_hi, const void *h_lo,
+                             float *splitk_ws, int64_t splitk_ws_floats, void *stream) {
+    return vocab_fwd_run(h, ldh, W, ldw, bias, M, V, K, logits, ld_logits, part_max, part_sum, part_idx, h_hi, h_lo,
+                         splitk_ws, splitk_ws_floats, stream, false);
+}
+int isc_vocab_route_(const float *W, int ldw, const float *bias, int M, int V, int K, float *part_max, float *part_sum,
+                     int32_t *part_idx, const void *h_hi, const void *h_lo, float *splitk_ws, int64_t splitk_ws_floats,
+                     void *stream) {
+    return vocab_fwd_run(nullptr, K, W, ldw, bias, M, V, K, nullptr, 0, part_max, part_sum, part_idx, h_hi, h_lo,
+                         splitk_ws, splitk_ws_floats, stream, true);
+}
diff --git a/insenticap_model_amd/csrc/rows.hip b/insenticap_model_amd/csrc/rows.hip
--- a/insenticap_model_amd/csrc/rows.hip
+++ b/insenticap_model_amd/csrc/rows.hip
@@ -1099,6 +1099,7 @@
     if (!p || !x) return ISC_E_NULL;
     if (!isc_rows_step_supported(p)) return ISC_E_SHAPE;
     if (!p->pmax || !p->psum || !p->pidx) return ISC_E_NULL;
+    if (!p->h1_prev || !p->h2_prev || !p->h1 || !p->h2 || (p->att_e && p->words_e && !p->f)) return ISC_E_NULL;
     hipStream_t st = (hipStream_t)stream;
     const int rows = p->rows, H = p->H, E = p->E, A = p->A, W = p->W, V = p->V;
     const int ld1 = H + E + W, ld2 = E + H;
diff --git a/insenticap_model_amd/csrc/step.hip b/insenticap_model_amd/csrc/step.hip
--- a/insenticap_model_amd/csrc/step.hip
+++ b/insenticap_model_amd/csrc/step.hip
@@ -13,7 +13,13 @@
         if (rc__) return rc__; \
     } while (0)
 
-extern "C" int isc_step_fwd(const isc_step_plan *p, void *stream) {
+int isc_lstm_route_(const isc_lstm_problem *q, void *stream);
+int isc_linear_route_(const isc_linear_problem *pr, int n_prob, void *stream);
+int isc_vocab_route_(const float *W, int ldw, const float *bias, int M, int V, int K, float *part_max, float *part_sum,
+                     int32_t *part_idx, const void *h_hi, const void *h_lo, float *splitk_ws, int64_t splitk_ws_floats,
+                     void *stream);
+
+static int step_fwd_run(const isc_step_plan *p, void *stream, bool probe) {
     if (!p) return ISC_E_NULL;
     const int rows = p->rows, H = p->H, E = p->E, A = p->A, W = p->W, V = p->V;
     if (rows <= 0 || H <= 0) return ISC_E_SHAPE;
@@ -38,6 +44,22 @@
     const bool wplanes = planes && (!has_c || (p->v_hi && p->v_lo)) && (!has_s || (p->s_hi && p->s_lo)) &&
                          (!gate || (p->f_hi && p->f_lo));
 #define PW(x) (wplanes ? (x) : nullptr)
+    const bool lean = !p->h1 || !p->h2 || !p->h1_prev || !p->h2_prev || (gate && !p->f);
+    if (lean && (!planes || p->out_mask || !p->pmax || (gate && !p->f && (!wplanes || (p->gate_Gc && p->gate_Gs)))))
+        return ISC_E_NULL;
+    if (lean && !probe) RET(step_fwd_run(p, stream, true));
+    auto planes_only = [](const isc_seg *sg, int n) {
+        for (int i = 0; i < n; ++i)
+            if (!sg[i].A) return true;
+        return false;
+    };
+    auto on_planes = [](int route) { return route < 0 ? route : (route == 1 || route == 2 ? ISC_OK : ISC_E_NULL); };
+    auto lstm_on_large_tiles = [&](isc_lstm_problem l, int keep0, int nkeep) {
+        if (isc_lstm_route_(&l, stream) != 1) return false;
+        for (int i = 0; i < nkeep; ++i) l.seg[i] = l.seg[keep0 + i];
+        l.nseg = nkeep;
+        return isc_lstm_route_(&l, stream) == 1;
+    };
 
     {
         isc_lstm_problem l = {};
@@ -51,7 +73,14 @@
         l.pre = p->pre1; l.tab = p->tab; l.tab_ids = p->tok; l.tab_ids_stride = p->tok_stride;
         l.pre_div = p->pre_rows ? 1 : row_div;
         l.splitk_ws = p->splitk_ws; l.splitk_ws_floats = p->splitk_ws_floats;
-        RET(isc_lstm_fwd(&l, stream));
+        if (p->state_zero && p->tab) {
+            l.nseg = 0;
+        } else if (p->state_zero && lstm_on_large_tiles(l, 1, 1)) {
+            l.seg[0] = l.seg[1];
+            l.nseg = 1;
+        }
+        if (probe && lean && planes_only(l.seg, l.nseg)) RET(on_planes(isc_lstm_route_(&l, stream)));
+        if (!probe) RET(isc_lstm_fwd(&l, stream));
     }
     {
         isc_linear_problem q[3] = {};
@@ -65,7 +94,8 @@
         if (has_s) lin(p->W_h2word, p->b_h2word, p->qw, off_s, rows_s);
         if (gate) lin(p->W_gh, p->b_gh, p->z, 0, rows);
         q[0].splitk_ws = p->splitk_ws; q[0].splitk_ws_floats = p->splitk_ws_floats;
-        RET(isc_linear_fwd(q, n, stream));
+        if (probe && lean && !p->h1) RET(on_planes(isc_linear_route_(q, n, stream)));
+        if (!probe) RET(isc_linear_fwd(q, n, stream));
     }
     const bool fused_gate = gate && p->gate_Gc && p->gate_Gs;
     {
@@ -87,7 +117,8 @@
             x.row_ids = p->words_ids; x.row_ids_ld = p->words_ids_ld;
             x.rows = rows_s; x.row_div = row_div;
         }
-        if (fused_gate) {
+        if (probe) {
+        } else if (fused_gate) {
             isc_scan_gate_args g = {};
             g.scan[0] = sc[0]; g.scan[1] = sc[1];
             g.scan[0].out = nullptr; g.scan[0].out_hi = g.scan[0].out_lo = nullptr;
@@ -111,8 +142,8 @@
         x.nseg = 2; x.M = rows; x.N = A; x.bias0 = p->b_gc; x.bias1 = p->b_gs; x.ldc = A; x.C = p->z;
         x.accumulate = 1;
         x.splitk_ws = p->splitk_ws; x.splitk_ws_floats = p->splitk_ws_floats;
-        RET(isc_linear_fwd(&x, 1, stream));
-        RET(isc_gate_mix_fwd(p->z, p->w_gate, p->b_gate, p->v, p->s, rows, A, E, p->f, p->beta, p->beta_ld,
+        if (!probe) RET(isc_linear_fwd(&x, 1, stream));
+        if (!probe) RET(isc_gate_mix_fwd(p->z, p->w_gate, p->b_gate, p->v, p->s, rows, A, E, p->f, p->beta, p->beta_ld,
                              PW(p->f_hi), PW(p->f_lo), stream));
         feat = p->f; feat_hi = PW(p->f_hi); feat_lo = PW(p->f_lo);
     }
@@ -126,20 +157,29 @@
         l.c_prev = p->c2_prev; l.h_out = p->h2; l.c_out = p->c2; l.gates_out = p->g2;
         l.h_keep_mask = p->out_mask; l.mask_scale = p->out_scale; l.hdrop_out = p->hdrop;
         l.splitk_ws = p->splitk_ws; l.splitk_ws_floats = p->splitk_ws_floats;
-        RET(isc_lstm_fwd(&l, stream));
-    }
-    if (p->pmax)
+        if (p->state_zero && lstm_on_large_tiles(l, 0, 2)) l.nseg = 2;
+        if (probe && lean && planes_only(l.seg, l.nseg)) RET(on_planes(isc_lstm_route_(&l, stream)));
+        if (!probe) RET(isc_lstm_fwd(&l, stream));
+    }
+    if (probe && p->pmax && lean && !p->h2)
+        RET(on_planes(isc_vocab_route_(p->W_cls, H, p->b_cls, rows, V, H, p->pmax, p->psum, p->pidx, PL(p->h2_hi),
+                                       PL(p->h2_lo), p->splitk_ws, p->splitk_ws_floats, stream)));
+    if (p->pmax && !probe)
     RET(isc_vocab_fwd(p->out_mask ? p->hdrop : p->h2, H, p->W_cls, H, p->b_cls, rows, V, H, p->logits,
                       p->ld_logits, p->pmax, p->psum, p->pidx, p->out_mask ? nullptr : PL(p->h2_hi),
                       p->out_mask ? nullptr : PL(p->h2_lo), p->splitk_ws, p->splitk_ws_floats, stream));
 #undef PL
 #undef PW
+    if (probe) return ISC_OK;
     if (p->apply_logsoftmax) {
         if (!p->logits || !p->pmax) return ISC_E_NULL;
         RET(isc_logsoftmax_apply(p->logits, p->ld_logits, rows, V, p->pmax, p->psum, nullptr, stream));
     }
     return ISC_OK;
 }
+
+extern "C" int isc_step_fwd(const isc_step_plan *p, void *stream) { return step_fwd_run(p, stream, false); }
+extern "C" int isc_step_fwd_check(const isc_step_plan *p, void *stream) { return step_fwd_run(p, stream, true); }
 
 static inline isc_linear_problem nn_problem(const float *A, int lda, const float *Wm, int ldw, int K, int M,
                                             int N, float *C, int accumulate) {
diff --git a/insenticap_model_amd/ops.py b/insenticap_model_amd/ops.py
--- a/insenticap_model_amd/ops.py
+++ b/insenticap_model_amd/ops.py
@@ -430,10 +430,11 @@
              mask_scale=1.0, hdrop_out=None, pre=None, tab=None, tab_ids=None, h_planes=None, pre_div=1, ws=None):
     lib = _lib.load()
     p = LstmProblem()
-    _fill_segs(p.seg, segs)
+    if segs:
+        _fill_segs(p.seg, segs)
     p.nseg = len(segs)
     p.M, p.H = c_prev.shape
-    assert c_prev.is_contiguous() and h_out.is_contiguous() and c_out.is_contiguous()
+    assert c_prev.is_contiguous() and (h_out is None or h_out.is_contiguous()) and c_out.is_contiguous()
     p.b_ih, p.b_hh = ptr(b_ih), ptr(b_hh)
     if pre is not None:
         pre_div = max(int(pre_div), 1)
@@ -442,7 +443,7 @@
     if tab is not None:
         assert tab.is_contiguous() and tab.shape[1] == 4 * p.H and tab_ids.dtype == torch.int64
         p.tab, p.tab_ids, p.tab_ids_stride = tab.data_ptr(), tab_ids.data_ptr(), tab_ids.stride(0)
-    p.c_prev, p.h_out, p.c_out = c_prev.data_ptr(), h_out.data_ptr(), c_out.data_ptr()
+    p.c_prev, p.h_out, p.c_out = c_prev.data_ptr(), ptr(h_out), c_out.data_ptr()
     p.gates_out = ptr(gates_out)
     p.h_keep_mask = ptr(h_keep_mask)
     p.mask_scale = mask_scale
@@ -463,6 +464,14 @@
 
 def step_fwd(plan):
     check(_lib.load().isc_step_fwd(C.byref(plan), stream()), 'isc_step_fwd')
+
+
+def step_fwd_ok(plan):
+    return _lib.load().isc_step_fwd_check(C.byref(plan), stream()) == 0
+
+
+def lstm_cells_launches():
+    return _lib.load().isc_lstm_cells_launches()
 
 
 class stream_gate:
@@ -674,11 +683,11 @@
     lib = _lib.load()
     B, A = z.shape
     D = v.shape[1]
-    assert z.is_contiguous() and v.is_contiguous() and s.is_contiguous() and out.is_contiguous()
+    assert z.is_contiguous() and v.is_contiguous() and s.is_contiguous() and (out is None or out.is_contiguous())
     bl = beta_out.stride(0) if beta_out is not None else 0
     e0 = TIMER.begin()
     check(lib.isc_gate_mix_fwd(z.data_ptr(), w.data_ptr(), ptr(w_bias), v.data_ptr(), s.data_ptr(), B, A, D,
-                               out.data_ptr(), ptr(beta_out), bl, *_planes_ptrs(out_planes, out), stream()),
+                               ptr(out), ptr(beta_out), bl, *_planes_ptrs(out_planes, v), stream()),
           'isc_gate_mix_fwd')
     TIMER.end(e0, 'gate_mix[%dx%d]' % (B, A), 0.0, 4.0 * B * (A + 3 * D))
 
```

After: 441,500 (median of 6 runs). Within noise of the previous version (+0.6%).
